# santi-pdp/segan_pytorch

Hardware: AMD Instinct MI355X
Metric: 16384-sample waveform chunks/sec (GAN step) (higher is better)
Workload: dtype f32

## Files before the change

### include/segan_hip.h

```cpp
#ifndef SEGAN_HIP_H
#define SEGAN_HIP_H

#include <stddef.h>
#include <stdint.h>

#ifdef __cplusplus
extern "C" {
#endif

#define SEGAN_ABI_VERSION 17

#define SEGAN_PAD_REFLECT 0
#define SEGAN_PAD_ZERO 1

#define SEGAN_ACT_NONE 0
#define SEGAN_ACT_TANH 1

typedef struct segan_src {
  const float* p0;
  const float* p1;
  int32_t C0;
  int32_t C1;
  const float* scale;
  const float* shift;
// ... 2 lines not shown

int segan_abi_version(void);
const char* segan_last_error(void);

int segan_set_reserved_slots(int n);

size_t segan_packed_f_bytes(int M, int N, int S);
size_t segan_packed_t_bytes(int M, int N, int S);

int segan_pack_weights(const float* w, float* wf, float* wt, int M, int N, int K, int S,
                       int pad_t, void* stream);

#define SEGAN_PREC_FP32 0
#define SEGAN_PREC_BF16 1
#define SEGAN_PREC_BF16X3 3
#define SEGAN_PREC_FP32_BLOCKED 4
size_t segan_packed_bf_bytes(int M, int N, int S, int tform, int planes);
int segan_pack_weights_bf(const float* w, void* out, int M, int N, int K, int S, int tform,
                          int pad_t, int planes, void* stream);

size_t segan_bf16_scratch_bytes(int op, int B, int N, int M, int L, int K, int S, int pad, int planes);
size_t segan_corr_scratch_bytes(void);
void segan_debug_last_corr(int* out6);
void segan_debug_last_wgrad(int* out6);

int segan_conv1d_fwd(const segan_src* x, const void* wf, const float* bias, float* out, int B,
                     int N, int M, int L, int K, int S, int padL, int mode, int roll,
                     int precision, void* scratch, size_t scratch_bytes, void* stream);

int segan_conv1d_dgrad(const float* da, const void* wt, const float* w, float* dx, float* halo,
                       int B, int N, int M, int L, int K, int S, int padL, int roll, int precision,
                       void* scratch, size_t scratch_bytes, void* stream);

#define SEGAN_WGRAD_DETERMINISTIC 1
size_t segan_wgrad_scratch_bytes(int B, int M, int N, int Ls, int S, int precision, int flags);
int segan_wgrad(const segan_src* lo, const segan_src* hi, float* dw, int B, int M, int N, int Ls,
                int K, int S, int padL, int mode, int roll, int precision, int flags, void* scratch,
                size_t scratch_bytes, void* stream);

int segan_deconv1d_fwd(const segan_src* x, const void* wt, const float* w, const float* bias,
                       float* y, int B, int M, int N, int Ls, int K, int S, int pad, int act,
                       int precision, void* scratch, size_t scratch_bytes, void* stream);

int segan_deconv1d_dgrad(const float* dy, const void* wf, float* dx0, float* dx1, int B, int M,
                         int M0, int N, int Ls, int K, int S, int pad, int precision, void* scratch,
                         size_t scratch_bytes, void* stream);


int segan_bn_nsplit(int B, int C, int L);
int segan_bn_stats(const float* x, const float* gamma, const float* beta, float eps,
                   float momentum, float* running_mean, float* running_var, float* mean,
                   float* rstd, float* scale, float* shift, float* ws, int B, int C, int L,
                   void* stream);
int segan_bn_partial(const float* x, float* ws, int B, int C, int L, void* stream);
int segan_bn_final(const float* ws, int nsplit_total, const float* gamma, const float* beta,
                   float eps, float momentum, float* running_mean, float* running_var, float* mean,
                   float* rstd, float* scale, float* shift, int C, void* stream);

int segan_affine_tanh(const float* x, const float* scale, const float* shift, float* y, int B,
                      int C, int L, void* stream);
int segan_scale_mask(const float* x, const float* scale, const float* mask, float* y, int B, int C,
                     int L, void* stream);

int segan_affine_prelu(const float* x, const float* scale, const float* shift, const float* slope,
                       float* y, int B, int C, int L, void* stream);

int segan_sum_skip(const float* x0, const float* slope0, const float* x1, const float* alpha,
                   float* out, int B, int C, int L, void* stream);

int segan_act_bwd(const float* a, const float* dh, const float* dskip, const float* slope,
                  const float* alpha, const float* bn_mean, const float* bn_rstd,
                  const float* bn_gamma, const float* bn_beta, float* da, float* dslope,
                  float* dalpha, float* dgamma, float* dbeta, float* dbias, float* ws, int B, int C,
                  int L, void* stream);
int segan_act_bwd_bn_reduce(const float* a, const float* dh, const float* slope,
                            const float* bn_mean, const float* bn_rstd, const float* bn_gamma,
                            const float* bn_beta, float* dslope, float* dgamma, float* dbeta,
                            float* totals, float* ws, int B, int C, int L, void* stream);
int segan_act_bwd_bn_apply(const float* a, const float* dh, const float* slope,
                           const float* bn_mean, const float* bn_rstd, const float* bn_gamma,
                           const float* bn_beta, const float* totals, float* da, float* dbias,
                           float* ws, int B, int C, int L, double count_total, void* stream);

int segan_tanh_bwd(const float* y, const float* dy, const float* clean, float l1_scale, float* da,
                   float* dbias, float* ws, int B, int C, int L, void* stream);


#define SEGAN_GEMM_DETERMINISTIC 1
size_t segan_gemm_scratch_bytes(int M, int N, int K);
int segan_gemm(const float* A, int64_t sam, int64_t sak, const float* B, int64_t sbk, int64_t sbn,
               float* C, int64_t ldc, int M, int N, int K, int beta0, int flags, void* scratch,
               size_t scratch_bytes, void* stream);

int segan_bias_prelu_rows(const float* x, const float* bias, const float* slope, float* y,
                          int rows, int cols, void* stream);
int segan_bias_prelu_rows_bwd(const float* x, const float* bias, const float* slope,
                              const float* dy, float* dx, float* dslope, float* dbias, int rows,
                              int cols, void* stream);

int segan_mse_const(const float* x, float target, float* loss, float* grad, const float* gout,
                    float gscale, int n, void* stream);
int segan_bce_logits_const(const float* x, float target, float* loss, float* grad,
                           const float* gout, float gscale, int n, void* stream);
int segan_l1_mean(const float* x, const float* y, float* loss, float* ws, int64_t n,
                  void* stream);
int segan_l1_bwd(const float* x, const float* y, const float* gout, float gscale, float* grad,
                 int64_t n, void* stream);

size_t segan_packed_g_bytes(int M, int N, int S);
int segan_pack_weights_g(const float* w, float* wg, int M, int N, int K, int S, void* stream);
int segan_conv1d_dgrad_short(const float* da, const float* wg, float* dx, int B, int N, int M,
                             int L, int K, int S, int padL, int roll, void* stream);

int segan_pool_time_fwd(const float* x, float* y, int* idx, int rows, int L, int mode,
                        void* stream);
int segan_pool_time_bwd(const float* dy, const int* idx, float* dx, int rows, int L, int mode,
                        void* stream);

int segan_mse_mean(const float* x, const float* y, float* loss, float* ws, int64_t n,
                   void* stream);
int segan_mse_bwd(const float* x, const float* y, const float* gout, float gscale, float* grad,
                  int64_t n, void* stream);

size_t segan_snorm_ws_floats(int A, int Bd, int K, int dim);
int segan_snorm_fwd(const float* w, float* u, float* v, float* w_sn, float* sigma, float* ws, int A,
                    int Bd, int K, int dim, int power_iteration, float eps, void* stream);
int segan_snorm_bwd(const float* dw_sn, const float* w, const float* u, const float* v,
                    const float* sigma, float* dw, float* ws, int A, int Bd, int K, int dim,
                    void* stream);

int segan_stft_pitch(int n_fft);
int segan_stft_basis(float* basis, int n_fft, int win, void* stream);
int segan_stft_frames(const float* x, float* frames, int B, int T, int n_fft, int hop, int win,
                      void* stream);
int segan_powdb(const float* S, float* db, int64_t rows, int nbins, int pitch, float eps,
                void* stream);
int segan_powdb_bwd(const float* S, const float* ddb, float* dS, int64_t rows, int nbins, int pitch,
                    float eps, void* stream);
int segan_stft_overlap_add(const float* dframes, float* dx, int B, int T, int n_fft, int hop,
                           int win, void* stream);

int segan_pcm16_prep(const int16_t* pcm, const unsigned char* first, float* clean, float* noisy,
                     int B, int T, double coef, void* stream);

int segan_deemphasis(const float* y, float* x, int rows, int T, double coef, void* stream);
int segan_ssnr_frames(int T, int srate);
int segan_ssnr(const float* ref, const float* deg, float* seg, float* out, int rows, int T,
               int srate, double eps, void* stream);
int segan_wss(const float* ref, const float* deg, double* dist, int rows, int T, int srate,
              void* stream);
int segan_llr(const float* ref, const float* deg, double* dist, int rows, int T, int srate,
              void* stream);
int segan_stoi_plan(int srate, int* pq, int* ntaps, double* taps, int cap, int* bands);
int segan_stoi_dims(int T, int srate, int* dims);
int segan_stoi(const float* ref, const float* deg, const int* lengths, int rows, int T, int srate,
               double* xr, double* yr, double* energy, int* mask, int* kept, int* count,
               double* xs, double* ys, double* X, double* Y, double* rho, double* d, void* stream);

int segan_asl_p56(const float* x, const int* lengths, int rows, int T, int srate, int nbits,
                  double* level, int* counts, int* status, double* q, void* stream);
int segan_additive_mix(const float* clean, const int* lengths, const float* bank, int64_t n_bank,
                       const int64_t* starts, const double* snr_db, const double* px,
                       const float* prev, int rows, int T, float* noisy, float* prev_out,
                       double* info, int* istat, void* stream);
int segan_pcm16_wave(const int16_t* pcm, const int* index, float* wave, float* prev, int n, int B,
                     int T, void* stream);
// ... 35 lines not shown
```

### segan_pytorch_amd/_lib.py

```python
import ctypes
import os
from ctypes import POINTER, Structure, c_char_p, c_double, c_float, c_int, c_int32, c_int64, c_size_t, c_void_p

_HERE = os.path.dirname(os.path.abspath(__file__))
LIB_PATH = os.environ.get('SEGAN_HIP_LIB') or os.path.join(_HERE, 'libsegan_hip.so')

PAD_REFLECT = 0
PAD_ZERO = 1
ACT_NONE = 0
ACT_TANH = 1
ABI_VERSION = 17


class SeganSrc(Structure):
    _fields_ = [('p0', c_void_p), ('p1', c_void_p), ('C0', c_int32), ('C1', c_int32),
                ('scale', c_void_p), ('shift', c_void_p), ('slope', c_void_p)]


_P = c_void_p
_SRC = POINTER(SeganSrc)

SIGNATURES = {
    'segan_abi_version': (c_int, []),
    'segan_set_reserved_slots': (c_int, [c_int]),
    'segan_last_error': (c_char_p, []),
    'segan_packed_f_bytes': (c_size_t, [c_int, c_int, c_int]),
    'segan_packed_t_bytes': (c_size_t, [c_int, c_int, c_int]),
    'segan_pack_weights': (c_int, [_P, _P, _P, c_int, c_int, c_int, c_int, c_int, _P]),
    'segan_packed_bf_bytes': (c_size_t, [c_int, c_int, c_int, c_int, c_int]),
    'segan_pack_weights_bf': (c_int, [_P, _P, c_int, c_int, c_int, c_int, c_int, c_int, c_int, _P]),
    'segan_corr_scratch_bytes': (c_size_t, []),
    'segan_bf16_scratch_bytes': (c_size_t, [c_int] * 9),
    'segan_debug_last_corr': (None, [POINTER(c_int)]),
    'segan_debug_last_wgrad': (None, [POINTER(c_int)]),
    'segan_conv1d_fwd': (c_int, [_SRC, _P, _P, _P, c_int, c_int, c_int, c_int, c_int, c_int, c_int,
                                 c_int, c_int, c_int, _P, c_size_t, _P]),
    'segan_conv1d_dgrad': (c_int, [_P, _P, _P, _P, _P, c_int, c_int, c_int, c_int, c_int, c_int, c_int,
                                   c_int, c_int, _P, c_size_t, _P]),
    'segan_wgrad': (c_int, [_SRC, _SRC, _P, c_int, c_int, c_int, c_int, c_int, c_int, c_int, c_int,
                            c_int, c_int, c_int, _P, c_size_t, _P]),
    'segan_wgrad_scratch_bytes': (c_size_t, [c_int, c_int, c_int, c_int, c_int, c_int, c_int]),
    'segan_deconv1d_fwd': (c_int, [_SRC, _P, _P, _P, _P, c_int, c_int, c_int, c_int, c_int, c_int, c_int,
                                   c_int, c_int, _P, c_size_t, _P]),
    'segan_deconv1d_dgrad': (c_int, [_P, _P, _P, _P, c_int, c_int, c_int, c_int, c_int, c_int, c_int,
                                     c_int, c_int, _P, c_size_t, _P]),
    'segan_bn_nsplit': (c_int, [c_int, c_int, c_int]),
    'segan_bn_stats': (c_int, [_P, _P, _P, c_float, c_float, _P, _P, _P, _P, _P, _P, _P, c_int, c_int,
                               c_int, _P]),
    'segan_bn_partial': (c_int, [_P, _P, c_int, c_int, c_int, _P]),
    'segan_bn_final': (c_int, [_P, c_int, _P, _P, c_float, c_float, _P, _P, _P, _P, _P, _P, c_int, _P]),
    'segan_act_bwd_bn_reduce': (c_int, [_P] * 12 + [c_int, c_int, c_int, _P]),
    'segan_act_bwd_bn_apply': (c_int, [_P] * 11 + [c_int, c_int, c_int, c_double, _P]),
    'segan_affine_prelu': (c_int, [_P, _P, _P, _P, _P, c_int, c_int, c_int, _P]),
    'segan_affine_tanh': (c_int, [_P, _P, _P, _P, c_int, c_int, c_int, _P]),
    'segan_scale_mask': (c_int, [_P, _P, _P, _P, c_int, c_int, c_int, _P]),
    'segan_sum_skip': (c_int, [_P, _P, _P, _P, _P, c_int, c_int, c_int, _P]),
    'segan_bce_logits_const': (c_int, [_P, c_float, _P, _P, _P, c_float, c_int, _P]),
    'segan_act_bwd': (c_int, [_P] * 16 + [c_int, c_int, c_int, _P]),
    'segan_tanh_bwd': (c_int, [_P, _P, _P, c_float, _P, _P, _P, c_int, c_int, c_int, _P]),
    'segan_gemm_scratch_bytes': (c_size_t, [c_int, c_int, c_int]),
    'segan_gemm': (c_int, [_P, c_int64, c_int64, _P, c_int64, c_int64, _P, c_int64, c_int, c_int,
                           c_int, c_int, c_int, _P, c_size_t, _P]),
    'segan_bias_prelu_rows': (c_int, [_P, _P, _P, _P, c_int, c_int, _P]),
    'segan_bias_prelu_rows_bwd': (c_int, [_P, _P, _P, _P, _P, _P, _P, c_int, c_int, _P]),
    'segan_mse_const': (c_int, [_P, c_float, _P, _P, _P, c_float, c_int, _P]),
    'segan_l1_bwd': (c_int, [_P, _P, _P, c_float, _P, c_int64, _P]),
    'segan_l1_mean': (c_int, [_P, _P, _P, _P, c_int64, _P]),
    'segan_packed_g_bytes': (c_size_t, [c_int, c_int, c_int]),
    'segan_pack_weights_g': (c_int, [_P, _P, c_int, c_int, c_int, c_int, _P]),
    'segan_conv1d_dgrad_short': (c_int, [_P, _P, _P, c_int, c_int, c_int, c_int, c_int, c_int, c_int,
                                        c_int, _P]),
    'segan_pool_time_fwd': (c_int, [_P, _P, _P, c_int, c_int, c_int, _P]),
    'segan_pool_time_bwd': (c_int, [_P, _P, _P, c_int, c_int, c_int, _P]),
    'segan_mse_mean': (c_int, [_P, _P, _P, _P, c_int64, _P]),
    'segan_mse_bwd': (c_int, [_P, _P, _P, c_float, _P, c_int64, _P]),
    'segan_snorm_ws_floats': (c_size_t, [c_int, c_int, c_int, c_int]),
    'segan_snorm_fwd': (c_int, [_P, _P, _P, _P, _P, _P, c_int, c_int, c_int, c_int, c_int, c_float, _P]),
    'segan_snorm_bwd': (c_int, [_P, _P, _P, _P, _P, _P, _P, c_int, c_int, c_int, c_int, _P]),
    'segan_pcm16_prep': (c_int, [_P, _P, _P, _P, c_int, c_int, c_double, _P]),
    'segan_stft_basis': (c_int, [_P, c_int, c_int, _P]),
    'segan_stft_frames': (c_int, [_P, _P, c_int, c_int, c_int, c_int, c_int, _P]),
    'segan_stft_pitch': (c_int, [c_int]),
    'segan_powdb': (c_int, [_P, _P, c_int64, c_int, c_int, c_float, _P]),
    'segan_powdb_bwd': (c_int, [_P, _P, _P, c_int64, c_int, c_int, c_float, _P]),
    'segan_stft_overlap_add': (c_int, [_P, _P, c_int, c_int, c_int, c_int, c_int, _P]),
    'segan_deemphasis': (c_int, [_P, _P, c_int, c_int, c_double, _P]),
    'segan_ssnr_frames': (c_int, [c_int, c_int]),
    'segan_ssnr': (c_int, [_P, _P, _P, _P, c_int, c_int, c_int, c_double, _P]),
    'segan_wss': (c_int, [_P, _P, _P, c_int, c_int, c_int, _P]),
    'segan_llr': (c_int, [_P, _P, _P, c_int, c_int, c_int, _P]),
    'segan_stoi_plan': (c_int, [c_int, POINTER(c_int), POINTER(c_int), _P, c_int, POINTER(c_int)]),
    'segan_stoi_dims': (c_int, [c_int, c_int, POINTER(c_int)]),
    'segan_stoi': (c_int, [_P, _P, _P, c_int, c_int, c_int] + [_P] * 13),
    'segan_asl_p56': (c_int, [_P, _P, c_int, c_int, c_int, c_int, _P, _P, _P, _P, _P]),
    'segan_additive_mix': (c_int, [_P, _P, _P, c_int64, _P, _P, _P, _P, c_int, c_int, _P, _P, _P, _P, _P]),
    'segan_resample_plan': (c_int, [c_int, c_int, c_int, c_double, POINTER(c_int), POINTER(c_int), _P, c_int]),
    'segan_resample_dims': (c_int, [c_int, c_int, c_int, POINTER(c_int)]),
    'segan_resample': (c_int, [_P, c_int, _P, c_int, c_int, c_int, c_int, c_int, c_double, _P, c_int,
                               c_int, _P, _P, _P, _P]),
    'segan_pcm16_wave': (c_int, [_P, _P, _P, _P, c_int, c_int, c_int, _P]),
    'segan_preemph_rows': (c_int, [_P, _P, _P, _P, _P, c_int, c_int, c_int, c_double, _P]),
    'segan_rmsprop_step': (c_int, [_P, _P, _P, c_float, c_float, c_float, c_int64, _P]),
    'segan_adam_step': (c_int, [_P, _P, _P, _P, c_float, c_double, c_double, c_float, c_int, c_int64,
                                _P]),
    'segan_fill': (c_int, [_P, c_float, c_int64, _P]),
    'segan_scale': (c_int, [_P, c_float, c_int64, _P]),
    'segan_comm_id_bytes': (c_int, []),
    'segan_comm_unique_id': (c_int, [_P]),
    'segan_comm_init': (c_int, [POINTER(c_void_p), c_int, c_int, _P]),
    'segan_comm_destroy': (c_int, [_P]),
    'segan_comm_rank': (c_int, [_P]),
    'segan_comm_world': (c_int, [_P]),
    'segan_allreduce': (c_int, [_P, _P, c_size_t, c_float, _P]),
    'segan_broadcast': (c_int, [_P, _P, c_size_t, c_int, _P]),
    'segan_allgather': (c_int, [_P, _P, _P, c_size_t, _P]),
}

_lib = None


def load():
    global _lib
    if _lib is not None:
# ... 30 lines not shown
```

### segan_pytorch_amd/csrc/segan_common.h

```cpp
#pragma once
#include <hip/hip_runtime.h>
#include <stdint.h>
#include <stdio.h>
#include <stdarg.h>
#include "../../include/segan_hip.h"

#define SEGAN_OK 0
#define SEGAN_EINVAL (-1)
#define SEGAN_ELAUNCH (-2)
#define SEGAN_EUNSUPPORTED (-3)

void segan_set_error(const char* fmt, ...);
int segan_check_launch(const char* what);

#define SEGAN_REQUIRE(cond, ...)                 \
  do {                                           \
    if (!(cond)) {                               \
      segan_set_error(__VA_ARGS__);              \
      return SEGAN_EINVAL;                       \
    }                                            \
  } while (0)

typedef float f32x16 __attribute__((ext_vector_type(16)));
typedef float f32x4 __attribute__((ext_vector_type(4)));

#define SEGAN_ACC_BLOCK 8

template <int NI, int NJ>
__device__ __forceinline__ void acc_block_flush(f32x16 (&acc)[NI][NJ], f32x16 (&sum)[NI][NJ]) {
#pragma unroll
  for (int i = 0; i < NI; ++i)
#pragma unroll
    for (int j = 0; j < NJ; ++j) {
      sum[i][j] += acc[i][j];
#pragma unroll
      for (int e = 0; e < 16; ++e) acc[i][j][e] = 0.0f;
    }
}

int segan_reserved_slots_value(void);
static inline int segan_grid_slots(int occ) {
  const int g = 256 * occ - segan_reserved_slots_value();
  return g < 64 ? 64 : g;
}

static inline int ceil_div(int a, int b) { return (a + b - 1) / b; }
static inline int round_up(int a, int b) { return ceil_div(a, b) * b; }

__host__ __device__ static inline int segan_hi_index(int p, int L, int padL, int mode, int roll) {
  int i = p - padL;
  if (mode == SEGAN_PAD_REFLECT) {
    if (i < 0) i = -i;
    if (i >= L) i = 2 * (L - 1) - i;
  }
  if (i < 0 || i >= L) return -1;
  if (roll != 0) {
    i -= roll;
    if (i < 0) i += L;
    if (i >= L) i -= L;
  }
  return i;
}

#define SEGAN_MAX_XF_CH 16384

struct ChanXf {
  float sc, sh, sl;
};

__device__ __forceinline__ ChanXf segan_chan_xf(const segan_src& s, int c) {
  ChanXf x;
  x.sc = s.scale[c];
  x.sh = s.shift[c];
  x.sl = s.slope[c];
  return x;
}

__device__ __forceinline__ float segan_apply_xf(const ChanXf& x, float v) {
  v = fmaf(v, x.sc, x.sh);
  return v > 0.0f ? v : v * x.sl;
}

int segan_src_defaults(segan_src* s, hipStream_t st, const char* what);

__device__ __forceinline__ const float* segan_src_row(const segan_src& s, int b, int n, int L) {
  if (n < s.C0) return s.p0 + ((size_t)b * s.C0 + n) * (size_t)L;
  return s.p1 + ((size_t)b * s.C1 + (n - s.C0)) * (size_t)L;
}

__device__ __forceinline__ float warp_sum(float v) {
#pragma unroll
  for (int o = 32; o > 0; o >>= 1) v += __shfl_down(v, o, 64);
  return v;
}
```

### segan_pytorch_amd/csrc/segan_conv.hip

```cpp
#include "segan_conv_shared.h"

template <int MB, int NB, int WM, int U>
struct TileGeom {
  static constexpr int S = 32 / U;
  static constexpr int WN = 4 / WM;
  static constexpr int NI = MB / (32 * WM);
  static constexpr int NJ = NB / (32 * WN);
  static constexpr int NPT = MB / S;
};

struct TileWork {
  int tile, c0, c1;
  bool partial;
  int piece;
};

struct TileIter {
  int tileA;
  long unit, unit_end;
  int first_tile;
  __device__ __forceinline__ void init(const CorrArgs& a, int nch) {
    tileA = blockIdx.x;
    unit = (long)blockIdx.x * a.sk_units;
    unit_end = min(unit + (long)a.sk_units, a.sk_total);
// ... 1379 lines not shown
  SEGAN_REQUIRE(precision_ok(precision), "deconv1d_dgrad: precision must be 0, 1, 3 or 4");
  SEGAN_REQUIRE(stride_ok(S), "deconv1d_dgrad: stride %d not in {1,2,4}", S);
  SEGAN_REQUIRE(K >= 1 && K <= 32, "deconv1d_dgrad: kernel width %d not in [1,32]", K);
  SEGAN_REQUIRE(B > 0 && N > 0 && M > 0 && Ls > 0, "deconv1d_dgrad: bad sizes");
  SEGAN_REQUIRE(M0 >= 0 && M0 <= M, "deconv1d_dgrad: split %d outside [0,%d]", M0, M);
  SEGAN_REQUIRE(dy && wf, "deconv1d_dgrad: NULL pointer");
  SEGAN_REQUIRE(dx0 || dx1, "deconv1d_dgrad: both destinations NULL");
  const int U = 32 / S;
  CorrArgs a = {};
  a.acc_block = acc_block;
  a.in.p0 = dy; a.in.p1 = nullptr; a.in.C0 = N; a.in.C1 = 0;
  a.in.scale = a.in.shift = a.in.slope = nullptr;
  a.wp = (const float*)wf;
  a.bias = nullptr; a.halo = nullptr;
  a.B = B; a.Cv = N * S; a.Ktot = N * 32; a.RP = f_pitch(M); a.Rvalid = M;
  a.Tcols = Ls; a.Ctot = B * Ls;
  a.Lin = S * Ls; a.padL = pad; a.mode = SEGAN_PAD_ZERO; a.roll = 0;
  a.win_start = 0; a.H = U - 1;
  a.NP = 1; a.Nout = 0;
  if (M0 == 0) { a.out0 = dx1; a.OC0 = M; a.out1 = nullptr; a.OC1 = 0; }
  else { a.out0 = dx0; a.OC0 = M0; a.out1 = dx1; a.OC1 = M - M0; }
  a.Lout = Ls; a.act = SEGAN_ACT_NONE;
  a.out0_elems = (size_t)B * a.OC0 * Ls;
  a.out1_elems = (size_t)B * a.OC1 * Ls;
  a.f_pair = f_pair(N, K); a.zphase = -1;
  if (precision) {
    CorrArgs a2 = a;
    const int e = segan_corr_bf2_f(a2, U, wf, precision, scratch, scratch_bytes, (hipStream_t)stream);
    return e;
  }
  set_scratch(a, scratch, scratch_bytes);
  return launch_corr<true, false>(a, U, (hipStream_t)stream);
}

extern "C" int segan_deconv1d_fwd(const segan_src* x, const void* wt, const float* w,
                                  const float* bias, float* y, int B, int M, int N, int Ls, int K,
                                  int S, int pad, int act, int precision, void* scratch,
                                  size_t scratch_bytes, void* stream) {
  const int acc_block = precision == SEGAN_PREC_FP32_BLOCKED;
  if (acc_block) precision = SEGAN_PREC_FP32;
  SEGAN_REQUIRE(precision_ok(precision), "deconv1d_fwd: precision must be 0, 1, 3 or 4");
  SEGAN_REQUIRE(stride_ok(S), "deconv1d_fwd: stride %d not in {1,2,4}", S);
  SEGAN_REQUIRE(K >= 1 && K <= 32, "deconv1d_fwd: kernel width %d not in [1,32]", K);
  SEGAN_REQUIRE(B > 0 && N > 0 && M > 0 && Ls > 0, "deconv1d_fwd: bad sizes");
  SEGAN_REQUIRE(y && (wt || (w && N <= 2)), "deconv1d_fwd: NULL pointer");
  SEGAN_REQUIRE(pad >= 0 && K - 2 * pad - S == (K & 1),
                "deconv1d_fwd: K=%d S=%d pad=%d does not give an output of S*Ls samples", K, S, pad);
  SEGAN_REQUIRE(act == SEGAN_ACT_NONE || act == SEGAN_ACT_TANH, "deconv1d_fwd: bad activation");
  if (int e = check_src(x, M, "deconv1d_fwd")) return e;
  const int U = 32 / S;
  CorrArgs a = {};
  a.acc_block = acc_block;
  a.in = *x;
  a.wp = (const float*)wt;
  a.out0 = y; a.out1 = nullptr; a.bias = bias; a.halo = nullptr;
  a.NP = t_np(N, S); a.Nout = N;
  a.B = B; a.Cv = M; a.Ktot = M * U; a.RP = t_pitch(N, S); a.Rvalid = S * a.NP;
  a.Tcols = Ls; a.Ctot = B * Ls;
  a.Lin = Ls; a.padL = 0; a.mode = SEGAN_PAD_ZERO; a.roll = 0;
  int cmin = 1 << 30, cmax = 0;
  for (int r = 0; r < S; ++r) {
    const int c = (r + pad) / S;
    cmin = c < cmin ? c : cmin;
    cmax = c > cmax ? c : cmax;
  }
  for (int r = 0; r < 4; ++r) a.rowshift[r] = r < S ? (r + pad) / S - cmin : 0;
  a.win_start = cmin - (U - 1);
  a.H = U - 1 + (cmax - cmin);
  a.OC0 = N; a.OC1 = 0; a.Lout = S * Ls; a.act = act;
  a.o_padL = 0; a.o_roll = 0; a.o_padR = 0;
  a.out0_elems = (size_t)B * N * S * Ls;
  a.f_pair = 0; a.zphase = t_zphase(K, S, pad);
  if (w && N <= 2) return segan_launch_tsmall(a, w, K, M, N, S, pad, (hipStream_t)stream);
  if (precision && act == SEGAN_ACT_NONE) {
    CorrArgs a2 = a;
    const int e = segan_corr_bf2_t(a2, U, wt, precision, scratch, scratch_bytes, (hipStream_t)stream);
    return e;
  }
  SEGAN_REQUIRE(precision == 0, "deconv1d_fwd: tanh epilogue only on the fp32 path");
  set_scratch(a, scratch, scratch_bytes);
  return launch_corr<false, true>(a, U, (hipStream_t)stream);
}

extern "C" int segan_conv1d_dgrad(const float* da, const void* wt, const float* w, float* dx,
                                  float* halo, int B, int N, int M, int L, int K, int S, int padL,
                                  int roll, int precision, void* scratch, size_t scratch_bytes,
                                  void* stream) {
  const int acc_block = precision == SEGAN_PREC_FP32_BLOCKED;
  if (acc_block) precision = SEGAN_PREC_FP32;
  SEGAN_REQUIRE(precision_ok(precision), "conv1d_dgrad: precision must be 0, 1, 3 or 4");
  SEGAN_REQUIRE(stride_ok(S), "conv1d_dgrad: stride %d not in {1,2,4}", S);
  SEGAN_REQUIRE(K >= 1 && K <= 32, "conv1d_dgrad: kernel width %d not in [1,32]", K);
  SEGAN_REQUIRE(B > 0 && N > 0 && M > 0 && L > 0 && L % S == 0, "conv1d_dgrad: bad sizes");
  SEGAN_REQUIRE(da && dx && halo && (wt || (w && N <= 2)), "conv1d_dgrad: NULL pointer");
  SEGAN_REQUIRE(roll > -L && roll < L, "conv1d_dgrad: |roll| must be < L");
  const int padR = K - 1 - padL >= 0 ? (K - S - padL > 0 ? K - S - padL : 0) : -1;
  SEGAN_REQUIRE(padL >= 0 && padR >= 0 && padL < L && K - S - padL < L, "conv1d_dgrad: bad padding");
  const int U = 32 / S;
  const int Ls = L / S;
  hipStream_t st = (hipStream_t)stream;
  CorrArgs a = {};
  a.acc_block = acc_block;
  a.in.p0 = da; a.in.p1 = nullptr; a.in.C0 = M; a.in.C1 = 0;
  a.in.scale = a.in.shift = a.in.slope = nullptr;
  a.wp = (const float*)wt;
  a.out0 = dx; a.out1 = nullptr; a.bias = nullptr; a.halo = halo;
  a.NP = t_np(N, S); a.Nout = N;
  a.B = B; a.Cv = M; a.Ktot = M * U; a.RP = t_pitch(N, S); a.Rvalid = S * a.NP;
  a.Tcols = (L + padL + padR - 1) / S + 1;
  a.Ctot = B * a.Tcols;
  a.Lin = Ls; a.padL = 0; a.mode = SEGAN_PAD_ZERO; a.roll = 0;
  for (int r = 0; r < 4; ++r) a.rowshift[r] = 0;
  a.win_start = -(U - 1);
  a.H = U - 1;
  a.OC0 = N; a.OC1 = 0; a.Lout = L; a.act = SEGAN_ACT_NONE;
  a.o_padL = padL; a.o_roll = roll; a.o_padR = padR;
  a.out0_elems = (size_t)B * N * L;
  a.halo_elems = (size_t)B * N * (padL + padR);
  a.f_pair = 0; a.zphase = t_zphase(K, S, 0);
  set_scratch(a, scratch, scratch_bytes);
  int e;
  if (w && N <= 2) {
    e = segan_launch_tsmall(a, w, K, M, N, S, 0, st);
  } else if (precision) {
    CorrArgs a2 = a;
    e = segan_corr_bf2_t(a2, U, wt, precision, scratch, scratch_bytes, st);
  } else {
    e = launch_corr<false, true>(a, U, st);
  }
  if (e) return e;
  if (padL + padR > 0) {
    const int rows = B * N;
    const int per_sample = (padL < L - 1 - padR) ? 1 : 0;
    const long nthreads = per_sample ? (long)rows * (padL + padR) : rows;
    hipLaunchKernelGGL(fold_halo_kernel, dim3((unsigned)((nthreads + 255) / 256)), dim3(256), 0, st,
                       dx, halo, rows, L, padL, padR, roll, per_sample);
    return segan_check_launch("fold_halo_kernel");
  }
  return SEGAN_OK;
}

static bool short_ok(int N, int M, int L, int K, int S, int padL) {
  if (!stride_ok(S) || L % S != 0) return false;
  const int Ls = L / S;
  return (Ls == 4 || Ls == 8 || Ls == 16 || Ls == 32 || Ls == 64) && N % 4 == 0 &&
         M % CS_KC == 0 && K >= 1 && K <= 32 && padL >= 0 && K - 1 - padL >= 0 && padL < L &&
         K - S - padL < L;
}

extern "C" size_t segan_packed_g_bytes(int M, int N, int S) {
  if (!stride_ok(S) || M <= 0 || N <= 0) return 0;
  return (size_t)M * N * 32 * sizeof(float);
}

extern "C" int segan_pack_weights_g(const float* w, float* wg, int M, int N, int K, int S,
                                    void* stream) {
  SEGAN_REQUIRE(w && wg && M > 0 && N > 0, "pack_weights_g: bad arguments");
  SEGAN_REQUIRE(stride_ok(S) && K >= 1 && K <= 32, "pack_weights_g: stride in {1,2,4}, K <= 32");
  const size_t total = (size_t)M * N * 32;
  const int blocks = (int)((total + 255) / 256 > 8192 ? 8192 : (total + 255) / 256);
  hipLaunchKernelGGL(pack_g_kernel, dim3(blocks), dim3(256), 0, (hipStream_t)stream, w, wg, M, N, K,
                     S);
  return segan_check_launch("pack_weights_g");
}

extern "C" int segan_conv1d_dgrad_short(const float* da, const float* wg, float* dx, int B, int N,
                                        int M, int L, int K, int S, int padL, int roll,
                                        void* stream) {
  SEGAN_REQUIRE(da && wg && dx && B > 0, "conv1d_dgrad_short: bad arguments");
  SEGAN_REQUIRE(roll > -L && roll < L, "conv1d_dgrad_short: |roll| must be < L");
  if (!short_ok(N, M, L, K, S, padL)) {
    segan_set_error("conv1d_dgrad_short: geometry not covered (L/S in {4,8,16,32,64}, N %% 4 == 0, "
                    "M %% 16 == 0)");
    return SEGAN_EUNSUPPORTED;
  }
  ShortArgs a;
  a.da = da; a.wg = wg; a.dx = dx;
  a.B = B; a.N = N; a.M = M; a.L = L; a.Ls = L / S; a.padL = padL;
  a.padRw = K - S - padL > 0 ? K - S - padL : 0;
  a.roll = roll;
  a.ncoltiles = ceil_div(B, 128 / a.Ls);
  const size_t lds = 4 * 32 * 65 * sizeof(float);
  const dim3 grid((unsigned)(N / 4 * a.ncoltiles));
  static const bool blocked = [] {
    const char* e = getenv("SEGAN_SHORT_ORDER");
    return !(e && e[0] == '0');
  }();
  a.xr8 = a.xbc = 0;
  if (blocked && (N / 4) % 8 == 0) {
    a.xr8 = N / 4 / 8;
    a.xbc = a.xr8 >= 128 ? 1 : 128 / a.xr8;
  }
  hipStream_t st = (hipStream_t)stream;
  if (S == 4) hipLaunchKernelGGL(conv_dgrad_short_kernel<4>, grid, dim3(256), lds, st, a);
  else if (S == 2) hipLaunchKernelGGL(conv_dgrad_short_kernel<2>, grid, dim3(256), lds, st, a);
  else hipLaunchKernelGGL(conv_dgrad_short_kernel<1>, grid, dim3(256), lds, st, a);
  return segan_check_launch("conv_dgrad_short_kernel");
}
```

### segan_pytorch_amd/csrc/segan_conv_edge.hip

```cpp
#include "segan_conv_shared.h"

template <int S, int N, int PM, int KT>
__global__ __launch_bounds__(256) void tsmall_kernel(const CorrArgs a, const float* __restrict__ w,
                                                     int Krt, int M) {
  const int K = KT ? KT : Krt;
  constexpr int U = 32 / S;
  constexpr int MC = 16;
  constexpr int TW = 256 + U;
  __shared__ float xs[MC][TW + 1];
  const int tid = threadIdx.x;
  const int b = blockIdx.y;
  const int q0 = blockIdx.x * 256;
  const int q = q0 + tid;
  float acc[S][N];
#pragma unroll
  for (int r = 0; r < S; ++r)
#pragma unroll
    for (int n = 0; n < N; ++n) acc[r][n] = 0.0f;

  const int t0 = q0 + a.win_start + tid, t1 = t0 + 256;
  const bool ok0 = t0 >= 0 && t0 < a.Lin, ok1 = tid < U && t1 >= 0 && t1 < a.Lin;
  const int o0 = ok0 ? t0 : 0, o1 = ok1 ? t1 : 0;
  const int bo0 = b * a.in.C0 * a.Lin, bo1 = b * a.in.C1 * a.Lin;
  float pv0[MC], pv1[MC];
  auto load_rows = [&](int mc0) {
#pragma unroll
    for (int mc = 0; mc < MC; ++mc) {
      const int m = mc0 + mc < M ? mc0 + mc : 0;
      const bool seg1 = m >= a.in.C0;
      const float* rowp = seg1 ? a.in.p1 + (size_t)(m - a.in.C0) * a.Lin + bo1
                               : a.in.p0 + (size_t)m * a.Lin + bo0;
      pv0[mc] = rowp[o0];
      pv1[mc] = rowp[o1];
    }
  };
  load_rows(0);
  for (int mc0 = 0; mc0 < M; mc0 += MC) {
#pragma unroll
    for (int mc = 0; mc < MC; ++mc) {
      const bool mok = mc0 + mc < M;
      const ChanXf xf = segan_chan_xf(a.in, mok ? mc0 + mc : 0);
      xs[mc][tid] = (mok && ok0) ? segan_apply_xf(xf, pv0[mc]) : 0.0f;
      if (tid < U) xs[mc][256 + tid] = (mok && ok1) ? segan_apply_xf(xf, pv1[mc]) : 0.0f;
    }
    __syncthreads();
    if (mc0 + MC < M) load_rows(mc0 + MC);
    const int mcn = min(MC, M - mc0);
    for (int mc = 0; mc < mcn; ++mc) {
      float xv[U + 1];
#pragma unroll
      for (int j = 0; j <= U; ++j) xv[j] = xs[mc][tid + j];
      const float* wm = w + (size_t)(mc0 + mc) * N * K;
#pragma unroll
      for (int r = 0; r < S; ++r) {
        const int rho = (r + PM) % S;
        const int cs = (r + PM) / S;
#pragma unroll
        for (int u = 0; u < U; ++u) {
          const int k = S * u + rho;
          if (KT) {
            if (k < KT) {
#pragma unroll
              for (int n = 0; n < N; ++n)
                acc[r][n] = fmaf(wm[n * KT + k], xv[cs + (U - 1) - u], acc[r][n]);
            }
          } else {
            const int kc = k < K ? k : K - 1;
#pragma unroll
            for (int n = 0; n < N; ++n) {
              float wv = wm[n * K + kc];
              wv = k < K ? wv : 0.0f;
              acc[r][n] = fmaf(wv, xv[cs + (U - 1) - u], acc[r][n]);
            }
          }
        }
      }
    }
    __syncthreads();
  }
  if (q >= a.Tcols) return;
#pragma unroll
  for (int r = 0; r < S; ++r)
#pragma unroll
    for (int n = 0; n < N; ++n) {
      float v = acc[r][n] + (a.bias ? a.bias[n] : 0.0f);
      if (a.act == SEGAN_ACT_TANH) v = tanhf(v);
      const int P = S * q + r;
      int ii = P - a.o_padL;
      const size_t rowoff = (size_t)b * N + n;
      if (ii >= 0 && ii < a.Lout) {
        if (a.o_roll != 0) {
          ii -= a.o_roll;
          if (ii < 0) ii += a.Lout;
          if (ii >= a.Lout) ii -= a.Lout;
        }
        a.out0[rowoff * (size_t)a.Lout + ii] = v;
      } else if (a.halo != nullptr) {
        const int hl = a.o_padL + a.o_padR;
        if (ii < 0) a.halo[rowoff * hl + P] = v;
        else if (ii - a.Lout < a.o_padR) a.halo[rowoff * hl + a.o_padL + (ii - a.Lout)] = v;
      }
    }
}

template <int S, int N, int KT>
static int launch_tsmall_snk(const CorrArgs& a, const float* w, int K, int M, int pad,
                             hipStream_t st) {
  dim3 grid(ceil_div(a.Tcols, 256), a.B);
  switch (pad % S) {
    case 0: hipLaunchKernelGGL((tsmall_kernel<S, N, 0, KT>), grid, dim3(256), 0, st, a, w, K, M); break;
    case 1: hipLaunchKernelGGL((tsmall_kernel<S, N, 1 % S, KT>), grid, dim3(256), 0, st, a, w, K, M); break;
    case 2: hipLaunchKernelGGL((tsmall_kernel<S, N, 2 % S, KT>), grid, dim3(256), 0, st, a, w, K, M); break;
    default: hipLaunchKernelGGL((tsmall_kernel<S, N, 3 % S, KT>), grid, dim3(256), 0, st, a, w, K, M); break;
  }
  return segan_check_launch("tsmall_kernel");
}

template <int S, int N>
static int launch_tsmall_sn(const CorrArgs& a, const float* w, int K, int M, int pad,
                            hipStream_t st) {
  if (K == 31) return launch_tsmall_snk<S, N, 31>(a, w, K, M, pad, st);
  return launch_tsmall_snk<S, N, 0>(a, w, K, M, pad, st);
}


template <int N, int PM>
__global__ __launch_bounds__(256) void tsmall4_kernel(const CorrArgs a, const float* __restrict__ w,
                                                      int M) {
  constexpr int S = 4, U = 8, KT = 31, Q = 4;
  constexpr int MC = 8;
  constexpr int TWQ = Q * 256 + 12;
  __shared__ __attribute__((aligned(16))) float xs[MC][TWQ];
  const int tid = threadIdx.x;
  const int b = blockIdx.y;
  const int q0 = blockIdx.x * (Q * 256);
  typedef float f32x2 __attribute__((ext_vector_type(2)));
  f32x2 acc[Q / 2][S][N];
#pragma unroll
  for (int i = 0; i < Q / 2; ++i)
#pragma unroll
    for (int r = 0; r < S; ++r)
#pragma unroll
      for (int n = 0; n < N; ++n) acc[i][r][n] = f32x2{0.0f, 0.0f};
  int so[5];
  unsigned sok = 0u;
#pragma unroll
  for (int i = 0; i < 5; ++i) {
    const int j = tid + 256 * i;
    const int t = q0 + a.win_start + j;
    const bool ok = (i < 4 || tid < 12) && t >= 0 && t < a.Lin;
    so[i] = ok ? t : 0;
    if (ok) sok |= 1u << i;
  }
  const int bo0 = b * a.in.C0 * a.Lin, bo1 = b * a.in.C1 * a.Lin;
  float pv[MC][5];
  auto load_rows = [&](int mc0) {
#pragma unroll
    for (int mc = 0; mc < MC; ++mc) {
      const int m = mc0 + mc < M ? mc0 + mc : 0;
      const bool seg1 = m >= a.in.C0;
      const float* rowp = seg1 ? a.in.p1 + (size_t)(m - a.in.C0) * a.Lin + bo1
                               : a.in.p0 + (size_t)m * a.Lin + bo0;
#pragma unroll
      for (int i = 0; i < 5; ++i) pv[mc][i] = rowp[so[i]];
    }
  };
  load_rows(0);
  for (int mc0 = 0; mc0 < M; mc0 += MC) {
#pragma unroll
    for (int mc = 0; mc < MC; ++mc) {
      const bool mok = mc0 + mc < M;
      const ChanXf xf = segan_chan_xf(a.in, mok ? mc0 + mc : 0);
#pragma unroll
      for (int i = 0; i < 4; ++i)
        xs[mc][tid + 256 * i] = (mok && ((sok >> i) & 1u)) ? segan_apply_xf(xf, pv[mc][i]) : 0.0f;
      if (tid < 12) xs[mc][1024 + tid] = (mok && ((sok >> 4) & 1u)) ? segan_apply_xf(xf, pv[mc][4]) : 0.0f;
    }
    __syncthreads();
    if (mc0 + MC < M) load_rows(mc0 + MC);
    const int mcn = min(MC, M - mc0);
    for (int mc = 0; mc < mcn; ++mc) {
      f32x2 xe[6], xo[5];
#pragma unroll
      for (int i = 0; i < 3; ++i) {
        const f32x4 t4 = *reinterpret_cast<const f32x4*>(&xs[mc][4 * tid + 4 * i]);
        xe[2 * i] = f32x2{t4[0], t4[1]};
        xe[2 * i + 1] = f32x2{t4[2], t4[3]};
      }
#pragma unroll
      for (int i = 0; i < 5; ++i) xo[i] = f32x2{xs[mc][4 * tid + 2 * i + 1], xs[mc][4 * tid + 2 * i + 2]};
      typedef const __attribute__((address_space(4))) float cfl;
      constexpr int NPW = (N * KT + 1) / 2;
      cfl* wm = (cfl*)w + (size_t)(mc0 + mc) * N * KT;
      f32x2 wp[NPW];
#pragma unroll
      for (int p = 0; p < NPW; ++p) {
        const int f0 = 2 * p + 1 < N * KT ? 2 * p : N * KT - 2;
        wp[p] = f32x2{wm[f0], wm[f0 + 1]};
      }
#pragma unroll
      for (int r = 0; r < S; ++r) {
        const int rho = (r + PM) % S, cs = (r + PM) / S;
#pragma unroll
        for (int u = 0; u < U; ++u) {
          const int k = S * u + rho;
          if (k < KT) {
#pragma unroll
            for (int n = 0; n < N; ++n) {
              const int f = n * KT + k;
              const bool last = 2 * (f >> 1) + 1 >= N * KT;
              const int p = f >> 1, h = last ? 1 : (f & 1);
#pragma unroll
              for (int ip = 0; ip < Q / 2; ++ip) {
                const int j = 2 * ip + cs + (U - 1) - u;
                const f32x2 xp = (j & 1) ? xo[j >> 1] : xe[j >> 1];
                if (h)
                  asm("v_pk_fma_f32 %0, %1, %2, %0 op_sel:[1,0,0] op_sel_hi:[1,1,1]"
                      : "+v"(acc[ip][r][n]) : "s"(wp[p]), "v"(xp));
                else
                  asm("v_pk_fma_f32 %0, %1, %2, %0 op_sel:[0,0,0] op_sel_hi:[0,1,1]"
                      : "+v"(acc[ip][r][n]) : "s"(wp[p]), "v"(xp));
              }
            }
          }
        }
      }
    }
    __syncthreads();
  }
#pragma unroll
  for (int n = 0; n < N; ++n) {
    const float bs = a.bias ? a.bias[n] : 0.0f;
    const size_t rowoff = (size_t)b * N + n;
#pragma unroll
    for (int i = 0; i < Q; ++i) {
      const int q = q0 + Q * tid + i;
      if (q >= a.Tcols) continue;
      float v[S];
#pragma unroll
      for (int r = 0; r < S; ++r) {
        v[r] = acc[i >> 1][r][n][i & 1] + bs;
        if (a.act == SEGAN_ACT_TANH) v[r] = tanhf(v[r]);
      }
      const int i0 = S * q - a.o_padL;
      if (a.o_roll == 0 && i0 >= 0 && i0 + 3 < a.Lout && (a.o_padL & 3) == 0) {
        const f32x4 o = {v[0], v[1], v[2], v[3]};
        *reinterpret_cast<f32x4*>(a.out0 + rowoff * (size_t)a.Lout + i0) = o;
        continue;
      }
#pragma unroll
      for (int r = 0; r < S; ++r) {
        const int P = S * q + r;
        int ii = P - a.o_padL;
        if (ii >= 0 && ii < a.Lout) {
          if (a.o_roll != 0) {
            ii -= a.o_roll;
            if (ii < 0) ii += a.Lout;
            if (ii >= a.Lout) ii -= a.Lout;
          }
          a.out0[rowoff * (size_t)a.Lout + ii] = v[r];
        } else if (a.halo != nullptr) {
          const int hl = a.o_padL + a.o_padR;
          if (ii < 0) a.halo[rowoff * hl + P] = v[r];
          else if (ii - a.Lout < a.o_padR) a.halo[rowoff * hl + a.o_padL + (ii - a.Lout)] = v[r];
        }
      }
    }
  }
}

template <int N>
static int launch_tsmall4(const CorrArgs& a, const float* w, int M, int pad, hipStream_t st) {
  dim3 grid(ceil_div(a.Tcols, 1024), a.B);
  switch (pad % 4) {
    case 0: hipLaunchKernelGGL((tsmall4_kernel<N, 0>), grid, dim3(256), 0, st, a, w, M); break;
    case 1: hipLaunchKernelGGL((tsmall4_kernel<N, 1>), grid, dim3(256), 0, st, a, w, M); break;
    case 2: hipLaunchKernelGGL((tsmall4_kernel<N, 2>), grid, dim3(256), 0, st, a, w, M); break;
    default: hipLaunchKernelGGL((tsmall4_kernel<N, 3>), grid, dim3(256), 0, st, a, w, M); break;
  }
  return segan_check_launch("tsmall4_kernel");
}

int segan_launch_tsmall(CorrArgs& a, const float* w, int K, int M, int N, int S, int pad,
                         hipStream_t st) {
  if (int e = segan_src_defaults(&a.in, st, "tsmall")) return e;
  if (S == 4 && K == 31 && a.Tcols >= 1024)
    return N == 1 ? launch_tsmall4<1>(a, w, M, pad, st) : launch_tsmall4<2>(a, w, M, pad, st);
  if (N == 1) {
    if (S == 4) return launch_tsmall_sn<4, 1>(a, w, K, M, pad, st);
    if (S == 2) return launch_tsmall_sn<2, 1>(a, w, K, M, pad, st);
    return launch_tsmall_sn<1, 1>(a, w, K, M, pad, st);
  }
  if (S == 4) return launch_tsmall_sn<4, 2>(a, w, K, M, pad, st);
  if (S == 2) return launch_tsmall_sn<2, 2>(a, w, K, M, pad, st);
  return launch_tsmall_sn<1, 2>(a, w, K, M, pad, st);
}


template <int S, int N, int XW>
__device__ __forceinline__ void fsmall_stage_window(const CorrArgs& a, int b, int t0, int tid,
                                                    float (&xs)[N][XW]) {
  constexpr int NX = (XW + 255) / 256;
  constexpr int BT = 6;
  const float* rows[N];
  ChanXf xf[N];
#pragma unroll
  for (int n = 0; n < N; ++n) {
    rows[n] = segan_src_row(a.in, b, n, a.Lin);
    xf[n] = segan_chan_xf(a.in, n);
  }
#pragma unroll
  for (int g0 = 0; g0 < NX; g0 += BT) {
    float v[N][BT];
    int idx[BT];
#pragma unroll
    for (int i = 0; i < BT; ++i) {
      const int j = tid + 256 * (g0 + i);
      idx[i] = (g0 + i < NX && j < XW) ? segan_hi_index(S * t0 + j, a.Lin, a.padL, a.mode, a.roll) : -1;
#pragma unroll
      for (int n = 0; n < N; ++n) v[n][i] = rows[n][idx[i] >= 0 ? idx[i] : 0];
    }
#pragma unroll
    for (int i = 0; i < BT; ++i) {
      const int j = tid + 256 * (g0 + i);
      if (g0 + i < NX && j < XW) {
#pragma unroll
        for (int n = 0; n < N; ++n) xs[n][j] = idx[i] >= 0 ? segan_apply_xf(xf[n], v[n][i]) : 0.0f;
      }
    }
  }
}

template <int S, int N, int WST>
__device__ __forceinline__ void fsmall_stage_weights(const CorrArgs& a, int m0, int tid, float* ws) {
  constexpr int U = 32 / S;
  constexpr int NW = 64 * N * 32 / 256;
  constexpr int BT = 8;
  static_assert(NW % BT == 0, "weight staging batches");
#pragma unroll
  for (int g0 = 0; g0 < NW; g0 += BT) {
    float v[BT];
#pragma unroll
    for (int i = 0; i < BT; ++i) {
      const int e = tid + 256 * (g0 + i);
      const int ml = e & 63, nk = e >> 6;
      const int n = nk >> 5, k = nk & 31;
      const int row = (n * S + k % S) * U + k / S;
      const int m = m0 + ml;
      v[i] = a.wp[(size_t)row * a.RP + (m < a.RP ? m : 0)];
      v[i] = m < a.RP ? v[i] : 0.0f;
    }
#pragma unroll
    for (int i = 0; i < BT; ++i) {
      const int e = tid + 256 * (g0 + i);
      const int ml = e & 63, nk = e >> 6;
      ws[ml * WST + (nk >> 5) * 32 + (nk & 31)] = v[i];
    }
  }
}

template <int S, int N>
__global__ __launch_bounds__(256) void fsmall_kernel(const CorrArgs a, int M) {
  constexpr int XW = S * 256 + 32;
  constexpr int WST = N * 32 + 4;
  __shared__ __attribute__((aligned(16))) float xs[N][XW];
  __shared__ __attribute__((aligned(16))) float ws[64 * WST];
  const int tid = threadIdx.x;
  const int b = blockIdx.y;
  const int t0 = blockIdx.x * 256;
  fsmall_stage_window<S, N, XW>(a, b, t0, tid, xs);
  const int t = t0 + tid;
  for (int m0 = 0; m0 < M; m0 += 64) {
    fsmall_stage_weights<S, N, WST>(a, m0, tid, ws);
    __syncthreads();
    float xv[N][32];
#pragma unroll
    for (int n = 0; n < N; ++n) {
      if (S == 4) {
// ... 146 lines not shown
```

### segan_pytorch_amd/csrc/segan_conv_shared.h

```cpp
#pragma once
#include "segan_common.h"
#include <stdlib.h>

#define KCH 64

struct ColTile {
  int col0, b0, t_first, len0;
};

__device__ __forceinline__ ColTile make_coltile(int col0, int Tcols, int NBcols) {
  ColTile t;
  t.col0 = col0;
  t.b0 = col0 / Tcols;
  t.t_first = col0 - t.b0 * Tcols;
  t.len0 = min(Tcols - t.t_first, NBcols);
  return t;
}

__device__ __forceinline__ void lds_pos_decode(const ColTile& ct, int j, int Tcols, int H, int& s,
                                               int& tau) {
  if (j < ct.len0 + H) {
    s = 0;
    tau = ct.t_first + j;
  } else {
// ... 23 lines not shown
  int Lin;
  int padL, mode, roll;
  int win_start, H, RLs;
  int rowshift[4];
  int NP, Nout;
  int OC0, OC1, Lout, act;
  int o_padL, o_roll, o_padR;
  int in_identity;
  int sk_nfull;
  int sk_units;
  long sk_total;
  int rt0;
  size_t out0_elems, out1_elems, halo_elems;
  float* sk_ws;
  size_t sk_ws_floats;
  int xf_mode;
  int acc_block;
  int RLv, nld;
  int f_pair;
  int zphase;
  int tile_order, nrt;
};




static inline int samples_per_tile(int Tcols, int NB) {
  if (Tcols >= NB) return (Tcols % NB == 0) ? 1 : 2;
  return (NB % Tcols == 0) ? NB / Tcols : (NB + Tcols - 2) / Tcols + 1;
}

static inline int t_np(int N, int S) { return round_up(N, 128 / S); }

struct WgradArgs {
  segan_src lo;
  segan_src hi;
  float* dw;
  int B, M, N, K, Ls, Lhi;
  int Cv;
  int padL, mode, roll;
  int Ctot;
  int cols_per_split;
  int H, RLw;
  int ls_magic;
  int per_magic;
  int bf_qc;
  int bf_cps;
  int Mp;
  int w2_cps, w2_nch;
  int w2_cpsample;
  int w2_spc;
  int w2_lsshift;
  int w2_pw, w2_nld;
  float* w2_slabs;
};

__device__ __forceinline__ float epi_bias(const float* bias, int base, int rl0, int h) {
  typedef const __attribute__((address_space(4))) float cfloat;
  cfloat* bp = (cfloat*)bias + base;
  const float lo = bp[rl0], hi = bp[rl0 + 4];
  return h ? hi : lo;
}

static inline int f_pitch(int M) { return M <= 64 ? 64 : round_up(M, 128); }
static inline int f_rows(int N) { return round_up(N * 32, KCH); }
static inline int t_pitch(int N, int S) { return S * t_np(N, S); }
static inline int t_rows(int M, int S) { return round_up(M * (32 / S), KCH); }

static inline int f_pair(int N, int K) { return K == 31 && N > 2 && (N & 1) == 0; }
static inline int t_zphase(int K, int S, int pad_t) {
  return (K == 31 && S > 1) ? (((S - 1 - pad_t) % S) + S) % S : -1;
}

static inline bool stride_ok(int S) { return S == 1 || S == 2 || S == 4; }
static inline bool precision_ok(int p) { return p == 0 || p == 1 || p == 3; }
static inline int check_src(const segan_src* s, int C, const char* what) {
  SEGAN_REQUIRE(s != nullptr && s->p0 != nullptr, "%s: source is NULL", what);
  SEGAN_REQUIRE(s->C0 > 0 && s->C1 >= 0 && s->C0 + s->C1 == C,
                "%s: channel segments %d+%d != %d", what, s->C0, s->C1, C);
  SEGAN_REQUIRE(s->C1 == 0 || s->p1 != nullptr, "%s: second segment pointer is NULL", what);
  return SEGAN_OK;
}

int segan_launch_tsmall(CorrArgs& a, const float* w, int K, int M, int N, int S, int pad, hipStream_t st);
int segan_launch_fsmall(CorrArgs& a, int M, int N, int S, hipStream_t st);

void segan_note_corr_launch(int kind, unsigned grid, const CorrArgs& a, int ntiles);
int segan_corr_bf2_f(CorrArgs& a, int U, const void* wp3, int planes, void* scratch,
                     size_t scratch_bytes, hipStream_t st);
int segan_corr_bf2_t(CorrArgs& a, int U, const void* wp3, int planes, void* scratch,
                     size_t scratch_bytes, hipStream_t st);
size_t segan_corr_bf2_scratch_bytes(int B, int Cv, int Tcols, int H, int planes);
int segan_wgrad_bf2(WgradArgs& a, int U, int planes, void* scratch, size_t scratch_bytes, hipStream_t st);
void segan_note_wgrad_launch(int kind, int tiles, int nsplit, int chunks_per_split);
size_t segan_wgrad_bf2_scratch_bytes(int B, int M, int N, int Ls, int S, int planes);
```

### segan_pytorch_amd/csrc/segan_pointwise.hip

```cpp
#include "segan_common.h"

#define PW_THREADS 256

static int pw_nsplit(int B, int C, int L) {
  int ns = ceil_div(2048, C);
  if (ns > B) ns = B;
  long per = (long)B * L / ns;
  while (ns > 1 && per < 2048) {
    ns = (ns + 1) / 2;
    per = (long)B * L / ns;
  }
  return ns < 1 ? 1 : ns;
}

extern "C" int segan_bn_nsplit(int B, int C, int L) {
  if (B <= 0 || C <= 0 || L <= 0) return 0;
  return pw_nsplit(B, C, L);
}

template <int NV>
__device__ __forceinline__ void block_sum(float (&v)[NV], float* sm) {
  const int lane = threadIdx.x & 63, wave = threadIdx.x >> 6;
#pragma unroll
  for (int k = 0; k < NV; ++k) v[k] = warp_sum(v[k]);
  if (lane == 0)
#pragma unroll
    for (int k = 0; k < NV; ++k) sm[wave * NV + k] = v[k];
  __syncthreads();
  if (threadIdx.x == 0) {
#pragma unroll
    for (int k = 0; k < NV; ++k) {
      float s = 0.f;
      for (int w = 0; w < PW_THREADS / 64; ++w) s += sm[w * NV + k];
      v[k] = s;
    }
  }
  __syncthreads();
}

struct ChanRange {
  int c, b_beg, b_end;
};
__device__ __forceinline__ ChanRange chan_range(int B, int nsplit) {
  ChanRange r;
  r.c = blockIdx.x;
  const int per = (B + nsplit - 1) / nsplit;
  r.b_beg = blockIdx.y * per;
  r.b_end = min(B, r.b_beg + per);
  return r;
}

__device__ __forceinline__ void chan_combine(float& n, float& mean, float& m2, float nb, float mb,
                                             float qb) {
  const float tot = n + nb;
  if (tot <= 0.0f) return;
  const float d = mb - mean;
  const float f = nb / tot;
  mean = fmaf(d, f, mean);
  m2 = m2 + qb + d * d * n * f;
  n = tot;
}

__global__ void bn_partial_kernel(const float* __restrict__ x, float* __restrict__ ws, int B, int C,
                                  int L, int nsplit) {
  __shared__ float sm[3 * (PW_THREADS / 64)];
  const ChanRange cr = chan_range(B, nsplit);
  const int nb = cr.b_end - cr.b_beg;
  const float* base = x + ((size_t)cr.b_beg * C + cr.c) * L;
  const size_t sstride = (size_t)C * L;
  const bool vec = (L & 3) == 0 && ((uintptr_t)x & 15) == 0;
  const int Lv = vec ? L >> 2 : L;
  int tr = PW_THREADS;
  while (tr > Lv && tr > 1) tr >>= 1;
  const int rp = PW_THREADS / tr;
  const int t0 = threadIdx.x % tr, r0 = threadIdx.x / tr;
  float K = 0.0f, s1 = 0.0f, s2 = 0.0f, n = 0.0f;
  if (r0 < nb && t0 < Lv) K = base[(size_t)r0 * sstride + (vec ? 4 * t0 : t0)];
  for (int b = r0; b < nb; b += rp) {
    const float* row = base + b * sstride;
    if (vec) {
      for (int t = t0; t < Lv; t += tr) {
        const f32x4 u = *reinterpret_cast<const f32x4*>(row + 4 * t);
#pragma unroll
        for (int e = 0; e < 4; ++e) {
          const float d = u[e] - K;
          s1 += d;
          s2 = fmaf(d, d, s2);
        }
        n += 4.0f;
      }
    } else {
      for (int t = t0; t < Lv; t += tr) {
        const float d = row[t] - K;
        s1 += d;
        s2 = fmaf(d, d, s2);
        n += 1.0f;
      }
    }
  }
  float mean = 0.0f, m2 = 0.0f;
  if (n > 0.0f) {
    const float r = s1 / n;
    mean = K + r;
    m2 = fmaxf(s2 - s1 * r, 0.0f);
  }
#pragma unroll
  for (int o = 32; o > 0; o >>= 1) {
    const float nb2 = __shfl_down(n, o, 64), mb2 = __shfl_down(mean, o, 64), qb2 = __shfl_down(m2, o, 64);
    chan_combine(n, mean, m2, nb2, mb2, qb2);
  }
  const int lane = threadIdx.x & 63, wave = threadIdx.x >> 6;
  if (lane == 0) {
    sm[3 * wave] = n; sm[3 * wave + 1] = mean; sm[3 * wave + 2] = m2;
  }
  __syncthreads();
  if (threadIdx.x == 0) {
    for (int w = 1; w < PW_THREADS / 64; ++w) chan_combine(n, mean, m2, sm[3 * w], sm[3 * w + 1], sm[3 * w + 2]);
    float* w = ws + ((size_t)blockIdx.y * C + cr.c) * 3;
    w[0] = n;
    w[1] = mean;
    w[2] = m2;
  }
}

__device__ __forceinline__ void bn_affine(float gamma, float beta, float mean, float rstd,
                                          float& scale, float& shift) {
  scale = gamma * rstd;
  shift = fmaf(-mean, scale, beta);
}

__global__ void bn_final_kernel(const float* __restrict__ ws, const float* gamma, const float* beta,
                                float eps, float momentum, float* running_mean, float* running_var,
                                float* mean_o, float* rstd_o, float* scale_o, float* shift_o, int C,
                                int nsplit) {
  const int c = blockIdx.x * blockDim.x + threadIdx.x;
  if (c >= C) return;
  double n = 0.0, mean = 0.0, m2 = 0.0;
  for (int s = 0; s < nsplit; ++s) {
    const float* w = ws + ((size_t)s * C + c) * 3;
    const double nb = w[0], mb = w[1], qb = w[2];
    if (nb <= 0.0) continue;
    const double tot = n + nb;
    const double d = mb - mean;
    mean += d * nb / tot;
    m2 += qb + d * d * n * nb / tot;
    n = tot;
  }
  const double var = n > 0 ? m2 / n : 0.0;
  const float rstd = (float)(1.0 / sqrt(var + (double)eps));
  const float g = gamma ? gamma[c] : 1.0f;
  const float bt = beta ? beta[c] : 0.0f;
  float sc, sh;
  bn_affine(g, bt, (float)mean, rstd, sc, sh);
  if (mean_o) mean_o[c] = (float)mean;
  if (rstd_o) rstd_o[c] = rstd;
  if (scale_o) scale_o[c] = sc;
  if (shift_o) shift_o[c] = sh;
  if (running_mean) running_mean[c] = (1.0f - momentum) * running_mean[c] + momentum * (float)mean;
  if (running_var) {
    const double unb = n > 1 ? m2 / (n - 1.0) : var;
    running_var[c] = (1.0f - momentum) * running_var[c] + momentum * (float)unb;
  }
}

extern "C" int segan_bn_stats(const float* x, const float* gamma, const float* beta, float eps,
                              float momentum, float* running_mean, float* running_var, float* mean,
                              float* rstd, float* scale, float* shift, float* ws, int B, int C,
                              int L, void* stream) {
  SEGAN_REQUIRE(x && ws, "bn_stats: NULL pointer");
  SEGAN_REQUIRE(B > 0 && C > 0 && L > 0, "bn_stats: bad sizes");
  hipStream_t st = (hipStream_t)stream;
  const int ns = pw_nsplit(B, C, L);
  hipLaunchKernelGGL(bn_partial_kernel, dim3(C, ns), dim3(PW_THREADS), 0, st, x, ws, B, C, L, ns);
  hipLaunchKernelGGL(bn_final_kernel, dim3(ceil_div(C, 64)), dim3(64), 0, st, ws, gamma, beta, eps,
                     momentum, running_mean, running_var, mean, rstd, scale, shift, C, ns);
  return segan_check_launch("bn_stats");
}

extern "C" int segan_bn_partial(const float* x, float* ws, int B, int C, int L, void* stream) {
  SEGAN_REQUIRE(x && ws, "bn_partial: NULL pointer");
  SEGAN_REQUIRE(B > 0 && C > 0 && L > 0, "bn_partial: bad sizes");
  const int ns = pw_nsplit(B, C, L);
  hipLaunchKernelGGL(bn_partial_kernel, dim3(C, ns), dim3(PW_THREADS), 0, (hipStream_t)stream, x, ws,
                     B, C, L, ns);
  return segan_check_launch("bn_partial");
}

extern "C" int segan_bn_final(const float* ws, int nsplit_total, const float* gamma,
                              const float* beta, float eps, float momentum, float* running_mean,
                              float* running_var, float* mean, float* rstd, float* scale,
                              float* shift, int C, void* stream) {
  SEGAN_REQUIRE(ws && nsplit_total > 0 && C > 0, "bn_final: bad arguments");
  hipLaunchKernelGGL(bn_final_kernel, dim3(ceil_div(C, 64)), dim3(64), 0, (hipStream_t)stream, ws,
                     gamma, beta, eps, momentum, running_mean, running_var, mean, rstd, scale, shift,
                     C, nsplit_total);
  return segan_check_launch("bn_final");
}

__global__ void affine_prelu_kernel(const float* __restrict__ x, const float* scale,
                                    const float* shift, const float* slope, float* __restrict__ y,
                                    size_t total, int C, int L) {
  for (size_t i = blockIdx.x * (size_t)blockDim.x + threadIdx.x; i < total;
       i += (size_t)gridDim.x * blockDim.x) {
    const int c = (int)((i / L) % C);
    float v = x[i];
    v = fmaf(v, scale ? scale[c] : 1.0f, shift ? shift[c] : 0.0f);
    if (slope) v = v > 0.f ? v : v * slope[c];
    y[i] = v;
  }
}

extern "C" int segan_affine_prelu(const float* x, const float* scale, const float* shift,
                                  const float* slope, float* y, int B, int C, int L, void* stream) {
// ... 5 lines not shown
                     shift, slope, y, total, C, L);
  return segan_check_launch("affine_prelu");
}

__global__ void affine_tanh_kernel(const float* __restrict__ x, const float* scale,
                                   const float* shift, float* __restrict__ y, size_t total, int C,
                                   int L) {
  for (size_t i = blockIdx.x * (size_t)blockDim.x + threadIdx.x; i < total;
       i += (size_t)gridDim.x * blockDim.x) {
    const int c = (int)((i / L) % C);
    y[i] = tanhf(fmaf(x[i], scale ? scale[c] : 1.0f, shift ? shift[c] : 0.0f));
  }
}

extern "C" int segan_affine_tanh(const float* x, const float* scale, const float* shift, float* y,
                                 int B, int C, int L, void* stream) {
  SEGAN_REQUIRE(x && y, "affine_tanh: NULL pointer");
  SEGAN_REQUIRE(B > 0 && C > 0 && L > 0, "affine_tanh: bad sizes");
  const size_t total = (size_t)B * C * L;
  const int blocks = (int)((total + 255) / 256 > 4096 ? 4096 : (total + 255) / 256);
  hipLaunchKernelGGL(affine_tanh_kernel, dim3(blocks), dim3(256), 0, (hipStream_t)stream, x, scale,
                     shift, y, total, C, L);
  return segan_check_launch("affine_tanh");
}

__global__ void scale_mask_kernel(const float* __restrict__ x, const float* scale,
                                  const float* __restrict__ mask, float* __restrict__ y,
                                  size_t total, int C, int L) {
  for (size_t i = blockIdx.x * (size_t)blockDim.x + threadIdx.x; i < total;
       i += (size_t)gridDim.x * blockDim.x) {
    const int c = (int)((i / L) % C);
    y[i] = x[i] * (scale ? scale[c] : 1.0f) * mask[i];
  }
}

extern "C" int segan_scale_mask(const float* x, const float* scale, const float* mask, float* y,
                                int B, int C, int L, void* stream) {
  SEGAN_REQUIRE(x && mask && y, "scale_mask: NULL pointer");
  SEGAN_REQUIRE(B > 0 && C > 0 && L > 0, "scale_mask: bad sizes");
  const size_t total = (size_t)B * C * L;
  const int blocks = (int)((total + 255) / 256 > 4096 ? 4096 : (total + 255) / 256);
  hipLaunchKernelGGL(scale_mask_kernel, dim3(blocks), dim3(256), 0, (hipStream_t)stream, x, scale,
                     mask, y, total, C, L);
  return segan_check_launch("scale_mask");
}

__global__ void sum_skip_kernel(const float* __restrict__ x0, const float* slope0,
                                const float* __restrict__ x1, const float* alpha,
                                float* __restrict__ out, size_t total, int C, int L) {
  for (size_t i = blockIdx.x * (size_t)blockDim.x + threadIdx.x; i < total;
       i += (size_t)gridDim.x * blockDim.x) {
    const int c = (int)((i / L) % C);
    float v = x0[i];
    if (slope0) v = v > 0.f ? v : v * slope0[c];
    out[i] = fmaf(alpha[c], x1[i], v);
  }
}

extern "C" int segan_sum_skip(const float* x0, const float* slope0, const float* x1,
                              const float* alpha, float* out, int B, int C, int L, void* stream) {
  SEGAN_REQUIRE(x0 && x1 && alpha && out, "sum_skip: NULL pointer");
  SEGAN_REQUIRE(B > 0 && C > 0 && L > 0, "sum_skip: bad sizes");
  const size_t total = (size_t)B * C * L;
  const int blocks = (int)((total + 255) / 256 > 4096 ? 4096 : (total + 255) / 256);
  hipLaunchKernelGGL(sum_skip_kernel, dim3(blocks), dim3(256), 0, (hipStream_t)stream, x0, slope0,
                     x1, alpha, out, total, C, L);
  return segan_check_launch("sum_skip");
}

struct ActBwdArgs {
  const float* a;
  const float* dh;
  const float* dskip;
  const float* slope;
  const float* alpha;
  const float* mean;
  const float* rstd;
  const float* gamma;
  const float* beta;
  float* da;
  float* ws;
  int B, C, L, nsplit;
  float inv_count;
};

template <int PHASE>
__global__ void act_bwd_kernel(const ActBwdArgs p) {
  __shared__ float sm[16];
  const ChanRange cr = chan_range(p.B, p.nsplit);
  const int c = cr.c;
  const int nb = cr.b_end - cr.b_beg;
  const float sl = p.slope ? p.slope[c] : 1.0f;
  const float al = p.alpha ? p.alpha[c] : 0.0f;
  float mu = 0.f, rs = 1.f, ga = 1.f, be = 0.f, dbeta_m = 0.f, dgamma_m = 0.f, sc = 1.f, sh = 0.f;
  if (PHASE != 0) {
    mu = p.mean[c];
    rs = p.rstd[c];
    ga = p.gamma ? p.gamma[c] : 1.0f;
    be = p.beta ? p.beta[c] : 0.0f;
    bn_affine(ga, be, mu, rs, sc, sh);
  }
  if (PHASE == 2) {
    const float* tot = p.ws + (size_t)p.nsplit * p.C * 4 + (size_t)c * 2;
    dbeta_m = tot[0] * p.inv_count;
    dgamma_m = tot[1] * p.inv_count;
  }
  float r[3] = {0.f, 0.f, 0.f};
  const bool has_skip = p.dskip != nullptr;
  auto elem = [&](float av, float dh, float ds) -> float {
    if (PHASE == 0) {
      float g = dh * (av > 0.f ? 1.0f : sl);
      r[0] += dh * (av > 0.f ? 0.0f : av);
      if (has_skip) {
        g = fmaf(al, ds, g);
        r[1] = fmaf(ds, av, r[1]);
      }
      r[2] += g;
      return g;
    }
    const float xh = (av - mu) * rs;
    const float v = fmaf(av, sc, sh);
    const float g = dh * (v > 0.f ? 1.0f : sl);
    if (PHASE == 1) {
      r[0] += dh * (v > 0.f ? 0.0f : v);
      r[1] += g;
      r[2] = fmaf(g, xh, r[2]);
      return 0.0f;
    }
    const float d = ga * rs * (g - dbeta_m - xh * dgamma_m);
    r[0] += d;
    return d;
  };
  const size_t base = ((size_t)cr.b_beg * p.C + c) * p.L;
  const size_t sstride = (size_t)p.C * p.L;
  const bool vec = (p.L & 3) == 0 &&
                   (((uintptr_t)p.a | (uintptr_t)p.dh | (uintptr_t)p.dskip | (uintptr_t)p.da) & 15) == 0;
  const int Lv = vec ? p.L >> 2 : p.L;
  int tr = PW_THREADS;
  while (tr > Lv && tr > 1) tr >>= 1;
  const int rp = PW_THREADS / tr;
  const int t0 = threadIdx.x % tr, r0 = threadIdx.x / tr;
  const f32x4 z4 = {0.f, 0.f, 0.f, 0.f};
  for (int b = r0; b < nb; b += rp) {
    const size_t ro = base + b * sstride;
    if (vec) {
      for (int t = t0; t < Lv; t += tr) {
        const size_t i = ro + 4 * (size_t)t;
        const f32x4 av = *reinterpret_cast<const f32x4*>(p.a + i);
        const f32x4 dh = p.dh ? *reinterpret_cast<const f32x4*>(p.dh + i) : z4;
        const f32x4 ds = has_skip ? *reinterpret_cast<const f32x4*>(p.dskip + i) : z4;
        f32x4 o;
#pragma unroll
        for (int e = 0; e < 4; ++e) o[e] = elem(av[e], dh[e], ds[e]);
        if (PHASE != 1) *reinterpret_cast<f32x4*>(p.da + i) = o;
      }
    } else {
      for (int t = t0; t < Lv; t += tr) {
        const size_t i = ro + t;
        const float o = elem(p.a[i], p.dh ? p.dh[i] : 0.0f, has_skip ? p.dskip[i] : 0.0f);
        if (PHASE != 1) p.da[i] = o;
      }
    }
  }
  block_sum<3>(r, sm);
  if (threadIdx.x == 0) {
    float* w = p.ws + ((size_t)blockIdx.y * p.C + c) * 4;
    w[0] = r[0];
    w[1] = r[1];
    w[2] = r[2];
  }
}

template <int PHASE>
__global__ void act_bwd_final_kernel(const ActBwdArgs p, float* dslope, float* dalpha,
                                     float* dgamma, float* dbeta, float* dbias) {
  const int c = blockIdx.x * blockDim.x + threadIdx.x;
  if (c >= p.C) return;
  float s0 = 0.f, s1 = 0.f, s2 = 0.f;
  for (int s = 0; s < p.nsplit; ++s) {
    const float* w = p.ws + ((size_t)s * p.C + c) * 4;
    s0 += w[0];
    s1 += w[1];
    s2 += w[2];
  }
  if (PHASE == 0) {
    if (dslope) dslope[c] += s0;
    if (dalpha) dalpha[c] += s1;
    if (dbias) dbias[c] += s2;
  } else if (PHASE == 1) {
    if (dslope) dslope[c] += s0;
    if (dbeta) dbeta[c] += s1;
    if (dgamma) dgamma[c] += s2;
    float* tot = p.ws + (size_t)p.nsplit * p.C * 4 + (size_t)c * 2;
    tot[0] = s1;
    tot[1] = s2;
  } else {
    if (dbias) dbias[c] += s0;
  }
}

extern "C" int segan_act_bwd(const float* a, const float* dh, const float* dskip,
                             const float* slope, const float* alpha, const float* bn_mean,
                             const float* bn_rstd, const float* bn_gamma, const float* bn_beta,
                             float* da, float* dslope, float* dalpha, float* dgamma, float* dbeta,
                             float* dbias, float* ws, int B, int C, int L, void* stream) {
  SEGAN_REQUIRE(a && da && ws, "act_bwd: NULL pointer");
  SEGAN_REQUIRE(dh || dskip, "act_bwd: no incoming gradient");
  SEGAN_REQUIRE(B > 0 && C > 0 && L > 0, "act_bwd: bad sizes");
  SEGAN_REQUIRE((bn_mean == nullptr) == (bn_rstd == nullptr), "act_bwd: mean/rstd must pair");
  SEGAN_REQUIRE(!(dskip && !alpha), "act_bwd: dskip needs alpha");
  SEGAN_REQUIRE(!(bn_mean && dskip), "act_bwd: BN layers have no skip tap");
  hipStream_t st = (hipStream_t)stream;
  ActBwdArgs p;
  p.a = a; p.dh = dh; p.dskip = dskip; p.slope = slope; p.alpha = alpha;
  p.mean = bn_mean; p.rstd = bn_rstd; p.gamma = bn_gamma; p.beta = bn_beta;
  p.da = da; p.ws = ws; p.B = B; p.C = C; p.L = L;
  p.nsplit = pw_nsplit(B, C, L);
  p.inv_count = 1.0f / ((float)B * (float)L);
  const dim3 grid(C, p.nsplit), fgrid(ceil_div(C, 64));
  if (!bn_mean) {
    hipLaunchKernelGGL(act_bwd_kernel<0>, grid, dim3(PW_THREADS), 0, st, p);
    hipLaunchKernelGGL(act_bwd_final_kernel<0>, fgrid, dim3(64), 0, st, p, dslope, dalpha, dgamma,
                       dbeta, dbias);
  } else {
    hipLaunchKernelGGL(act_bwd_kernel<1>, grid, dim3(PW_THREADS), 0, st, p);
    hipLaunchKernelGGL(act_bwd_final_kernel<1>, fgrid, dim3(64), 0, st, p, dslope, dalpha, dgamma,
                       dbeta, dbias);
    hipLaunchKernelGGL(act_bwd_kernel<2>, grid, dim3(PW_THREADS), 0, st, p);
    hipLaunchKernelGGL(act_bwd_final_kernel<2>, fgrid, dim3(64), 0, st, p, dslope, dalpha, dgamma,
                       dbeta, dbias);
  }
  return segan_check_launch("act_bwd");
}

extern "C" int segan_act_bwd_bn_reduce(const float* a, const float* dh, const float* slope,
                                       const float* bn_mean, const float* bn_rstd,
                                       const float* bn_gamma, const float* bn_beta, float* dslope,
                                       float* dgamma, float* dbeta, float* totals, float* ws, int B,
                                       int C, int L, void* stream) {
  SEGAN_REQUIRE(a && dh && bn_mean && bn_rstd && totals && ws, "act_bwd_bn_reduce: NULL pointer");
  SEGAN_REQUIRE(B > 0 && C > 0 && L > 0, "act_bwd_bn_reduce: bad sizes");
  hipStream_t st = (hipStream_t)stream;
  ActBwdArgs p;
  p.a = a; p.dh = dh; p.dskip = nullptr; p.slope = slope; p.alpha = nullptr;
  p.mean = bn_mean; p.rstd = bn_rstd; p.gamma = bn_gamma; p.beta = bn_beta;
  p.da = nullptr; p.ws = ws; p.B = B; p.C = C; p.L = L;
  p.nsplit = pw_nsplit(B, C, L);
  p.inv_count = 1.0f / ((float)B * (float)L);
  hipLaunchKernelGGL(act_bwd_kernel<1>, dim3(C, p.nsplit), dim3(PW_THREADS), 0, st, p);
  hipLaunchKernelGGL(act_bwd_final_kernel<1>, dim3(ceil_div(C, 64)), dim3(64), 0, st, p, dslope,
                     (float*)nullptr, dgamma, dbeta, (float*)nullptr);
  if (hipMemcpyAsync(totals, ws + (size_t)p.nsplit * C * 4, (size_t)C * 2 * sizeof(float),
                     hipMemcpyDeviceToDevice, st) != hipSuccess) {
    segan_set_error("act_bwd_bn_reduce: copy of the totals failed");
    return SEGAN_ELAUNCH;
  }
  return segan_check_launch("act_bwd_bn_reduce");
}

extern "C" int segan_act_bwd_bn_apply(const float* a, const float* dh, const float* slope,
                                      const float* bn_mean, const float* bn_rstd,
                                      const float* bn_gamma, const float* bn_beta,
                                      const float* totals, float* da, float* dbias, float* ws, int B,
                                      int C, int L, double count_total, void* stream) {
  SEGAN_REQUIRE(a && dh && bn_mean && bn_rstd && totals && da && ws, "act_bwd_bn_apply: NULL pointer");
  SEGAN_REQUIRE(B > 0 && C > 0 && L > 0 && count_total >= (double)B * L, "act_bwd_bn_apply: bad sizes");
  hipStream_t st = (hipStream_t)stream;
  ActBwdArgs p;
  p.a = a; p.dh = dh; p.dskip = nullptr; p.slope = slope; p.alpha = nullptr;
  p.mean = bn_mean; p.rstd = bn_rstd; p.gamma = bn_gamma; p.beta = bn_beta;
  p.da = da; p.ws = ws; p.B = B; p.C = C; p.L = L;
  p.nsplit = pw_nsplit(B, C, L);
  p.inv_count = (float)(1.0 / count_total);
  if (hipMemcpyAsync(ws + (size_t)p.nsplit * C * 4, totals, (size_t)C * 2 * sizeof(float),
                     hipMemcpyDeviceToDevice, st) != hipSuccess) {
    segan_set_error("act_bwd_bn_apply: copy of the totals failed");
    return SEGAN_ELAUNCH;
  }
  hipLaunchKernelGGL(act_bwd_kernel<2>, dim3(C, p.nsplit), dim3(PW_THREADS), 0, st, p);
  hipLaunchKernelGGL(act_bwd_final_kernel<2>, dim3(ceil_div(C, 64)), dim3(64), 0, st, p,
                     (float*)nullptr, (float*)nullptr, (float*)nullptr, (float*)nullptr, dbias);
  return segan_check_launch("act_bwd_bn_apply");
}

__global__ void tanh_bwd_kernel(const float* __restrict__ y, const float* dy, const float* clean,
                                float l1_scale, float* __restrict__ da, float* ws, int B, int C,
                                int L, int nsplit) {
  __shared__ float sm[16];
  const ChanRange cr = chan_range(B, nsplit);
  const int nb = cr.b_end - cr.b_beg;
  const long cnt = (long)(nb > 0 ? nb : 0) * L;
  float r[1] = {0.f};
  for (long e = threadIdx.x; e < cnt; e += PW_THREADS) {
    const int b = cr.b_beg + (int)(e / L);
    const int t = (int)(e % L);
    const size_t i = ((size_t)b * C + cr.c) * L + t;
    const float yv = y[i];
    float g = dy ? dy[i] : 0.0f;
    if (clean) {
      const float d = yv - clean[i];
      g += l1_scale * (d > 0.f ? 1.0f : (d < 0.f ? -1.0f : 0.0f));
    }
    const float d = g * (1.0f - yv * yv);
    da[i] = d;
    r[0] += d;
  }
  block_sum<1>(r, sm);
  if (threadIdx.x == 0) ws[(size_t)blockIdx.y * C + cr.c] = r[0];
}

__global__ void sum_splits_add_kernel(const float* ws, float* out, int C, int nsplit) {
  const int c = blockIdx.x * blockDim.x + threadIdx.x;
  if (c >= C) return;
  float s = 0.f;
  for (int k = 0; k < nsplit; ++k) s += ws[(size_t)k * C + c];
  out[c] += s;
}

extern "C" int segan_tanh_bwd(const float* y, const float* dy, const float* clean, float l1_scale,
                              float* da, float* dbias, float* ws, int B, int C, int L,
                              void* stream) {
  SEGAN_REQUIRE(y && da && ws, "tanh_bwd: NULL pointer");
  SEGAN_REQUIRE(dy || clean, "tanh_bwd: no incoming gradient");
  SEGAN_REQUIRE(B > 0 && C > 0 && L > 0, "tanh_bwd: bad sizes");
  hipStream_t st = (hipStream_t)stream;
  const int ns = pw_nsplit(B, C, L);
  hipLaunchKernelGGL(tanh_bwd_kernel, dim3(C, ns), dim3(PW_THREADS), 0, st, y, dy, clean, l1_scale,
                     da, ws, B, C, L, ns);
  if (dbias)
    hipLaunchKernelGGL(sum_splits_add_kernel, dim3(ceil_div(C, 64)), dim3(64), 0, st, ws, dbias, C,
                       ns);
  return segan_check_launch("tanh_bwd");
}

__global__ void bias_prelu_rows_kernel(const float* __restrict__ x, const float* bias,
                                       const float* slope, float* __restrict__ y, int rows,
                                       int cols) {
  const size_t total = (size_t)rows * cols;
  for (size_t i = blockIdx.x * (size_t)blockDim.x + threadIdx.x; i < total;
       i += (size_t)gridDim.x * blockDim.x) {
    const int c = (int)(i % cols);
    float v = x[i] + (bias ? bias[c] : 0.0f);
    if (slope) v = v > 0.f ? v : v * slope[c];
    y[i] = v;
  }
}

extern "C" int segan_bias_prelu_rows(const float* x, const float* bias, const float* slope,
                                     float* y, int rows, int cols, void* stream) {
  SEGAN_REQUIRE(x && y && rows > 0 && cols > 0, "bias_prelu_rows: bad arguments");
  const size_t total = (size_t)rows * cols;
  const int blocks = (int)((total + 255) / 256 > 2048 ? 2048 : (total + 255) / 256);
  hipLaunchKernelGGL(bias_prelu_rows_kernel, dim3(blocks), dim3(256), 0, (hipStream_t)stream, x,
                     bias, slope, y, rows, cols);
  return segan_check_launch("bias_prelu_rows");
}
// ... 342 lines not shown
```

### segan_pytorch_amd/csrc/segan_wgrad.hip

```cpp
#include "segan_conv_shared.h"


template <int TK>
__device__ __forceinline__ int wg_sdiv(int x, int Ls, int magic) {
  return (Ls >= TK) ? (x >= Ls ? 1 : 0) : ((x * magic) >> 16);
}

template <int NI, int NJ>
__device__ __forceinline__ void wgrad_slab_store(float* slab, const f32x16 (&acc)[NI][NJ], int tid) {
  f32x4* s4 = reinterpret_cast<f32x4*>(slab);
#pragma unroll
  for (int i = 0; i < NI; ++i)
#pragma unroll
    for (int j = 0; j < NJ; ++j)
#pragma unroll
      for (int q = 0; q < 4; ++q) {
        const f32x4 v = {acc[i][j][4 * q], acc[i][j][4 * q + 1], acc[i][j][4 * q + 2],
                         acc[i][j][4 * q + 3]};
        s4[((i * NJ + j) * 4 + q) * 256 + tid] = v;
      }
}

template <int MB, int NBT>
__global__ __launch_bounds__(256) void wgrad_group_kernel(float* slabs, int nsplit, int gsz) {
// ... 220 lines not shown
      }
    }
  };

  load_chunk(0);
  store_chunk(0);
  __syncthreads();
  for (int ch = 0; ch < nch; ++ch) {
    const int buf = ch & 1;
    if (ch + 1 < nch) load_chunk(ch + 1);
    const float* Al = Al0 + buf * (MB * AST);
    const float* Bl = Bl0 + buf * (CVW * RLw);
    const int t_first = (split_beg + ch * TK) % Ls;
    int bpos[NJ8][NJ];
#pragma unroll
    for (int j = 0; j < NJ8; ++j) {
      const int k0 = 8 * j + 4 * h;
      const int p = k0 + wg_sdiv<TK>(t_first + k0, Ls, a.ls_magic) * a.H;
#pragma unroll
      for (int jj = 0; jj < NJ; ++jj) bpos[j][jj] = bbase[jj] + p;
    }
    f32x4 af0[NI], af1[NI];
    float bv0[NJ], bv1[NJ];
    auto read_a = [&](int j, f32x4 (&af)[NI]) {
#pragma unroll
      for (int i = 0; i < NI; ++i) af[i] = *reinterpret_cast<const f32x4*>(Al + aoff[i] + 8 * j);
    };
    auto read_b = [&](int s, float (&bv)[NJ]) {
#pragma unroll
      for (int jj = 0; jj < NJ; ++jj) bv[jj] = Bl[bpos[s / 4][jj] + (s & 3)];
    };
    auto mma = [&](const f32x4 (&af)[NI], int e, const float (&bv)[NJ]) {
#pragma unroll
      for (int i = 0; i < NI; ++i)
#pragma unroll
        for (int jj = 0; jj < NJ; ++jj)
          acc[i][jj] = __builtin_amdgcn_mfma_f32_32x32x2f32(af[i][e], bv[jj], acc[i][jj], 0, 0, 0);
    };
    read_a(0, af0);
    read_b(0, bv0);
#define SB __builtin_amdgcn_sched_barrier(0)
#pragma unroll
    for (int j = 0; j < NJ8; j += 2) {
      read_a(j + 1, af1);
      read_b(4 * j + 1, bv1); SB; mma(af0, 0, bv0); SB;
      read_b(4 * j + 2, bv0); SB; mma(af0, 1, bv1); SB;
      read_b(4 * j + 3, bv1); SB; mma(af0, 2, bv0); SB;
      read_b(4 * j + 4, bv0); SB; mma(af0, 3, bv1); SB;
      if (j + 2 < NJ8) read_a(j + 2, af0);
      read_b(4 * j + 5, bv1); SB; mma(af1, 0, bv0); SB;
      read_b(4 * j + 6, bv0); SB; mma(af1, 1, bv1); SB;
      read_b(4 * j + 7, bv1); SB; mma(af1, 2, bv0); SB;
      if (4 * j + 8 < TK / 2) read_b(4 * j + 8, bv0);
      SB; mma(af1, 3, bv1); SB;
    }
#undef SB
    if (ch + 1 < nch) store_chunk(buf ^ 1);
    __syncthreads();
  }

  if (a.w2_slabs) {
    wgrad_slab_store<NI, NJ>(a.w2_slabs + ((size_t)(blockIdx.z * gridDim.y + blockIdx.y) * gridDim.x +
                                           blockIdx.x) * (MB * NBT), acc, tid);
    return;
  }
#pragma unroll
  for (int j = 0; j < NJ; ++j) {
    const int cc = wn * (NBT / 2) + 32 * j + l31;
    const int cv = cv0 + cc / U;
    const int u = cc % U;
    const int n = cv / S, r = cv % S;
    const int k = S * u + r;
    if (cv >= a.Cv || k >= a.K) continue;
#pragma unroll
    for (int i = 0; i < NI; ++i)
#pragma unroll
      for (int e = 0; e < 16; ++e) {
        const int m = m0 + wm * (MB / 2) + 32 * i + (e & 3) + 8 * (e >> 2) + 4 * h;
        if (m < a.M) atomicAdd(a.dw + ((size_t)m * a.N + n) * a.K + k, acc[i][j][e]);
      }
  }
}

template <int U, int RB, int NN, bool LO_ID, bool HI_ID>
__global__ __launch_bounds__(256, RB >= 4 ? 1 : 2) void wgrad_edge_kernel(const WgradArgs a, int spw) {
  constexpr int S = 32 / U;
  constexpr int MB = RB <= 2 ? 64 : 128;
  constexpr int NIW = MB / 64;
  constexpr int NBLK = RB * NN;
  extern __shared__ __attribute__((aligned(16))) float red[];
  const int tid = threadIdx.x, lane = tid & 63;
  const int wave = __builtin_amdgcn_readfirstlane(tid >> 6);
  const int l31 = lane & 31, h = lane >> 5;
  const int k = S * (l31 % U) + l31 / U;
  const int Ls = a.Ls, Lhi = a.Lhi;
  const int spb = Ls >> 5;
  const int nsteps = a.B * spb;
  constexpr int DEPTH = RB * NN >= 4 ? 1 : 2;
  const int wg_beg = min(nsteps, (int)blockIdx.z * 4 * spw), wg_end = min(nsteps, wg_beg + 4 * spw);
  const int cnt = wg_end - wg_beg > wave ? (wg_end - wg_beg - wave + 3) / 4 : 0;

  f32x16 acc[RB][NN];
#pragma unroll
  for (int i = 0; i < RB; ++i)
#pragma unroll
    for (int j = 0; j < NN; ++j)
#pragma unroll
      for (int e = 0; e < 16; ++e) acc[i][j][e] = 0.0f;

  bool rok[RB];
  ChanXf axf[RB];
#pragma unroll
  for (int i = 0; i < RB; ++i) {
    const int m = 32 * i + l31;
    rok[i] = m < a.M;
    if (!LO_ID) axf[i] = segan_chan_xf(a.lo, rok[i] ? m : 0);
  }
  const int lrow = lane >> 3, lpc = lane & 7;
  int crow[RB][4];
  bool cs1[RB][4];
#pragma unroll
  for (int i = 0; i < RB; ++i)
#pragma unroll
    for (int q = 0; q < 4; ++q) {
      int m = 32 * i + 8 * q + lrow;
      m = m < a.M ? m : 0;
      cs1[i][q] = m >= a.lo.C0;
      crow[i][q] = (cs1[i][q] ? m - a.lo.C0 : m) * Ls;
    }
  const bool rows_full = (a.M & 31) == 0;
  bool hs1[NN];
  int hn[NN];
  ChanXf bxf[NN];
#pragma unroll
  for (int j = 0; j < NN; ++j) {
    const int n = j < a.N ? j : 0;
    hs1[j] = n >= a.hi.C0;
    hn[j] = hs1[j] ? n - a.hi.C0 : n;
    if (!HI_ID) bxf[j] = segan_chan_xf(a.hi, n);
  }

  constexpr int XWIN = 32 * S + 32, XL = (XWIN + 63) / 64;
  constexpr int WLDS = NN * XL * 64 + RB * 1024;
  float* win = red + wave * WLDS;
  float* atile = win + NN * XL * 64;
  struct Regs {
    f32x4 A[RB][4];
    float X[NN][XL];
    unsigned xok;
  };
  auto load = [&](Regs& R, int st) {
    const int b = st / spb;
    const int t0 = (st - b * spb) << 5;
    const float* sb0 = a.lo.p0 + (size_t)b * a.lo.C0 * Ls + t0 + 4 * lpc;
    const float* sb1 = a.lo.p1 + (size_t)b * a.lo.C1 * Ls + t0 + 4 * lpc;
#pragma unroll
    for (int i = 0; i < RB; ++i)
#pragma unroll
      for (int q = 0; q < 4; ++q)
        R.A[i][q] = *reinterpret_cast<const f32x4*>((cs1[i][q] ? sb1 : sb0) + crow[i][q]);
    R.xok = 0u;
    int off[XL];
#pragma unroll
    for (int e = 0; e < XL; ++e) {
      const int pw = lane + 64 * e;
      const int idx = segan_hi_index(S * t0 + pw, Lhi, a.padL, a.mode, a.roll);
      const bool ok = pw < XWIN && idx >= 0;
      if (ok) R.xok |= 1u << e;
      off[e] = ok ? idx : 0;
    }
#pragma unroll
    for (int j = 0; j < NN; ++j) {
      const float* q = hs1[j] ? a.hi.p1 + ((size_t)b * a.hi.C1 + hn[j]) * Lhi
                              : a.hi.p0 + ((size_t)b * a.hi.C0 + hn[j]) * Lhi;
#pragma unroll
      for (int e = 0; e < XL; ++e) R.X[j][e] = q[off[e]];
    }
  };
  auto compute = [&](Regs& R) {
#pragma unroll
    for (int i = 0; i < RB; ++i)
#pragma unroll
      for (int q = 0; q < 4; ++q)
        *reinterpret_cast<f32x4*>(atile + (32 * i + 8 * q + lrow) * 32 + 4 * (lpc ^ lrow)) = R.A[i][q];
    f32x4 Af[RB][4];
#pragma unroll
    for (int i = 0; i < RB; ++i)
#pragma unroll
      for (int q = 0; q < 4; ++q)
        Af[i][q] = *reinterpret_cast<const f32x4*>(atile + (32 * i + l31) * 32 + 4 * ((4 * h + q) ^ (l31 & 7)));
    if (!LO_ID || !rows_full) {
#pragma unroll
      for (int i = 0; i < RB; ++i)
#pragma unroll
        for (int q = 0; q < 4; ++q)
#pragma unroll
          for (int e = 0; e < 4; ++e) {
            float v = Af[i][q][e];
            if (!LO_ID) v = segan_apply_xf(axf[i], v);
            Af[i][q][e] = rok[i] ? v : 0.0f;
          }
    }
#pragma unroll
    for (int j = 0; j < NN; ++j)
#pragma unroll
      for (int e = 0; e < XL; ++e) {
        float v = R.X[j][e];
        if (!HI_ID) v = segan_apply_xf(bxf[j], v);
        win[j * (XL * 64) + lane + 64 * e] = ((R.xok >> e) & 1u) ? v : 0.0f;
      }
    float Bv[NN][16];
#pragma unroll
    for (int j = 0; j < NN; ++j)
#pragma unroll
      for (int s2 = 0; s2 < 16; ++s2) Bv[j][s2] = win[j * (XL * 64) + S * (16 * h + s2) + k];
#pragma unroll
    for (int s2 = 0; s2 < 16; ++s2)
#pragma unroll
      for (int i = 0; i < RB; ++i)
#pragma unroll
        for (int j = 0; j < NN; ++j)
          acc[i][j] = __builtin_amdgcn_mfma_f32_32x32x2f32(Af[i][s2 >> 2][s2 & 3], Bv[j][s2],
                                                           acc[i][j], 0, 0, 0);
  };

  if (cnt > 0) {
    auto stp = [&](int i) { return wg_beg + 4 * min(i, cnt - 1) + wave; };
    if (DEPTH == 1) {
      Regs R0, R1;
      load(R0, stp(0));
      for (int i = 0; i < cnt; i += 2) {
        load(R1, stp(i + 1));
        compute(R0);
        load(R0, stp(i + 2));
        if (i + 1 < cnt) compute(R1);
      }
    } else {
      Regs R0, R1, R2;
      load(R0, stp(0));
      load(R1, stp(1));
      for (int i = 0; i < cnt; i += 3) {
        load(R2, stp(i + 2));
        compute(R0);
        load(R0, stp(i + 3));
        if (i + 1 < cnt) compute(R1);
        load(R1, stp(i + 4));
        if (i + 2 < cnt) compute(R2);
      }
    }
  }

  __syncthreads();
#pragma unroll
  for (int i = 0; i < RB; ++i)
#pragma unroll
    for (int j = 0; j < NN; ++j)
#pragma unroll
      for (int e = 0; e < 16; ++e) red[((wave * NBLK + i * NN + j) * 16 + e) * 64 + lane] = acc[i][j][e];
  __syncthreads();
  const int wm = wave >> 1, wn = wave & 1;
  f32x16 out[NIW][1];
#pragma unroll
  for (int ii = 0; ii < NIW; ++ii) {
    const int rb = wm * NIW + ii;
#pragma unroll
    for (int e = 0; e < 16; ++e) {
      float sum = 0.0f;
      if (rb < RB && wn < NN) {
#pragma unroll
        for (int w = 0; w < 4; ++w) sum += red[((w * NBLK + rb * NN + wn) * 16 + e) * 64 + lane];
      }
      out[ii][0][e] = sum;
    }
  }
  if (a.w2_slabs) {
    wgrad_slab_store<NIW, 1>(a.w2_slabs + (size_t)blockIdx.z * (MB * 64), out, tid);
    return;
  }
  const int cc = wn * 32 + l31;
  const int cv = cc / U, u = cc % U;
  const int n = cv / S, r = cv % S;
  const int kk = S * u + r;
  if (cv >= a.Cv || kk >= a.K) return;
#pragma unroll
  for (int ii = 0; ii < NIW; ++ii)
#pragma unroll
    for (int e = 0; e < 16; ++e) {
      const int m = wm * (MB / 2) + 32 * ii + (e & 3) + 8 * (e >> 2) + 4 * h;
      if (m < a.M) atomicAdd(a.dw + ((size_t)m * a.N + n) * a.K + kk, out[ii][0][e]);
    }
}

#define WG2_TK 32
#define WG2_NLD 4

template <int U, bool XF, int MB = 128>
__global__ __launch_bounds__(256, 2) void wgrad2_kernel(const WgradArgs a) {
  constexpr int S = 32 / U;
  constexpr int TK = WG2_TK;
  constexpr int NBT = 128;
  constexpr int CVW = NBT / U;
  constexpr int WM = MB >= 64 ? 2 : 1, WN = 4 / WM;
  constexpr int NI = MB / (32 * WM), NJ = NBT / (32 * WN);
  constexpr int NLD = WG2_NLD;
  constexpr int NDMA = MB / 32;
  static_assert(CVW / S == 4, "one real hi channel per wave");
  static_assert(MB == 128 || MB == 64 || MB == 32, "block rows");

  extern __shared__ __attribute__((aligned(16))) float smem[];
  const int RLw = a.RLw;
  float* Al0 = smem;
  float* Bl0 = Al0 + 2 * MB * TK;

  const int tid = threadIdx.x;
  const int lane = tid & 63;
  const int wave = __builtin_amdgcn_readfirstlane(tid >> 6);
  const int wm = wave / WN, wn = wave % WN;
  const int l31 = lane & 31, h = lane >> 5;

  const int cv0 = blockIdx.x * CVW;
  const int m0 = blockIdx.y * MB;
  const int ch_beg = blockIdx.z * a.w2_cps;
  const int ch_end = min(ch_beg + a.w2_cps, a.w2_nch);
  if (ch_beg >= ch_end) return;
  const int Ls = a.Ls;
  const int cpsm = a.w2_cpsample;
  const int spc = a.w2_spc;

  const int b_first = cpsm ? ch_beg / cpsm : ch_beg * spc;
  int tq = cpsm ? ch_beg - b_first * cpsm : 0;
  int brel = 0;

  const long lo_left = (long)(a.B - b_first) * a.M * Ls * 4;
  const __amdgpu_buffer_rsrc_t lor = __builtin_amdgcn_make_buffer_rsrc(
      const_cast<float*>(a.lo.p0) + (size_t)b_first * a.M * Ls, 0,
// ... 326 lines not shown
    if (a.M <= 64) return launch_wgrad2<U, XF, 64>(a, st, deterministic, slabs, slab_floats_avail);
  }
  return launch_wgrad2<U, XF, 128>(a, st, deterministic, slabs, slab_floats_avail);
}

template <int U, bool LO_ID, bool HI_ID, int MB, int NBT>
static int launch_wgrad_tile(WgradArgs& a, hipStream_t st, float* slabs, size_t slab_floats) {
  constexpr int CVW = NBT / U;
  constexpr int TK = 32;
  int NS;
  if (a.Ls >= TK) NS = (a.Ls % TK == 0) ? 1 : 2;
  else NS = (TK % a.Ls == 0) ? TK / a.Ls : (TK + a.Ls - 2) / a.Ls + 1;
  a.H = U - 1;
  a.RLw = TK + NS * a.H;
  a.RLw += (8 - a.RLw % 32 + 32) % 32;
  if (a.RLw > 256 || a.Ls % 4 != 0) {
    segan_set_error("wgrad: low-rate length %d unsupported for stride %d (needs a multiple of 4, "
                    "and >= %d)", a.Ls, 32 / U, U / 2);
    return SEGAN_EUNSUPPORTED;
  }
  if ((long)a.B * a.M * a.Ls >= (1L << 31) || (long)a.B * a.N * a.Lhi >= (1L << 31)) {
    segan_set_error("wgrad: operand exceeds the 2^31 element indexing limit");
    return SEGAN_EUNSUPPORTED;
  }
  if (int e = segan_src_defaults(&a.lo, st, "wgrad(lo)")) return e;
  if (int e = segan_src_defaults(&a.hi, st, "wgrad(hi)")) return e;
  a.ls_magic = (65536 + a.Ls - 1) / a.Ls;
  a.per_magic = (65536 + a.Ls + a.H - 1) / (a.Ls + a.H);
  const int ncol = ceil_div(a.Cv, CVW);
  const int nrow = ceil_div(a.M, MB);
  const int tiles = ncol * nrow;
  const int chunks = ceil_div(a.Ctot, TK);
  int nsplit = ceil_div(1536, tiles);
  if (nsplit > chunks / 4) nsplit = chunks / 4;
  if (nsplit < 1) nsplit = 1;
  const int chunks_per = ceil_div(chunks, nsplit);
  nsplit = ceil_div(chunks, chunks_per);
  a.cols_per_split = chunks_per * TK;
  const size_t lds = (size_t)(2 * MB * (TK + 4) + 2 * CVW * a.RLw) * sizeof(float);
  auto kern = wgrad_kernel<U, TK, LO_ID, HI_ID, MB, NBT>;
  static bool attr_done[16];
  const int d = wg_cur_device();
  if (!attr_done[d]) {
    (void)hipFuncSetAttribute(reinterpret_cast<const void*>(kern),
                              hipFuncAttributeMaxDynamicSharedMemorySize, 160 * 1024);
    attr_done[d] = true;
  }
  a.w2_slabs = nullptr;
  if (nsplit == 1) slabs = nullptr;
  if (slabs) {
    if (slab_floats < (size_t)tiles * nsplit * MB * NBT) {
      segan_set_error("wgrad: deterministic mode needs %zu bytes of scratch for the partial tiles",
                      (size_t)tiles * nsplit * MB * NBT * sizeof(float));
      return SEGAN_EINVAL;
    }
    a.w2_slabs = slabs;
  }
  g_last_wgrad[0] = 1; g_last_wgrad[1] = tiles; g_last_wgrad[2] = nsplit; g_last_wgrad[3] = chunks_per;
  g_last_wgrad[4] = 0; g_last_wgrad[5] = 0;
  hipLaunchKernelGGL(kern, dim3(ncol, nrow, nsplit), dim3(256), lds, st, a);
  if (int e = segan_check_launch("wgrad_kernel")) return e;
  if (slabs) {
    int zstep = 1;
    if (nsplit >= 128 && tiles <= 8) {
      zstep = 32;
      hipLaunchKernelGGL((wgrad_group_kernel<MB, NBT>), dim3(ncol, nrow, ceil_div(nsplit, zstep)),
                         dim3(256), 0, st, slabs, nsplit, zstep);
      if (int e = segan_check_launch("wgrad_group_kernel")) return e;
    }
    hipLaunchKernelGGL((wgrad_reduce_kernel<U, MB, NBT>), dim3(ncol, nrow), dim3(256), 0, st, a, nsplit,
                       zstep);
    return segan_check_launch("wgrad_reduce_kernel");
  }
  return SEGAN_OK;
}

static bool wgrad_edge_geometry_ok(const WgradArgs& a, int U) {
  if (a.Cv > 64 / U || a.N > 2) return false;
  if (a.Ls % 32 != 0) return false;
  if (a.M > 128 || (a.M > 64 && a.N > 1)) return false;
  return true;
}

template <int U, int RB, int NN, bool LO_ID, bool HI_ID>
static int launch_wgrad_edge_tile(WgradArgs& a, hipStream_t st, float* slabs, size_t slab_floats) {
  constexpr int MB = RB <= 2 ? 64 : 128;
  if ((long)a.B * a.M * a.Ls >= (1L << 31) || (long)a.B * a.N * a.Lhi >= (1L << 31)) {
    segan_set_error("wgrad: operand exceeds the 2^31 element indexing limit");
    return SEGAN_EUNSUPPORTED;
  }
  if (int e = segan_src_defaults(&a.lo, st, "wgrad(lo)")) return e;
  if (int e = segan_src_defaults(&a.hi, st, "wgrad(hi)")) return e;
  const int nsteps = a.B * (a.Ls / 32);
  constexpr int OCC = RB >= 4 ? 1 : 2;
  int nwg = ceil_div(nsteps, 4 * 8);
  if (nwg > 256 * OCC) nwg = 256 * OCC;
  const int spw = ceil_div(nsteps, 4 * nwg);
  nwg = ceil_div(nsteps, 4 * spw);
  a.w2_slabs = nullptr;
  if (nwg == 1) slabs = nullptr;
  if (slabs) {
    if (slab_floats < (size_t)nwg * MB * 64) {
      segan_set_error("wgrad: deterministic mode needs %zu bytes of scratch for the partial tiles",
                      (size_t)nwg * MB * 64 * sizeof(float));
      return SEGAN_EINVAL;
    }
    a.w2_slabs = slabs;
  }
  g_last_wgrad[0] = 4; g_last_wgrad[1] = 1; g_last_wgrad[2] = nwg; g_last_wgrad[3] = spw;
  g_last_wgrad[4] = 0; g_last_wgrad[5] = 0;
  constexpr int XL = (32 * (32 / U) + 32 + 63) / 64;
  const size_t lds_red = (size_t)4 * RB * NN * 1024 * sizeof(float);
  const size_t lds_win = (size_t)4 * (NN * XL * 64 + RB * 1024) * sizeof(float);
  const size_t lds = lds_red > lds_win ? lds_red : lds_win;
  auto kern = wgrad_edge_kernel<U, RB, NN, LO_ID, HI_ID>;
  static bool attr_done[16];
  const int d = wg_cur_device();
  if (!attr_done[d]) {
    (void)hipFuncSetAttribute(reinterpret_cast<const void*>(kern),
                              hipFuncAttributeMaxDynamicSharedMemorySize, 160 * 1024);
    attr_done[d] = true;
  }
  hipLaunchKernelGGL(kern, dim3(1, 1, nwg), dim3(256), lds, st, a, spw);
  if (int e = segan_check_launch("wgrad_edge_kernel")) return e;
  if (slabs) {
    int zstep = 1;
    if (nwg >= 128) {
      zstep = 32;
      hipLaunchKernelGGL((wgrad_group_kernel<MB, 64>), dim3(1, 1, ceil_div(nwg, zstep)), dim3(256), 0,
                         st, slabs, nwg, zstep);
      if (int e = segan_check_launch("wgrad_group_kernel")) return e;
    }
    hipLaunchKernelGGL((wgrad_reduce_kernel<U, MB, 64>), dim3(1, 1), dim3(256), 0, st, a, nwg, zstep);
    return segan_check_launch("wgrad_reduce_kernel");
  }
  return SEGAN_OK;
}

template <int U, bool LO_ID, bool HI_ID>
static int launch_wgrad_edge(WgradArgs& a, hipStream_t st, float* slabs, size_t slab_floats) {
  if (a.N == 1) {
    if (a.M <= 32) return launch_wgrad_edge_tile<U, 1, 1, LO_ID, HI_ID>(a, st, slabs, slab_floats);
    if (a.M <= 64) return launch_wgrad_edge_tile<U, 2, 1, LO_ID, HI_ID>(a, st, slabs, slab_floats);
    return launch_wgrad_edge_tile<U, 4, 1, LO_ID, HI_ID>(a, st, slabs, slab_floats);
  }
  if (a.M <= 32) return launch_wgrad_edge_tile<U, 1, 2, LO_ID, HI_ID>(a, st, slabs, slab_floats);
  return launch_wgrad_edge_tile<U, 2, 2, LO_ID, HI_ID>(a, st, slabs, slab_floats);
}

template <int U, bool LO_ID, bool HI_ID>
static int launch_wgrad_x(WgradArgs& a, hipStream_t st, float* slabs, size_t slab_floats) {
  static const bool edge_on = getenv("SEGAN_WGRAD_EDGE") == nullptr || atoi(getenv("SEGAN_WGRAD_EDGE")) != 0;
  if (edge_on && wgrad_edge_geometry_ok(a, U)) return launch_wgrad_edge<U, LO_ID, HI_ID>(a, st, slabs, slab_floats);
  if (a.Cv <= 64 / U) {
    if (a.M <= 64) return launch_wgrad_tile<U, LO_ID, HI_ID, 64, 64>(a, st, slabs, slab_floats);
    return launch_wgrad_tile<U, LO_ID, HI_ID, 128, 64>(a, st, slabs, slab_floats);
  }
  return launch_wgrad_tile<U, LO_ID, HI_ID, 128, 128>(a, st, slabs, slab_floats);
}

template <int U>
static int launch_wgrad_t(WgradArgs& a, hipStream_t st, float* slabs, size_t slab_floats) {
  const bool lo_id = !a.lo.scale && !a.lo.shift && !a.lo.slope;
  const bool hi_id = !a.hi.scale && !a.hi.shift && !a.hi.slope;
  if (lo_id && hi_id) return launch_wgrad_x<U, true, true>(a, st, slabs, slab_floats);
  if (lo_id) return launch_wgrad_x<U, true, false>(a, st, slabs, slab_floats);
  if (hi_id) return launch_wgrad_x<U, false, true>(a, st, slabs, slab_floats);
  return launch_wgrad_x<U, false, false>(a, st, slabs, slab_floats);
}

template <int U>
static int launch_wgrad_fp32(WgradArgs& a, hipStream_t st, bool deterministic, float* scratch,
                             size_t scratch_floats) {
  float* slabs = nullptr;
  size_t slab_floats = 0;
  const size_t lo_floats = (size_t)a.B * a.M * a.Ls;
  const bool lo_plain = !a.lo.scale && !a.lo.shift && !a.lo.slope && a.lo.C1 == 0;
  bool fast = wgrad2_geometry_ok(a, U);
  if (fast && !lo_plain && (scratch == nullptr || scratch_floats < lo_floats)) fast = false;
  size_t used = (fast && !lo_plain) ? lo_floats : 0;
  if (deterministic) {
    if (scratch == nullptr) {
      segan_set_error("wgrad: deterministic mode needs scratch (segan_wgrad_scratch_bytes)");
      return SEGAN_EINVAL;
    }
    slabs = scratch + used;
    slab_floats = scratch_floats - used;
  }
  if (fast) {
    if (!lo_plain) {
      if (int e = segan_src_defaults(&a.lo, st, "wgrad(lo)")) return e;
      const bool xf = true;
      const long total = (long)lo_floats / 4;
      const unsigned grid = (unsigned)(total / 256 > 8192 ? 8192 : (total + 255) / 256);
      hipLaunchKernelGGL(wgrad_lo_materialize_kernel, dim3(grid), dim3(256), 0, st, a.lo, scratch,
                         a.B, a.M, a.Ls / 4, xf ? 1 : 0);
      if (int e = segan_check_launch("wgrad_lo_materialize_kernel")) return e;
      a.lo.p0 = scratch; a.lo.p1 = nullptr; a.lo.C0 = a.M; a.lo.C1 = 0;
      a.lo.scale = a.lo.shift = a.lo.slope = nullptr;
    }
    const bool hi_xf = a.hi.scale || a.hi.shift || a.hi.slope;
    if (hi_xf) {
      if (int e = segan_src_defaults(&a.hi, st, "wgrad(hi)")) return e;
    }
    const int rc = hi_xf ? launch_wgrad2_rows<U, true>(a, st, deterministic, slabs, slab_floats)
                         : launch_wgrad2_rows<U, false>(a, st, deterministic, slabs, slab_floats);
    if (rc != SEGAN_EUNSUPPORTED) return rc;
  }
  return launch_wgrad_t<U>(a, st, slabs, slab_floats);
}

extern "C" size_t segan_wgrad_scratch_bytes(int B, int M, int N, int Ls, int S, int precision,
                                            int flags) {
  if (B <= 0 || M <= 0 || N <= 0 || Ls <= 0 || !stride_ok(S)) return 0;
  if (precision != SEGAN_PREC_FP32) {
    const int planes = precision == SEGAN_PREC_BF16 ? 1 : 3;
    return segan_wgrad_bf2_scratch_bytes(B, M, N, Ls, S, planes);
  }
  size_t bytes = (size_t)B * M * Ls * sizeof(float);
  if (flags & SEGAN_WGRAD_DETERMINISTIC) {
    const int U = 32 / S;
    const size_t tiles = (size_t)ceil_div(N * S, 128 / U) * ceil_div(M, 128);
    bytes += (tiles > 4096 ? tiles : 4096) * 128 * 128 * sizeof(float);
  }
  return bytes;
}

extern "C" int segan_wgrad(const segan_src* lo, const segan_src* hi, float* dw, int B, int M, int N,
                           int Ls, int K, int S, int padL, int mode, int roll, int precision,
                           int flags, void* scratch, size_t scratch_bytes, void* stream) {
  SEGAN_REQUIRE(precision_ok(precision), "wgrad: bad precision %d", precision);
  SEGAN_REQUIRE(stride_ok(S), "wgrad: stride %d not in {1,2,4}", S);
  SEGAN_REQUIRE(K >= 1 && K <= 32, "wgrad: kernel width %d not in [1,32]", K);
  SEGAN_REQUIRE(B > 0 && N > 0 && M > 0 && Ls > 0, "wgrad: bad sizes");
  SEGAN_REQUIRE(dw != nullptr, "wgrad: dw is NULL");
  SEGAN_REQUIRE(mode == SEGAN_PAD_REFLECT || mode == SEGAN_PAD_ZERO, "wgrad: bad pad mode");
  if (int e = check_src(lo, M, "wgrad(lo)")) return e;
  if (int e = check_src(hi, N, "wgrad(hi)")) return e;
  const int L = S * Ls;
  SEGAN_REQUIRE(roll > -L && roll < L, "wgrad: |roll| must be < L");
  WgradArgs a = {};
  a.lo = *lo; a.hi = *hi; a.dw = dw;
  a.B = B; a.M = M; a.N = N; a.K = K; a.Ls = Ls; a.Lhi = L;
  a.Cv = N * S; a.padL = padL; a.mode = mode; a.roll = roll;
  a.Ctot = B * Ls;
  hipStream_t st = (hipStream_t)stream;
  if (precision != SEGAN_PREC_FP32) {
    const int planes = precision == SEGAN_PREC_BF16 ? 1 : 3;
    WgradArgs a2 = a;
    return segan_wgrad_bf2(a2, 32 / S, planes, scratch, scratch_bytes, st);
  }
  const bool det = (flags & SEGAN_WGRAD_DETERMINISTIC) != 0;
  float* sc = (float*)scratch;
  const size_t scf = scratch ? scratch_bytes / sizeof(float) : 0;
  switch (S) {
    case 4: return launch_wgrad_fp32<8>(a, st, det, sc, scf);
    case 2: return launch_wgrad_fp32<16>(a, st, det, sc, scf);
    default: return launch_wgrad_fp32<32>(a, st, det, sc, scf);
  }
}
```

### segan_pytorch_amd/distributed.py

```python
import os
import time

import torch
import torch.distributed as dist

from . import ops


def is_dist():
    return dist.is_available() and dist.is_initialized() and dist.get_world_size() > 1


def world_size():
    return dist.get_world_size() if (dist.is_available() and dist.is_initialized()) else 1


def _collectives_on():
    if not (dist.is_available() and dist.is_initialized()):
        return False
    return dist.get_world_size() > 1 or os.environ.get('SEGAN_DP_SINGLE') == '1'


def rank():
    return dist.get_rank() if (dist.is_available() and dist.is_initialized()) else 0
# ... 374 lines not shown
def drop_reducer(optimizer):
    global _active
    r = _reducers.pop(id(optimizer), None)
    if r is not None and _active is r:
        _active = None


def arm(optimizer, passes=1):
    global _active
    if not _collectives_on():
        return
    _active = _reducer(optimizer)
    _active.arm(passes)


def grad_ready(*params):
    if _active is None:
        return
    for p in params:
        if p is not None:
            _active.ready(p)


def allreduce_grads(optimizer):
    global _active
    if not _collectives_on():
        return
    r = _reducer(optimizer)
    if _active is not None and _active is not r:
        _active.armed = False
    r.finish()
    _active = None


def broadcast_params(module, src=0):
    if not _collectives_on():
        return
    with torch.no_grad():
        for t in list(module.parameters()) + list(module.buffers()):
            if _native_cur is not None and t.is_cuda and t.dtype == torch.float32 and t.is_contiguous():
                _native_cur.broadcast(t.data, src)
            else:
                dist.broadcast(t.data, src)
    ops.bump_weights_epoch()


def broadcast_scalar(value, src=0, device=None):
    if not is_dist():
        return float(value)
    if device is None or dist.get_backend() != 'nccl':
        device = torch.device('cpu') if dist.get_backend() != 'nccl' else \
            torch.device('cuda', torch.cuda.current_device())
    t = torch.tensor([float(value)], dtype=torch.float64, device=device)
    dist.broadcast(t, src)
    return float(t.item())


def shard_batch(t, dim=0):
    ws, rk = world_size(), rank()
    if ws <= 1:
        return t
    n = t.shape[dim]
    if n % ws != 0:
        raise ValueError('global batch {} is not divisible by world size {}'.format(n, ws))
    per = n // ws
    return t.narrow(dim, rk * per, per)


def sync_bn_enabled():
    return _collectives_on() and os.environ.get("SEGAN_SYNC_BN", "0") == "1"


def bn_stats_sync(x, gamma, beta, eps, momentum, running_mean, running_var):
    ws = ops.bn_partial(x)
    if _native_cur is not None:
        allp = _native_cur.allgather(ws).view(-1, ws.shape[1], 3)
    else:
        parts = [torch.empty_like(ws) for _ in range(world_size())]
        dist.all_gather(parts, ws)
        allp = torch.cat(parts, 0).contiguous()
    return ops.bn_final(allp, gamma, beta, eps, momentum, running_mean, running_var)


def act_bwd_bn_sync(a, dh, slope, bn, dslope=None, dgamma=None, dbeta=None, dbias=None):
    totals, ws = ops.act_bwd_bn_reduce(a, dh, slope, bn, dslope, dgamma, dbeta)
    if _native_cur is not None:
        _native_cur.allreduce(totals, 1.0)
    else:
        dist.all_reduce(totals, op=dist.ReduceOp.SUM)
    count = float(a.shape[0]) * float(a.shape[2]) * world_size()
    return ops.act_bwd_bn_apply(a, dh, slope, bn, totals, count, dbias, ws)
```

### segan_pytorch_amd/functional.py

```python
import os

import torch

from . import ops
from .ops import ACT_NONE, ACT_TANH, PAD_REFLECT, PAD_ZERO, Src


def grad_buf(p):
    if p.grad is None:
        p.grad = torch.zeros_like(p, memory_format=torch.contiguous_format)
    elif not p.grad.is_contiguous():
        p.grad = p.grad.contiguous()
    return p.grad


def _gb(p, needed=True):
    if p is None or not needed or not p.requires_grad:
        return None
    return grad_buf(p)


def _bn_batch_stats(bn, training):
    return training or bn.running_mean is None or bn.running_var is None


def _bn_train_stats(c, bn, training=True):
    from . import distributed as sdist
    fn = sdist.bn_stats_sync if sdist.sync_bn_enabled() else ops.bn_stats
    track = training and bn.running_mean is not None and bn.running_var is not None
    momentum = 0.0
    if track:
        if bn.num_batches_tracked is not None:
            bn.num_batches_tracked += 1
        if bn.momentum is not None:
            momentum = bn.momentum
        else:
            momentum = 1.0 / float(bn.num_batches_tracked) if bn.num_batches_tracked is not None else 0.0
    return fn(c, bn.weight, bn.bias, bn.eps, momentum, bn.running_mean if track else None,
              bn.running_var if track else None)


def _bn_eval_affine(bn):
    rstd = torch.rsqrt(bn.running_var + bn.eps)
    gamma = bn.weight.detach() if bn.weight is not None else torch.ones_like(rstd)
    beta = bn.bias.detach() if bn.bias is not None else torch.zeros_like(rstd)
    scale = (gamma * rstd).contiguous()
    shift = (beta - bn.running_mean * scale).contiguous()
    return scale, shift, rstd.contiguous()


def _eval_bn_act_bwd(c, bn, scale, shift, rstd, dh, slope, dslope, y_tanh=None, dbias=None):
    if y_tanh is not None:
        g = ops.tanh_bwd(y_tanh, dh, dbias=_gb(bn.bias))
    else:
        v = ops.affine_prelu(c, scale, shift, None)
        g = ops.act_bwd(v, dh, slope=slope, dslope=dslope, dbias=_gb(bn.bias))
    if bn.weight is not None and bn.weight.requires_grad:
        xhat = ops.affine_prelu(c, rstd, (-bn.running_mean * rstd).contiguous(), None)
        grad_buf(bn.weight).add_((g * xhat).sum((0, 2)))
    dc = ops.affine_prelu(g, scale, None, None)
    if dbias is not None:
        ops.act_bwd(dc, dc, dbias=dbias)
    return dc


def _act_bwd_bn(a, dh, slope, bn, dslope, dgamma, dbeta, dbias):
    from . import distributed as sdist
    if sdist.sync_bn_enabled():
        return sdist.act_bwd_bn_sync(a, dh, slope, bn, dslope, dgamma, dbeta, dbias)
    return ops.act_bwd(a, dh, slope=slope, bn=bn, dslope=dslope, dgamma=dgamma, dbeta=dbeta,
                       dbias=dbias)


_WGRAD_OVERLAP = os.environ.get('SEGAN_WGRAD_OVERLAP', '0') == '1'
_side_streams = {}


class _SideStream(object):

    def __init__(self, *tensors):
        flat = []
        for t in tensors:
            if isinstance(t, Src):
                flat.extend((t.t0, t.t1, t.scale, t.shift, t.slope))
            else:
                flat.append(t)
        self.tensors = [t for t in flat if torch.is_tensor(t) and t.is_cuda]
        self.on = _WGRAD_OVERLAP and bool(self.tensors)

    def __enter__(self):
        if not self.on:
            return self
        dev = self.tensors[0].device
        main = torch.cuda.current_stream(dev)
        key = (dev.index, main.cuda_stream)
        side = _side_streams.get(key)
        if side is None:
            side = _side_streams[key] = torch.cuda.Stream(device=dev)
        side.wait_stream(main)
        self.side = side
        self.ctx = torch.cuda.stream(side)
        self.ctx.__enter__()
        return self

    def __exit__(self, *exc):
        if not self.on:
            return False
        self.ctx.__exit__(*exc)
        for t in self.tensors:
            t.record_stream(self.side)
        return False


def _join_side(ref):
    if not _WGRAD_OVERLAP or ref is None or not ref.is_cuda:
        return
    main = torch.cuda.current_stream(ref.device)
    side = _side_streams.get((ref.device.index, main.cuda_stream))
    if side is not None:
        main.wait_stream(side)


def _ready(*mods_or_params):
    from . import distributed as sdist
    if sdist._active is None:
        return
    ps = []
    for m in mods_or_params:
        if m is None:
            continue
        if isinstance(m, torch.nn.Module):
            ps.extend(torch.nn.Module.parameters(m))
        else:
            ps.append(m)
    sdist.grad_ready(*ps)


def _ones(n, ref):
    return torch.ones(n, device=ref.device, dtype=torch.float32)


def _cat(a, b):
    return torch.cat((a.detach().reshape(-1), b.detach().reshape(-1)))


import itertools as _it

_sn_epoch = _it.count(1 << 40)


def _is_sn(mod):
    return hasattr(mod, 'weight_orig')


# ... 381 lines not shown
            head = (hf, y1, a1, y2, a2, y3)
        else:
            if pt == 'conv':
                pc = ops.conv1d_fwd(Src(h), W.get(disc.pool_conv), disc.pool_conv.bias, 1,
                                    pad_mode=PAD_ZERO, padL=0, pack=disc._pool_pack)
                hp, idx = pc.view(B, -1), None
                extra['avg_conv_h'] = hp
            else:
                hp, idx = ops.pool_time_fwd(h, 'max' if pt == 'gmax' else 'avg')
            y3 = ops.linear_fwd(hp, W.get(fc))
            out = ops.bias_prelu_rows(y3, fc.bias, None)
            head = (h, hp, idx, y3)
        ctx.disc = disc
        ctx.rolls = tuple(rolls)
        ctx.x_needs = x.requires_grad or (x1 is not None and x1.requires_grad)
        ctx.split = None if x1 is None else (x.shape[1], x.requires_grad, x1.requires_grad)
        ctx.state = (cs, srcs, bns, head, W)
        disc._last_fwd = (cs, xfs)
        disc._last_extra = extra
        disc._last_head = head
        return out

    @staticmethod
    def backward(ctx, dout):
        disc = ctx.disc
        cs, srcs, bns, head, W = ctx.state
        blocks = list(disc.enc_blocks)
        fc = disc.fc
        dout = dout.contiguous()
        def lin_wgrad(mod, dy, xin):
            if W.needs_grad(mod):
                gw = W.grad_target(mod)
                ops.linear_wgrad(dy, xin, gw)
                W.finish(mod, gw)

        def prelu_bwd(y, lin, act, dact):
            gs = W.grad_target(act) if W.needs_grad(act) else None
            d = ops.bias_prelu_rows_bwd(y, lin.bias, W.get(act), dact, gs, _gb(lin.bias))
            if gs is not None:
                W.finish(act, gs)
            return d

        if disc.pool_type == 'none':
            hf, y1, a1, y2, a2, y3 = head
            dy3 = ops.bias_prelu_rows_bwd(y3, fc[4].bias, None, dout, None, _gb(fc[4].bias))
            lin_wgrad(fc[4], dy3, a2)
            da2 = ops.linear_dgrad(dy3, W.get(fc[4]))
            dy2 = prelu_bwd(y2, fc[2], fc[3], da2)
            lin_wgrad(fc[2], dy2, a1)
            da1 = ops.linear_dgrad(dy2, W.get(fc[2]))
            dy1 = prelu_bwd(y1, fc[0], fc[1], da1)
            lin_wgrad(fc[0], dy1, hf)
            dh = ops.linear_dgrad(dy1, W.get(fc[0])).view(cs[-1].shape)
            _ready(fc)
        else:
            h, hp, idx, y3 = head
            Lh = h.shape[2]
            dy3 = ops.bias_prelu_rows_bwd(y3, fc.bias, None, dout, None, _gb(fc.bias))
            lin_wgrad(fc, dy3, hp)
            dhp = ops.linear_dgrad(dy3, W.get(fc))
            if disc.pool_type == 'conv':
                pcm = disc.pool_conv
                dpc = dhp.view(h.shape[0], 1, Lh)
                if pcm.bias is not None and pcm.bias.requires_grad:
                    ops.act_bwd(dpc, dpc, dbias=grad_buf(pcm.bias))
                if W.needs_grad(pcm):
                    gw = W.grad_target(pcm)
                    ops.wgrad(Src(dpc), Src(h), gw, 1, 1, 0, PAD_ZERO)
                    W.finish(pcm, gw)
                dh = ops.conv1d_dgrad(dpc, W.get(pcm), Lh, 1, padL=0, pack=disc._pool_pack)
                _ready(fc, pcm)
            else:
                dh = ops.pool_time_bwd(dhp, idx, Lh, 'max' if disc.pool_type == 'gmax' else 'avg')
                _ready(fc)
        dx = None
        for l in range(len(blocks) - 1, -1, -1):
            blk = blocks[l]
            w = W.get(blk.conv)
            K, S = blk.kwidth, blk.stride
            bn = bns[l]
            if bn == 'eval':
                raise RuntimeError('Discriminator backward in eval() mode with BatchNorm is not '
                                   'supported; call .train() (the reference never does this)')
            if bn is not None:
                dc = _act_bwd_bn(cs[l], dh, blk.act.weight, bn, _gb(blk.act.weight), _gb(bn[2]),
                                 _gb(bn[3]), _gb(blk.conv.bias))
            else:
                dc = ops.act_bwd(cs[l], dh, slope=blk.act.weight, dslope=_gb(blk.act.weight),
                                 dbias=_gb(blk.conv.bias))
            padL = ops.conv_pad(K, S)[0]
            with _SideStream(dc, srcs[l]):
                if W.needs_grad(blk.conv):
                    gw = W.grad_target(blk.conv)
                    ops.wgrad(Src(dc), srcs[l], gw, K, S, padL, PAD_REFLECT, roll=ctx.rolls[l])
                    W.finish(blk.conv, gw)
                _ready(blk)
            if l > 0:
                dh = ops.conv1d_dgrad(dc, w, srcs[l].L, S, roll=ctx.rolls[l], pack=blk._pack)
            elif ctx.x_needs:
                dx = ops.conv1d_dgrad(dc, w, srcs[l].L, S, roll=ctx.rolls[l], pack=blk._pack)
        _join_side(dout)
        ctx.state = None
        dx1 = None
        if dx is not None and ctx.split is not None:
            c0, need0, need1 = ctx.split
            dx1 = dx[:, c0:].contiguous() if need1 else None
            dx = dx[:, :c0].contiguous() if need0 else None
        return (None, None, dx, dx1) + (None,) * (len(ctx.needs_input_grad) - 4)


class ConvBlockFn(torch.autograd.Function):

    @staticmethod
    def forward(ctx, blk, x, *params):
        x = x.contiguous()
        src = Src(x)
        W = _Weights()
        c = ops.conv1d_fwd(src, W.get(blk.conv), blk.conv.bias, blk.stride, pack=blk._pack)
        bn_saved = None
        scale = shift = None
        if blk.norm is not None:
            bn = blk.norm
            if _bn_batch_stats(bn, blk.training):
                mean, rstd, scale, shift = _bn_train_stats(c, bn, blk.training)
                bn_saved = (mean, rstd, bn.weight, bn.bias)
            else:
                scale, shift, rstd = _bn_eval_affine(bn)
                bn_saved = ('eval', scale, shift, rstd)
        h = ops.affine_prelu(c, scale, shift, blk.act.weight)
        a = c if blk.norm is None else ops.affine_prelu(c, scale, shift, None)
        ctx.blk = blk
        ctx.set_materialize_grads(False)
        ctx.x_needs = x.requires_grad
        ctx.state = (src, c, bn_saved, W)
        return h, a

    @staticmethod
    def backward(ctx, dh, da_lin):
        blk = ctx.blk
        src, c, bn, W = ctx.state
        K, S = blk.kwidth, blk.stride
        w = W.get(blk.conv)
        if dh is None and da_lin is None:
            return (None,) * len(ctx.needs_input_grad)
        dh = dh.contiguous() if dh is not None else None
        if bn is None:
            lin = da_lin.contiguous() if da_lin is not None else None
            dc = ops.act_bwd(c, dh, dskip=lin, slope=blk.act.weight,
                             alpha=_ones(c.shape[1], c) if lin is not None else None,
                             dslope=_gb(blk.act.weight), dbias=_gb(blk.conv.bias))
        else:
            if da_lin is not None or dh is None:
                raise RuntimeError('gradient through the linear output of a normalised '
                                   'GConv1DBlock is unsupported')
            if isinstance(bn[0], str):
                dc = _eval_bn_act_bwd(c, blk.norm, bn[1], bn[2], bn[3], dh, blk.act.weight,
                                      _gb(blk.act.weight), dbias=_gb(blk.conv.bias))
            else:
                dc = _act_bwd_bn(c, dh, blk.act.weight, bn, _gb(blk.act.weight), _gb(bn[2]), _gb(bn[3]),
                                 _gb(blk.conv.bias))
        padL = ops.conv_pad(K, S)[0]
        if W.needs_grad(blk.conv):
            gw = W.grad_target(blk.conv)
            ops.wgrad(Src(dc), src, gw, K, S, padL, PAD_REFLECT)
            W.finish(blk.conv, gw)
        dx = ops.conv1d_dgrad(dc, w, src.L, S, pack=blk._pack) if ctx.x_needs else None
        ctx.state = None
        return (None, dx) + (None,) * (len(ctx.needs_input_grad) - 2)


class DeconvBlockFn(torch.autograd.Function):

    @staticmethod
    def forward(ctx, blk, x, *params):
        x = x.contiguous()
# ... 152 lines not shown
```

### segan_pytorch_amd/ops.py

```python
import ctypes
import operator

import torch

from . import _lib
from . import layout
from ._lib import ACT_NONE, ACT_TANH, PAD_REFLECT, PAD_ZERO, SeganSrc, check


import os as _os

PREC_FP32, PREC_BF16, PREC_BF16X3 = 0, 1, 3
_PREC_NAMES = {'fp32': PREC_FP32, 'bf16': PREC_BF16, 'bf16x3': PREC_BF16X3}
_precision = _PREC_NAMES[_os.environ.get('SEGAN_PRECISION', 'fp32')]
_EUNSUPPORTED = -3


_deterministic = _os.environ.get('SEGAN_DETERMINISTIC', '0') == '1'


def set_deterministic(on):
    global _deterministic
    _deterministic = bool(on)


def get_deterministic():
    return _deterministic


_ACC_NAMES = ('plain', 'blocked')
_accumulation = _os.environ.get('SEGAN_ACCUMULATION', 'plain')
if _accumulation not in _ACC_NAMES:
    raise ValueError('SEGAN_ACCUMULATION must be one of {}'.format(_ACC_NAMES))
PREC_FP32_BLOCKED = 4


def set_accumulation(mode):
    global _accumulation
    if mode not in _ACC_NAMES:
        raise ValueError('accumulation must be one of {}'.format(_ACC_NAMES))
    _accumulation = mode


def get_accumulation():
    return _accumulation


def _fp32():
    return PREC_FP32_BLOCKED if _accumulation == 'blocked' else PREC_FP32


def set_precision(mode):
    global _precision
    if mode not in _PREC_NAMES:
        raise ValueError('precision must be one of {}'.format(sorted(_PREC_NAMES)))
    _precision = _PREC_NAMES[mode]


def get_precision():
    return [k for k, v in _PREC_NAMES.items() if v == _precision][0]


def _stream():
    return ctypes.c_void_p(torch._C._cuda_getCurrentRawStream(torch._C._cuda_getDevice()))


def _ptr(t):
    if t is None:
        return None
    return ctypes.c_void_p(t.data_ptr())


def _chk(t, name, ndim=None):
    if not isinstance(t, torch.Tensor):
        raise TypeError('{} must be a tensor, got {}'.format(name, type(t)))
    if not t.is_cuda:
        raise RuntimeError(
            '{} is on {}: segan_pytorch_amd runs only on an MI355X (HIP) device; '
            'there is no CPU path'.format(name, t.device))
    if t.dtype != torch.float32:
        raise TypeError('{} must be float32, got {}'.format(name, t.dtype))
    if not t.is_contiguous():
        raise ValueError('{} must be contiguous'.format(name))
    if ndim is not None and t.dim() != ndim:
        raise ValueError('{} must have {} dims, got {}'.format(name, ndim, tuple(t.shape)))
    return t


class Src(object):

# ... 231 lines not shown
    if padL is None:
        padL = conv_pad(K, S)[0]
    small = N <= 2
    _chk(w, 'weight', 3)
    pack = pack or WeightPack()
    if not small and not _precision and short_rows_ok(N, M, L, S):
        return conv1d_dgrad_short(da, w, L, S, roll=roll, padL=padL, pack=pack)
    dx = torch.empty((B, N, L), device=da.device, dtype=torch.float32)
    halo = torch.empty((B * N * max(K - 1, 1),), device=da.device, dtype=torch.float32)
    lib = _lib.load()
    if small:
        check(lib.segan_conv1d_dgrad(_ptr(da), None, _ptr(w.detach()), _ptr(dx), _ptr(halo), B, N,
                                     M, L, K, S, padL, roll, PREC_FP32, None, 0, _stream()),
              'conv1d_dgrad')
        return dx
    if _precision:
        keep, sp, sn = _bf_scratch(1, B, N, M, L, K, S, padL, da.device)
        rc = lib.segan_conv1d_dgrad(_ptr(da), _ptr(pack.bf(w, S, 0, 1, _precision)), None, _ptr(dx),
                                    _ptr(halo), B, N, M, L, K, S, padL, roll, _precision, sp, sn,
                                    _stream())
        if rc != _EUNSUPPORTED:
            check(rc, 'conv1d_dgrad')
            return dx
    if short_rows_ok(N, M, L, S):
        return conv1d_dgrad_short(da, w, L, S, roll=roll, padL=padL, pack=pack)
    check(lib.segan_conv1d_dgrad(_ptr(da), _ptr(pack.t(w, S, 0)), None, _ptr(dx), _ptr(halo), B, N,
                                 M, L, K, S, padL, roll, _fp32(), *_scratch(), _stream()),
          'conv1d_dgrad')
    return dx


def conv1d_dgrad_short(da, w, L, S, roll=0, padL=None, pack=None):
    _chk(da, 'da', 3)
    _chk(w, 'weight', 3)
    M, N, K = w.shape
    B = da.shape[0]
    if padL is None:
        padL = conv_pad(K, S)[0]
    dx = torch.empty((B, N, L), device=da.device, dtype=torch.float32)
    pack = pack or WeightPack()
    check(_lib.load().segan_conv1d_dgrad_short(_ptr(da), _ptr(pack.g(w, S)), _ptr(dx), B, N,
                                               M, L, K, S, padL, roll, _stream()),
          'conv1d_dgrad_short')
    return dx


_SHORT_LS = (4, 8, 16, 32, 64)


def short_rows_ok(N, M, L, S):
    return S in (2, 4) and L % S == 0 and (L // S) in _SHORT_LS and N % 4 == 0 and M % 16 == 0


def wgrad(lo, hi, dw, K, S, padL, pad_mode, roll=0):
    _chk(dw, 'dw', 3)
    M, N = lo.C, hi.C
    if tuple(dw.shape) != (M, N, K):
        raise ValueError('wgrad: dw {} != ({}, {}, {})'.format(tuple(dw.shape), M, N, K))
    if lo.B != hi.B or lo.L * S != hi.L:
        raise ValueError('wgrad: lo [{}x{}] / hi [{}x{}] inconsistent for stride {}'.format(
            lo.B, lo.L, hi.B, hi.L, S))
    cl, ch = lo.c_struct(), hi.c_struct()
    lib = _lib.load()
    if _precision != PREC_FP32:
        nbytes = lib.segan_wgrad_scratch_bytes(lo.B, M, N, lo.L, S, _precision, 0)
        scratch = _stream_scratch(nbytes, dw.device)
        rc = lib.segan_wgrad(ctypes.byref(cl), ctypes.byref(ch), _ptr(dw), lo.B, M, N, lo.L, K, S,
                             padL, pad_mode, roll, _precision, 0,
                             ctypes.c_void_p(scratch.data_ptr()) if scratch is not None else None,
                             nbytes if scratch is not None else 0, _stream())
        if rc != -3:
            check(rc, 'wgrad')
            return
    flags = 1 if _deterministic else 0
    lo_plain = lo.t1 is None and lo.scale is None and lo.shift is None and lo.slope is None
    scratch, nbytes = None, 0
    if flags or not lo_plain:
        nbytes = lib.segan_wgrad_scratch_bytes(lo.B, M, N, lo.L, S, PREC_FP32, flags)
        scratch = _stream_scratch(nbytes, dw.device)
    check(lib.segan_wgrad(ctypes.byref(cl), ctypes.byref(ch), _ptr(dw), lo.B, M, N, lo.L, K, S, padL,
                          pad_mode, roll, PREC_FP32, flags,
                          ctypes.c_void_p(scratch.data_ptr()) if scratch is not None else None, nbytes,
                          _stream()), 'wgrad')


def deconv1d_fwd(src, w, bias, S, act=ACT_NONE, pack=None):
    M, N, K = w.shape
    if src.C != M:
        raise ValueError('deconv1d_fwd: input has {} channels, weight expects {}'.format(src.C, M))
    pad = deconv_pad(K, S)
    B, Ls = src.B, src.L
    y = torch.empty((B, N, S * Ls), device=w.device, dtype=torch.float32)
    cs = src.c_struct()
    small = N <= 2
    _chk(w, 'weight', 3)
    pack = pack or WeightPack()
    lib = _lib.load()
    if small:
        check(lib.segan_deconv1d_fwd(ctypes.byref(cs), None, _ptr(w.detach()), _ptr(bias), _ptr(y),
                                     B, M, N, Ls, K, S, pad, act, PREC_FP32, None, 0, _stream()),
              'deconv1d_fwd')
        return y
    if _precision and act == ACT_NONE:
        keep, sp, sn = _bf_scratch(2, B, N, M, S * Ls, K, S, pad, w.device)
        rc = lib.segan_deconv1d_fwd(ctypes.byref(cs), _ptr(pack.bf(w, S, pad, 1, _precision)), None,
                                    _ptr(bias), _ptr(y), B, M, N, Ls, K, S, pad, act, _precision,
                                    sp, sn, _stream())
        if rc != _EUNSUPPORTED:
            check(rc, 'deconv1d_fwd')
            return y
    check(lib.segan_deconv1d_fwd(ctypes.byref(cs), _ptr(pack.t(w, S, pad)), None, _ptr(bias),
                                 _ptr(y), B, M, N, Ls, K, S, pad, act, _fp32(), *_scratch(),
                                 _stream()), 'deconv1d_fwd')
    return y


def deconv1d_dgrad(dy, w, S, M0=0, need0=True, need1=True, pack=None):
    _chk(dy, 'dy', 3)
    M, N, K = w.shape
    B = dy.shape[0]
    if dy.shape[1] != N or dy.shape[2] % S != 0:
        raise ValueError('deconv1d_dgrad: dy {} inconsistent with weight {}'.format(
            tuple(dy.shape), tuple(w.shape)))
    Ls = dy.shape[2] // S
    pad = deconv_pad(K, S)
    dx0 = dx1 = None
    if M0 > 0 and need0:
        dx0 = torch.empty((B, M0, Ls), device=dy.device, dtype=torch.float32)
    if M - M0 > 0 and need1:
        dx1 = torch.empty((B, M - M0, Ls), device=dy.device, dtype=torch.float32)
    if dx0 is None and dx1 is None:
        return None, None
    pack = pack or WeightPack()
    lib = _lib.load()
    if _precision:
        keep, sp, sn = _bf_scratch(3, B, N, M, S * Ls, K, S, pad, dy.device)
        rc = lib.segan_deconv1d_dgrad(_ptr(dy), _ptr(pack.bf(w, S, 0, 0, _precision)), _ptr(dx0),
                                      _ptr(dx1), B, M, M0, N, Ls, K, S, pad, _precision, sp, sn,
                                      _stream())
        if rc != _EUNSUPPORTED:
            check(rc, 'deconv1d_dgrad')
            return dx0, dx1
    check(lib.segan_deconv1d_dgrad(_ptr(dy), _ptr(pack.f(w, S)), _ptr(dx0), _ptr(dx1), B, M, M0, N,
                                   Ls, K, S, pad, _fp32(), *_scratch(), _stream()), 'deconv1d_dgrad')
    return dx0, dx1


def _ws(B, C, L, per_split, extra, device):
    ns = _lib.load().segan_bn_nsplit(B, C, L)
    return torch.empty((per_split * ns * C + extra * C,), device=device, dtype=torch.float32)


def bn_stats(x, gamma, beta, eps, momentum, running_mean, running_var):
    _chk(x, 'x', 3)
    B, C, L = x.shape
    mean = torch.empty(C, device=x.device, dtype=torch.float32)
    rstd = torch.empty_like(mean)
    scale = torch.empty_like(mean)
    shift = torch.empty_like(mean)
    ws = _ws(B, C, L, 3, 0, x.device)
    check(_lib.load().segan_bn_stats(_ptr(x), _ptr(gamma), _ptr(beta), eps, momentum,
                                     _ptr(running_mean), _ptr(running_var), _ptr(mean), _ptr(rstd),
                                     _ptr(scale), _ptr(shift), _ptr(ws), B, C, L, _stream()),
          'bn_stats')
    return mean, rstd, scale, shift

# ... 786 lines not shown
```

Before: 3555.

## Fuse BatchNorm/PReLU backward into first discriminator layer's wgrad and dgrad

For the discriminator's first conv layer with BatchNorm, the activation-backward apply step is no longer materialised as a separate gradient tensor. A lazy gradient source (activation, upstream grad, BN stats, reduced totals) is passed straight into the weight-gradient and small-N transposed-conv edge kernels, which compute the PReLU/BN gradient on the fly while loading. This removes one full read-write pass over a large early-layer activation and one kernel launch. The cost is extra per-element arithmetic and an extra input stream in the tsmall kernels, plus fallback paths when the lazy kernels are unsupported.

```diff
diff --git a/include/segan_hip.h b/include/segan_hip.h
--- a/include/segan_hip.h
+++ b/include/segan_hip.h
@@ -108,6 +108,27 @@
                            const float* bn_beta, const float* totals, float* da, float* dbias,
                            float* ws, int B, int C, int L, double count_total, void* stream);
 
+typedef struct segan_grad_src {
+  const float* a;
+  const float* dh;
+  const float* dskip;
+  const float* slope;
+  const float* alpha;
+  const float* bn_mean;
+  const float* bn_rstd;
+  const float* bn_gamma;
+  const float* bn_beta;
+  const float* totals;
+  float inv_count;
+} segan_grad_src;
+
+int segan_wgrad_lazy(const segan_grad_src* g, const segan_src* hi, float* dw, float* dbias, int B,
+                     int M, int N, int Ls, int K, int S, int padL, int mode, int roll, int precision,
+                     int flags, void* scratch, size_t scratch_bytes, void* stream);
+int segan_conv1d_dgrad_lazy(const segan_grad_src* g, const float* w, float* dx, float* halo, int B,
+                            int N, int M, int L, int K, int S, int padL, int roll, int precision,
+                            void* stream);
+
 int segan_tanh_bwd(const float* y, const float* dy, const float* clean, float l1_scale, float* da,
                    float* dbias, float* ws, int B, int C, int L, void* stream);
 
diff --git a/segan_pytorch_amd/_lib.py b/segan_pytorch_amd/_lib.py
--- a/segan_pytorch_amd/_lib.py
+++ b/segan_pytorch_amd/_lib.py
@@ -17,8 +17,16 @@
                 ('scale', c_void_p), ('shift', c_void_p), ('slope', c_void_p)]
 
 
+class SeganGradSrc(Structure):
+    _fields_ = [('a', c_void_p), ('dh', c_void_p), ('dskip', c_void_p), ('slope', c_void_p),
+                ('alpha', c_void_p), ('bn_mean', c_void_p), ('bn_rstd', c_void_p),
+                ('bn_gamma', c_void_p), ('bn_beta', c_void_p), ('totals', c_void_p),
+                ('inv_count', c_float)]
+
+
 _P = c_void_p
 _SRC = POINTER(SeganSrc)
+_GSRC = POINTER(SeganGradSrc)
 
 SIGNATURES = {
     'segan_abi_version': (c_int, []),
@@ -39,6 +47,8 @@
                                    c_int, c_int, _P, c_size_t, _P]),
     'segan_wgrad': (c_int, [_SRC, _SRC, _P, c_int, c_int, c_int, c_int, c_int, c_int, c_int, c_int,
                             c_int, c_int, c_int, _P, c_size_t, _P]),
+    'segan_wgrad_lazy': (c_int, [_GSRC, _SRC, _P, _P] + [c_int] * 11 + [_P, c_size_t, _P]),
+    'segan_conv1d_dgrad_lazy': (c_int, [_GSRC, _P, _P, _P] + [c_int] * 9 + [_P]),
     'segan_wgrad_scratch_bytes': (c_size_t, [c_int, c_int, c_int, c_int, c_int, c_int, c_int]),
     'segan_deconv1d_fwd': (c_int, [_SRC, _P, _P, _P, _P, c_int, c_int, c_int, c_int, c_int, c_int, c_int,
                                    c_int, c_int, _P, c_size_t, _P]),
diff --git a/segan_pytorch_amd/csrc/segan_common.h b/segan_pytorch_amd/csrc/segan_common.h
--- a/segan_pytorch_amd/csrc/segan_common.h
+++ b/segan_pytorch_amd/csrc/segan_common.h
@@ -83,6 +83,49 @@
 
 int segan_src_defaults(segan_src* s, hipStream_t st, const char* what);
 
+__device__ __forceinline__ void bn_affine(float gamma, float beta, float mean, float rstd,
+                                          float& scale, float& shift) {
+  scale = gamma * rstd;
+  shift = fmaf(-mean, scale, beta);
+}
+
+struct GradXf {
+  float sc, sh, sl;
+  float mu, rs;
+  float dbm, dgm;
+  float al;
+};
+
+__device__ __forceinline__ GradXf segan_grad_xf(const segan_grad_src& g, int c) {
+  GradXf x;
+  x.sl = g.slope ? g.slope[c] : 1.0f;
+  x.al = g.alpha ? g.alpha[c] : 0.0f;
+  x.mu = 0.f; x.rs = 1.f; x.sc = 1.f; x.sh = 0.f; x.dbm = 0.f; x.dgm = 0.f;
+  if (g.bn_mean) {
+    x.mu = g.bn_mean[c];
+    x.rs = g.bn_rstd[c];
+    bn_affine(g.bn_gamma ? g.bn_gamma[c] : 1.0f, g.bn_beta ? g.bn_beta[c] : 0.0f, x.mu, x.rs, x.sc, x.sh);
+    x.dbm = g.totals[2 * c] * g.inv_count;
+    x.dgm = g.totals[2 * c + 1] * g.inv_count;
+  }
+  return x;
+}
+
+template <bool BN>
+__device__ __forceinline__ float segan_grad_value(const GradXf& x, float a, float dh, float ds,
+                                                  bool has_skip) {
+#pragma clang fp contract(off)
+  if (BN) {
+    const float v = fmaf(a, x.sc, x.sh);
+    const float xh = (a - x.mu) * x.rs;
+    const float t = fmaf(dh, v > 0.f ? 1.0f : x.sl, -x.dbm);
+    return x.sc * fmaf(-x.dgm, xh, t);
+  }
+  float g = dh * (a > 0.f ? 1.0f : x.sl);
+  if (has_skip) g = fmaf(x.al, ds, g);
+  return g;
+}
+
 __device__ __forceinline__ const float* segan_src_row(const segan_src& s, int b, int n, int L) {
   if (n < s.C0) return s.p0 + ((size_t)b * s.C0 + n) * (size_t)L;
   return s.p1 + ((size_t)b * s.C1 + (n - s.C0)) * (size_t)L;
diff --git a/segan_pytorch_amd/csrc/segan_conv.hip b/segan_pytorch_amd/csrc/segan_conv.hip
--- a/segan_pytorch_amd/csrc/segan_conv.hip
+++ b/segan_pytorch_amd/csrc/segan_conv.hip
@@ -1485,10 +1485,10 @@
   return launch_corr<false, true>(a, U, (hipStream_t)stream);
 }
 
-extern "C" int segan_conv1d_dgrad(const float* da, const void* wt, const float* w, float* dx,
-                                  float* halo, int B, int N, int M, int L, int K, int S, int padL,
-                                  int roll, int precision, void* scratch, size_t scratch_bytes,
-                                  void* stream) {
+static int conv1d_dgrad_impl(const float* da, const void* wt, const float* w, float* dx,
+                             float* halo, int B, int N, int M, int L, int K, int S, int padL,
+                             int roll, int precision, void* scratch, size_t scratch_bytes,
+                             void* stream, const segan_grad_src* lz) {
   const int acc_block = precision == SEGAN_PREC_FP32_BLOCKED;
   if (acc_block) precision = SEGAN_PREC_FP32;
   SEGAN_REQUIRE(precision_ok(precision), "conv1d_dgrad: precision must be 0, 1, 3 or 4");
@@ -1524,7 +1524,7 @@
   set_scratch(a, scratch, scratch_bytes);
   int e;
   if (w && N <= 2) {
-    e = segan_launch_tsmall(a, w, K, M, N, S, 0, st);
+    e = segan_launch_tsmall(a, w, K, M, N, S, 0, st, lz);
   } else if (precision) {
     CorrArgs a2 = a;
     e = segan_corr_bf2_t(a2, U, wt, precision, scratch, scratch_bytes, st);
@@ -1541,6 +1541,29 @@
     return segan_check_launch("fold_halo_kernel");
   }
   return SEGAN_OK;
+}
+
+extern "C" int segan_conv1d_dgrad(const float* da, const void* wt, const float* w, float* dx,
+                                  float* halo, int B, int N, int M, int L, int K, int S, int padL,
+                                  int roll, int precision, void* scratch, size_t scratch_bytes,
+                                  void* stream) {
+  return conv1d_dgrad_impl(da, wt, w, dx, halo, B, N, M, L, K, S, padL, roll, precision, scratch,
+                           scratch_bytes, stream, nullptr);
+}
+
+extern "C" int segan_conv1d_dgrad_lazy(const segan_grad_src* g, const float* w, float* dx, float* halo,
+                                       int B, int N, int M, int L, int K, int S, int padL, int roll,
+                                       int precision, void* stream) {
+  SEGAN_REQUIRE(g && g->a && g->dh && w, "conv1d_dgrad_lazy: NULL pointer");
+  SEGAN_REQUIRE((g->bn_mean == nullptr) == (g->bn_rstd == nullptr), "conv1d_dgrad_lazy: mean/rstd must pair");
+  SEGAN_REQUIRE(!g->bn_mean || g->totals, "conv1d_dgrad_lazy: the BatchNorm kind needs totals");
+  static const bool edge_on = getenv("SEGAN_WGRAD_EDGE") == nullptr || atoi(getenv("SEGAN_WGRAD_EDGE")) != 0;
+  if (precision != SEGAN_PREC_FP32 || N > 2 || !g->bn_mean || g->dskip || !edge_on) {
+    segan_set_error("conv1d_dgrad_lazy: not the direct edge kernels' case (fp32, N <= 2, BatchNorm kind)");
+    return SEGAN_EUNSUPPORTED;
+  }
+  return conv1d_dgrad_impl(g->a, nullptr, w, dx, halo, B, N, M, L, K, S, padL, roll, precision, nullptr,
+                           0, stream, g);
 }
 
 static bool short_ok(int N, int M, int L, int K, int S, int padL) {
diff --git a/segan_pytorch_amd/csrc/segan_conv_edge.hip b/segan_pytorch_amd/csrc/segan_conv_edge.hip
--- a/segan_pytorch_amd/csrc/segan_conv_edge.hip
+++ b/segan_pytorch_amd/csrc/segan_conv_edge.hip
@@ -1,8 +1,8 @@
 #include "segan_conv_shared.h"
 
-template <int S, int N, int PM, int KT>
+template <int S, int N, int PM, int KT, bool LZ = false>
 __global__ __launch_bounds__(256) void tsmall_kernel(const CorrArgs a, const float* __restrict__ w,
-                                                     int Krt, int M) {
+                                                     int Krt, int M, const segan_grad_src lz) {
   const int K = KT ? KT : Krt;
   constexpr int U = 32 / S;
   constexpr int MC = 16;
@@ -23,6 +23,7 @@
   const int o0 = ok0 ? t0 : 0, o1 = ok1 ? t1 : 0;
   const int bo0 = b * a.in.C0 * a.Lin, bo1 = b * a.in.C1 * a.Lin;
   float pv0[MC], pv1[MC];
+  float dv0[LZ ? MC : 1], dv1[LZ ? MC : 1];
   auto load_rows = [&](int mc0) {
 #pragma unroll
     for (int mc = 0; mc < MC; ++mc) {
@@ -32,6 +33,11 @@
                                : a.in.p0 + (size_t)m * a.Lin + bo0;
       pv0[mc] = rowp[o0];
       pv1[mc] = rowp[o1];
+      if (LZ) {
+        const float* rowd = lz.dh + (size_t)m * a.Lin + bo0;
+        dv0[mc] = rowd[o0];
+        dv1[mc] = rowd[o1];
+      }
     }
   };
   load_rows(0);
@@ -39,6 +45,13 @@
 #pragma unroll
     for (int mc = 0; mc < MC; ++mc) {
       const bool mok = mc0 + mc < M;
+      if (LZ) {
+        const GradXf gx = segan_grad_xf(lz, mok ? mc0 + mc : 0);
+        xs[mc][tid] = (mok && ok0) ? segan_grad_value<true>(gx, pv0[mc], dv0[mc], 0.0f, false) : 0.0f;
+        if (tid < U)
+          xs[mc][256 + tid] = (mok && ok1) ? segan_grad_value<true>(gx, pv1[mc], dv1[mc], 0.0f, false) : 0.0f;
+        continue;
+      }
       const ChanXf xf = segan_chan_xf(a.in, mok ? mc0 + mc : 0);
       xs[mc][tid] = (mok && ok0) ? segan_apply_xf(xf, pv0[mc]) : 0.0f;
       if (tid < U) xs[mc][256 + tid] = (mok && ok1) ? segan_apply_xf(xf, pv1[mc]) : 0.0f;
@@ -103,30 +116,39 @@
     }
 }
 
-template <int S, int N, int KT>
+template <int S, int N, int KT, bool LZ>
 static int launch_tsmall_snk(const CorrArgs& a, const float* w, int K, int M, int pad,
-                             hipStream_t st) {
+                             hipStream_t st, const segan_grad_src& lz) {
   dim3 grid(ceil_div(a.Tcols, 256), a.B);
+  if (LZ) {
+    hipLaunchKernelGGL((tsmall_kernel<S, N, 0, KT, LZ>), grid, dim3(256), 0, st, a, w, K, M, lz);
+    return segan_check_launch("tsmall_kernel");
+  }
   switch (pad % S) {
-    case 0: hipLaunchKernelGGL((tsmall_kernel<S, N, 0, KT>), grid, dim3(256), 0, st, a, w, K, M); break;
-    case 1: hipLaunchKernelGGL((tsmall_kernel<S, N, 1 % S, KT>), grid, dim3(256), 0, st, a, w, K, M); break;
-    case 2: hipLaunchKernelGGL((tsmall_kernel<S, N, 2 % S, KT>), grid, dim3(256), 0, st, a, w, K, M); break;
-    default: hipLaunchKernelGGL((tsmall_kernel<S, N, 3 % S, KT>), grid, dim3(256), 0, st, a, w, K, M); break;
+    case 0: hipLaunchKernelGGL((tsmall_kernel<S, N, 0, KT, LZ>), grid, dim3(256), 0, st, a, w, K, M, lz); break;
+    case 1: hipLaunchKernelGGL((tsmall_kernel<S, N, 1 % S, KT, false>), grid, dim3(256), 0, st, a, w, K, M, lz); break;
+    case 2: hipLaunchKernelGGL((tsmall_kernel<S, N, 2 % S, KT, false>), grid, dim3(256), 0, st, a, w, K, M, lz); break;
+    default: hipLaunchKernelGGL((tsmall_kernel<S, N, 3 % S, KT, false>), grid, dim3(256), 0, st, a, w, K, M, lz); break;
   }
   return segan_check_launch("tsmall_kernel");
 }
 
 template <int S, int N>
 static int launch_tsmall_sn(const CorrArgs& a, const float* w, int K, int M, int pad,
-                            hipStream_t st) {
-  if (K == 31) return launch_tsmall_snk<S, N, 31>(a, w, K, M, pad, st);
-  return launch_tsmall_snk<S, N, 0>(a, w, K, M, pad, st);
-}
-
-
-template <int N, int PM>
+                            hipStream_t st, const segan_grad_src* lz) {
+  if (lz) {
+    if (K == 31) return launch_tsmall_snk<S, N, 31, true>(a, w, K, M, 0, st, *lz);
+    return launch_tsmall_snk<S, N, 0, true>(a, w, K, M, 0, st, *lz);
+  }
+  const segan_grad_src none = {};
+  if (K == 31) return launch_tsmall_snk<S, N, 31, false>(a, w, K, M, pad, st, none);
+  return launch_tsmall_snk<S, N, 0, false>(a, w, K, M, pad, st, none);
+}
+
+
+template <int N, int PM, bool LZ = false>
 __global__ __launch_bounds__(256) void tsmall4_kernel(const CorrArgs a, const float* __restrict__ w,
-                                                      int M) {
+                                                      int M, const segan_grad_src lz) {
   constexpr int S = 4, U = 8, KT = 31, Q = 4;
   constexpr int MC = 8;
   constexpr int TWQ = Q * 256 + 12;
@@ -154,6 +176,7 @@
   }
   const int bo0 = b * a.in.C0 * a.Lin, bo1 = b * a.in.C1 * a.Lin;
   float pv[MC][5];
+  float dv[LZ ? MC : 1][5];
   auto load_rows = [&](int mc0) {
 #pragma unroll
     for (int mc = 0; mc < MC; ++mc) {
@@ -163,6 +186,11 @@
                                : a.in.p0 + (size_t)m * a.Lin + bo0;
 #pragma unroll
       for (int i = 0; i < 5; ++i) pv[mc][i] = rowp[so[i]];
+      if (LZ) {
+        const float* rowd = lz.dh + (size_t)m * a.Lin + bo0;
+#pragma unroll
+        for (int i = 0; i < 5; ++i) dv[mc][i] = rowd[so[i]];
+      }
     }
   };
   load_rows(0);
@@ -170,6 +198,17 @@
 #pragma unroll
     for (int mc = 0; mc < MC; ++mc) {
       const bool mok = mc0 + mc < M;
+      if (LZ) {
+        const GradXf gx = segan_grad_xf(lz, mok ? mc0 + mc : 0);
+#pragma unroll
+        for (int i = 0; i < 4; ++i)
+          xs[mc][tid + 256 * i] = (mok && ((sok >> i) & 1u))
+                                      ? segan_grad_value<true>(gx, pv[mc][i], dv[mc][i], 0.0f, false) : 0.0f;
+        if (tid < 12)
+          xs[mc][1024 + tid] = (mok && ((sok >> 4) & 1u))
+                                   ? segan_grad_value<true>(gx, pv[mc][4], dv[mc][4], 0.0f, false) : 0.0f;
+        continue;
+      }
       const ChanXf xf = segan_chan_xf(a.in, mok ? mc0 + mc : 0);
 #pragma unroll
       for (int i = 0; i < 4; ++i)
@@ -270,30 +309,40 @@
 }
 
 template <int N>
-static int launch_tsmall4(const CorrArgs& a, const float* w, int M, int pad, hipStream_t st) {
+static int launch_tsmall4(const CorrArgs& a, const float* w, int M, int pad, hipStream_t st,
+                          const segan_grad_src* lz) {
   dim3 grid(ceil_div(a.Tcols, 1024), a.B);
+  if (lz) {
+    hipLaunchKernelGGL((tsmall4_kernel<N, 0, true>), grid, dim3(256), 0, st, a, w, M, *lz);
+    return segan_check_launch("tsmall4_kernel");
+  }
+  const segan_grad_src none = {};
   switch (pad % 4) {
-    case 0: hipLaunchKernelGGL((tsmall4_kernel<N, 0>), grid, dim3(256), 0, st, a, w, M); break;
-    case 1: hipLaunchKernelGGL((tsmall4_kernel<N, 1>), grid, dim3(256), 0, st, a, w, M); break;
-    case 2: hipLaunchKernelGGL((tsmall4_kernel<N, 2>), grid, dim3(256), 0, st, a, w, M); break;
-    default: hipLaunchKernelGGL((tsmall4_kernel<N, 3>), grid, dim3(256), 0, st, a, w, M); break;
+    case 0: hipLaunchKernelGGL((tsmall4_kernel<N, 0>), grid, dim3(256), 0, st, a, w, M, none); break;
+    case 1: hipLaunchKernelGGL((tsmall4_kernel<N, 1>), grid, dim3(256), 0, st, a, w, M, none); break;
+    case 2: hipLaunchKernelGGL((tsmall4_kernel<N, 2>), grid, dim3(256), 0, st, a, w, M, none); break;
+    default: hipLaunchKernelGGL((tsmall4_kernel<N, 3>), grid, dim3(256), 0, st, a, w, M, none); break;
   }
   return segan_check_launch("tsmall4_kernel");
 }
 
 int segan_launch_tsmall(CorrArgs& a, const float* w, int K, int M, int N, int S, int pad,
-                         hipStream_t st) {
+                         hipStream_t st, const segan_grad_src* lz) {
+  if (lz && pad != 0) {
+    segan_set_error("tsmall: a lazy input needs pad = 0");
+    return SEGAN_EINVAL;
+  }
   if (int e = segan_src_defaults(&a.in, st, "tsmall")) return e;
   if (S == 4 && K == 31 && a.Tcols >= 1024)
-    return N == 1 ? launch_tsmall4<1>(a, w, M, pad, st) : launch_tsmall4<2>(a, w, M, pad, st);
+    return N == 1 ? launch_tsmall4<1>(a, w, M, pad, st, lz) : launch_tsmall4<2>(a, w, M, pad, st, lz);
   if (N == 1) {
-    if (S == 4) return launch_tsmall_sn<4, 1>(a, w, K, M, pad, st);
-    if (S == 2) return launch_tsmall_sn<2, 1>(a, w, K, M, pad, st);
-    return launch_tsmall_sn<1, 1>(a, w, K, M, pad, st);
-  }
-  if (S == 4) return launch_tsmall_sn<4, 2>(a, w, K, M, pad, st);
-  if (S == 2) return launch_tsmall_sn<2, 2>(a, w, K, M, pad, st);
-  return launch_tsmall_sn<1, 2>(a, w, K, M, pad, st);
+    if (S == 4) return launch_tsmall_sn<4, 1>(a, w, K, M, pad, st, lz);
+    if (S == 2) return launch_tsmall_sn<2, 1>(a, w, K, M, pad, st, lz);
+    return launch_tsmall_sn<1, 1>(a, w, K, M, pad, st, lz);
+  }
+  if (S == 4) return launch_tsmall_sn<4, 2>(a, w, K, M, pad, st, lz);
+  if (S == 2) return launch_tsmall_sn<2, 2>(a, w, K, M, pad, st, lz);
+  return launch_tsmall_sn<1, 2>(a, w, K, M, pad, st, lz);
 }
 
 
diff --git a/segan_pytorch_amd/csrc/segan_conv_shared.h b/segan_pytorch_amd/csrc/segan_conv_shared.h
--- a/segan_pytorch_amd/csrc/segan_conv_shared.h
+++ b/segan_pytorch_amd/csrc/segan_conv_shared.h
@@ -129,7 +129,8 @@
   return SEGAN_OK;
 }
 
-int segan_launch_tsmall(CorrArgs& a, const float* w, int K, int M, int N, int S, int pad, hipStream_t st);
+int segan_launch_tsmall(CorrArgs& a, const float* w, int K, int M, int N, int S, int pad, hipStream_t st,
+                        const segan_grad_src* lz = nullptr);
 int segan_launch_fsmall(CorrArgs& a, int M, int N, int S, hipStream_t st);
 
 void segan_note_corr_launch(int kind, unsigned grid, const CorrArgs& a, int ntiles);
diff --git a/segan_pytorch_amd/csrc/segan_pointwise.hip b/segan_pytorch_amd/csrc/segan_pointwise.hip
--- a/segan_pytorch_amd/csrc/segan_pointwise.hip
+++ b/segan_pytorch_amd/csrc/segan_pointwise.hip
@@ -39,13 +39,14 @@
 }
 
 struct ChanRange {
-  int c, b_beg, b_end;
+  int c, split, b_beg, b_end;
 };
-__device__ __forceinline__ ChanRange chan_range(int B, int nsplit) {
+__device__ __forceinline__ ChanRange chan_range(int B, int nsplit, bool rev = false) {
   ChanRange r;
-  r.c = blockIdx.x;
+  r.c = rev ? gridDim.x - 1 - blockIdx.x : blockIdx.x;
+  r.split = rev ? gridDim.y - 1 - blockIdx.y : blockIdx.y;
   const int per = (B + nsplit - 1) / nsplit;
-  r.b_beg = blockIdx.y * per;
+  r.b_beg = r.split * per;
   r.b_end = min(B, r.b_beg + per);
   return r;
 }
@@ -123,12 +124,6 @@
   }
 }
 
-__device__ __forceinline__ void bn_affine(float gamma, float beta, float mean, float rstd,
-                                          float& scale, float& shift) {
-  scale = gamma * rstd;
-  shift = fmaf(-mean, scale, beta);
-}
-
 __global__ void bn_final_kernel(const float* __restrict__ ws, const float* gamma, const float* beta,
                                 float eps, float momentum, float* running_mean, float* running_var,
                                 float* mean_o, float* rstd_o, float* scale_o, float* shift_o, int C,
@@ -300,12 +295,13 @@
   float* ws;
   int B, C, L, nsplit;
   float inv_count;
+  int rev2;
 };
 
 template <int PHASE>
 __global__ void act_bwd_kernel(const ActBwdArgs p) {
   __shared__ float sm[16];
-  const ChanRange cr = chan_range(p.B, p.nsplit);
+  const ChanRange cr = chan_range(p.B, p.nsplit, PHASE == 2 && p.rev2);
   const int c = cr.c;
   const int nb = cr.b_end - cr.b_beg;
   const float sl = p.slope ? p.slope[c] : 1.0f;
@@ -325,29 +321,29 @@
   }
   float r[3] = {0.f, 0.f, 0.f};
   const bool has_skip = p.dskip != nullptr;
+  GradXf gx;
+  gx.sc = sc; gx.sh = sh; gx.sl = sl; gx.mu = mu; gx.rs = rs; gx.dbm = dbeta_m; gx.dgm = dgamma_m;
+  gx.al = al;
   auto elem = [&](float av, float dh, float ds) -> float {
     if (PHASE == 0) {
-      float g = dh * (av > 0.f ? 1.0f : sl);
+      const float g = segan_grad_value<false>(gx, av, dh, ds, has_skip);
       r[0] += dh * (av > 0.f ? 0.0f : av);
-      if (has_skip) {
-        g = fmaf(al, ds, g);
-        r[1] = fmaf(ds, av, r[1]);
-      }
+      if (has_skip) r[1] = fmaf(ds, av, r[1]);
       r[2] += g;
       return g;
+    }
+    if (PHASE == 2) {
+      const float d = segan_grad_value<true>(gx, av, dh, 0.0f, false);
+      r[0] += d;
+      return d;
     }
     const float xh = (av - mu) * rs;
     const float v = fmaf(av, sc, sh);
     const float g = dh * (v > 0.f ? 1.0f : sl);
-    if (PHASE == 1) {
-      r[0] += dh * (v > 0.f ? 0.0f : v);
-      r[1] += g;
-      r[2] = fmaf(g, xh, r[2]);
-      return 0.0f;
-    }
-    const float d = ga * rs * (g - dbeta_m - xh * dgamma_m);
-    r[0] += d;
-    return d;
+    r[0] += dh * (v > 0.f ? 0.0f : v);
+    r[1] += g;
+    r[2] = fmaf(g, xh, r[2]);
+    return 0.0f;
   };
   const size_t base = ((size_t)cr.b_beg * p.C + c) * p.L;
   const size_t sstride = (size_t)p.C * p.L;
@@ -382,7 +378,7 @@
   }
   block_sum<3>(r, sm);
   if (threadIdx.x == 0) {
-    float* w = p.ws + ((size_t)blockIdx.y * p.C + c) * 4;
+    float* w = p.ws + ((size_t)cr.split * p.C + c) * 4;
     w[0] = r[0];
     w[1] = r[1];
     w[2] = r[2];
@@ -415,6 +411,11 @@
   } else {
     if (dbias) dbias[c] += s0;
   }
+}
+
+static int act_bwd_reverse() {
+  static const int on = getenv("SEGAN_ACT_BWD_REVERSE") == nullptr || atoi(getenv("SEGAN_ACT_BWD_REVERSE")) != 0;
+  return on;
 }
 
 extern "C" int segan_act_bwd(const float* a, const float* dh, const float* dskip,
@@ -435,6 +436,7 @@
   p.da = da; p.ws = ws; p.B = B; p.C = C; p.L = L;
   p.nsplit = pw_nsplit(B, C, L);
   p.inv_count = 1.0f / ((float)B * (float)L);
+  p.rev2 = act_bwd_reverse();
   const dim3 grid(C, p.nsplit), fgrid(ceil_div(C, 64));
   if (!bn_mean) {
     hipLaunchKernelGGL(act_bwd_kernel<0>, grid, dim3(PW_THREADS), 0, st, p);
@@ -465,6 +467,7 @@
   p.da = nullptr; p.ws = ws; p.B = B; p.C = C; p.L = L;
   p.nsplit = pw_nsplit(B, C, L);
   p.inv_count = 1.0f / ((float)B * (float)L);
+  p.rev2 = 0;
   hipLaunchKernelGGL(act_bwd_kernel<1>, dim3(C, p.nsplit), dim3(PW_THREADS), 0, st, p);
   hipLaunchKernelGGL(act_bwd_final_kernel<1>, dim3(ceil_div(C, 64)), dim3(64), 0, st, p, dslope,
                      (float*)nullptr, dgamma, dbeta, (float*)nullptr);
@@ -490,6 +493,7 @@
   p.da = da; p.ws = ws; p.B = B; p.C = C; p.L = L;
   p.nsplit = pw_nsplit(B, C, L);
   p.inv_count = (float)(1.0 / count_total);
+  p.rev2 = act_bwd_reverse();
   if (hipMemcpyAsync(ws + (size_t)p.nsplit * C * 4, totals, (size_t)C * 2 * sizeof(float),
                      hipMemcpyDeviceToDevice, st) != hipSuccess) {
     segan_set_error("act_bwd_bn_apply: copy of the totals failed");
diff --git a/segan_pytorch_amd/csrc/segan_wgrad.hip b/segan_pytorch_amd/csrc/segan_wgrad.hip
--- a/segan_pytorch_amd/csrc/segan_wgrad.hip
+++ b/segan_pytorch_amd/csrc/segan_wgrad.hip
@@ -326,8 +326,15 @@
   }
 }
 
-template <int U, int RB, int NN, bool LO_ID, bool HI_ID>
-__global__ __launch_bounds__(256, RB >= 4 ? 1 : 2) void wgrad_edge_kernel(const WgradArgs a, int spw) {
+struct WgradLazyArgs {
+  segan_grad_src g;
+  float* dbias;
+  float* part;
+};
+
+template <int U, int RB, int NN, bool LO_ID, bool HI_ID, bool LZ = false>
+__global__ __launch_bounds__(256, RB >= 4 ? 1 : 2) void wgrad_edge_kernel(const WgradArgs a, int spw,
+                                                                          const WgradLazyArgs lz) {
   constexpr int S = 32 / U;
   constexpr int MB = RB <= 2 ? 64 : 128;
   constexpr int NIW = MB / 64;
@@ -360,6 +367,15 @@
     rok[i] = m < a.M;
     if (!LO_ID) axf[i] = segan_chan_xf(a.lo, rok[i] ? m : 0);
   }
+  GradXf gxf[RB];
+  float bsum[RB];
+  if (LZ) {
+#pragma unroll
+    for (int i = 0; i < RB; ++i) {
+      gxf[i] = segan_grad_xf(lz.g, rok[i] ? 32 * i + l31 : 0);
+      bsum[i] = 0.0f;
+    }
+  }
   const int lrow = lane >> 3, lpc = lane & 7;
   int crow[RB][4];
   bool cs1[RB][4];
@@ -390,6 +406,7 @@
   float* atile = win + NN * XL * 64;
   struct Regs {
     f32x4 A[RB][4];
+    f32x4 D[LZ ? RB : 1][4];
     float X[NN][XL];
     unsigned xok;
   };
@@ -403,6 +420,13 @@
 #pragma unroll
       for (int q = 0; q < 4; ++q)
         R.A[i][q] = *reinterpret_cast<const f32x4*>((cs1[i][q] ? sb1 : sb0) + crow[i][q]);
+    if (LZ) {
+      const float* sd = lz.g.dh + (size_t)b * a.lo.C0 * Ls + t0 + 4 * lpc;
+#pragma unroll
+      for (int i = 0; i < RB; ++i)
+#pragma unroll
+        for (int q = 0; q < 4; ++q) R.D[i][q] = *reinterpret_cast<const f32x4*>(sd + crow[i][q]);
+    }
     R.xok = 0u;
     int off[XL];
 #pragma unroll
@@ -468,6 +492,77 @@
                                                            acc[i][j], 0, 0, 0);
   };
 
+  auto lz_stage = [&](Regs& R, f32x4 (&Af)[RB][4]) {
+    f32x4 Df[RB][4];
+#pragma unroll
+    for (int i = 0; i < RB; ++i)
+#pragma unroll
+      for (int q = 0; q < 4; ++q)
+        *reinterpret_cast<f32x4*>(atile + (32 * i + 8 * q + lrow) * 32 + 4 * (lpc ^ lrow)) = R.A[i][q];
+#pragma unroll
+    for (int i = 0; i < RB; ++i)
+#pragma unroll
+      for (int q = 0; q < 4; ++q)
+        Af[i][q] = *reinterpret_cast<const f32x4*>(atile + (32 * i + l31) * 32 + 4 * ((4 * h + q) ^ (l31 & 7)));
+#pragma unroll
+    for (int i = 0; i < RB; ++i)
+#pragma unroll
+      for (int q = 0; q < 4; ++q)
+        *reinterpret_cast<f32x4*>(atile + (32 * i + 8 * q + lrow) * 32 + 4 * (lpc ^ lrow)) = R.D[i][q];
+#pragma unroll
+    for (int i = 0; i < RB; ++i)
+#pragma unroll
+      for (int q = 0; q < 4; ++q)
+        Df[i][q] = *reinterpret_cast<const f32x4*>(atile + (32 * i + l31) * 32 + 4 * ((4 * h + q) ^ (l31 & 7)));
+#pragma unroll
+    for (int j = 0; j < NN; ++j)
+#pragma unroll
+      for (int e = 0; e < XL; ++e) {
+        float v = R.X[j][e];
+        if (!HI_ID) v = segan_apply_xf(bxf[j], v);
+        win[j * (XL * 64) + lane + 64 * e] = ((R.xok >> e) & 1u) ? v : 0.0f;
+      }
+#pragma unroll
+    for (int i = 0; i < RB; ++i)
+#pragma unroll
+      for (int q = 0; q < 4; ++q)
+#pragma unroll
+        for (int e = 0; e < 4; ++e) {
+          float v = segan_grad_value<true>(gxf[i], Af[i][q][e], Df[i][q][e], 0.0f, false);
+          v = rok[i] ? v : 0.0f;
+          Af[i][q][e] = v;
+          bsum[i] += v;
+        }
+  };
+  auto lz_mma = [&](const f32x4 (&Af)[RB][4]) {
+    float Bv[NN][16];
+#pragma unroll
+    for (int j = 0; j < NN; ++j)
+#pragma unroll
+      for (int s2 = 0; s2 < 16; ++s2) Bv[j][s2] = win[j * (XL * 64) + S * (16 * h + s2) + k];
+#pragma unroll
+    for (int s2 = 0; s2 < 16; ++s2)
+#pragma unroll
+      for (int i = 0; i < RB; ++i)
+#pragma unroll
+        for (int j = 0; j < NN; ++j)
+          acc[i][j] = __builtin_amdgcn_mfma_f32_32x32x2f32(Af[i][s2 >> 2][s2 & 3], Bv[j][s2],
+                                                           acc[i][j], 0, 0, 0);
+  };
+
+  if (LZ) {
+    if (cnt > 0) {
+      auto stp = [&](int i) { return wg_beg + 4 * min(i, cnt - 1) + wave; };
+      f32x4 Af[RB][4];
+      Regs R0;
+      load(R0, stp(0));
+      for (int i = 0; i < cnt; ++i) {
+        lz_stage(R0, Af);
+        load(R0, stp(i + 1));
+        lz_mma(Af);
+      }
+    }
+  } else
   if (cnt > 0) {
     auto stp = [&](int i) { return wg_beg + 4 * min(i, cnt - 1) + wave; };
     if (DEPTH == 1) {
@@ -495,6 +590,22 @@
   }
 
   __syncthreads();
+  if (LZ) {
+#pragma unroll
+    for (int i = 0; i < RB; ++i) {
+      bsum[i] += __shfl_xor(bsum[i], 32, 64);
+      if (h == 0) red[(wave * RB + i) * 32 + l31] = bsum[i];
+    }
+    __syncthreads();
+    if (tid < 32 * RB) {
+      float sum = 0.0f;
+#pragma unroll
+      for (int w = 0; w < 4; ++w) sum += red[w * RB * 32 + tid];
+      if (lz.part) lz.part[(size_t)blockIdx.z * (32 * RB) + tid] = sum;
+      else if (lz.dbias && tid < a.M) atomicAdd(lz.dbias + tid, sum);
+    }
+    __syncthreads();
+  }
 #pragma unroll
   for (int i = 0; i < RB; ++i)
 #pragma unroll
@@ -987,9 +1098,20 @@
   return true;
 }
 
-template <int U, int RB, int NN, bool LO_ID, bool HI_ID>
-static int launch_wgrad_edge_tile(WgradArgs& a, hipStream_t st, float* slabs, size_t slab_floats) {
+__global__ void wgrad_lazy_sums_kernel(const WgradLazyArgs lz, int nwg, int pitch, int M) {
+  const int m = blockIdx.x * blockDim.x + threadIdx.x;
+  if (m >= M) return;
+  float sum = 0.0f;
+  for (int z = 0; z < nwg; ++z) sum += lz.part[(size_t)z * pitch + m];
+  lz.dbias[m] += sum;
+}
+
+template <int U, int RB, int NN, bool LO_ID, bool HI_ID, bool LZ = false>
+static int launch_wgrad_edge_tile(WgradArgs& a, hipStream_t st, float* slabs, size_t slab_floats,
+                                  const WgradLazyArgs* lzp = nullptr) {
   constexpr int MB = RB <= 2 ? 64 : 128;
+  WgradLazyArgs lz = {};
+  if (LZ) lz = *lzp;
   if ((long)a.B * a.M * a.Ls >= (1L << 31) || (long)a.B * a.N * a.Lhi >= (1L << 31)) {
     segan_set_error("wgrad: operand exceeds the 2^31 element indexing limit");
     return SEGAN_EUNSUPPORTED;
@@ -1004,13 +1126,15 @@
   nwg = ceil_div(nsteps, 4 * spw);
   a.w2_slabs = nullptr;
   if (nwg == 1) slabs = nullptr;
+  const size_t part_floats = LZ ? (size_t)nwg * 32 * RB : 0;
   if (slabs) {
-    if (slab_floats < (size_t)nwg * MB * 64) {
+    if (slab_floats < (size_t)nwg * MB * 64 + part_floats) {
       segan_set_error("wgrad: deterministic mode needs %zu bytes of scratch for the partial tiles",
-                      (size_t)nwg * MB * 64 * sizeof(float));
+                      ((size_t)nwg * MB * 64 + part_floats) * sizeof(float));
       return SEGAN_EINVAL;
     }
     a.w2_slabs = slabs;
+    if (LZ) lz.part = slabs + (size_t)nwg * MB * 64;
   }
   g_last_wgrad[0] = 4; g_last_wgrad[1] = 1; g_last_wgrad[2] = nwg; g_last_wgrad[3] = spw;
   g_last_wgrad[4] = 0; g_last_wgrad[5] = 0;
@@ -1018,7 +1142,7 @@
   const size_t lds_red = (size_t)4 * RB * NN * 1024 * sizeof(float);
   const size_t lds_win = (size_t)4 * (NN * XL * 64 + RB * 1024) * sizeof(float);
   const size_t lds = lds_red > lds_win ? lds_red : lds_win;
-  auto kern = wgrad_edge_kernel<U, RB, NN, LO_ID, HI_ID>;
+  auto kern = wgrad_edge_kernel<U, RB, NN, LO_ID, HI_ID, LZ>;
   static bool attr_done[16];
   const int d = wg_cur_device();
   if (!attr_done[d]) {
@@ -1026,8 +1150,13 @@
                               hipFuncAttributeMaxDynamicSharedMemorySize, 160 * 1024);
     attr_done[d] = true;
   }
-  hipLaunchKernelGGL(kern, dim3(1, 1, nwg), dim3(256), lds, st, a, spw);
+  hipLaunchKernelGGL(kern, dim3(1, 1, nwg), dim3(256), lds, st, a, spw, lz);
   if (int e = segan_check_launch("wgrad_edge_kernel")) return e;
+  if (LZ && lz.part && lz.dbias) {
+    hipLaunchKernelGGL(wgrad_lazy_sums_kernel, dim3(ceil_div(a.M, 64)), dim3(64), 0, st, lz, nwg, 32 * RB,
+                       a.M);
+    if (int e = segan_check_launch("wgrad_lazy_sums_kernel")) return e;
+  }
   if (slabs) {
     int zstep = 1;
     if (nwg >= 128) {
@@ -1164,3 +1293,62 @@
     default: return launch_wgrad_fp32<32>(a, st, det, sc, scf);
   }
 }
+
+template <int U>
+static int launch_wgrad_edge_lazy(WgradArgs& a, hipStream_t st, float* slabs, size_t slab_floats,
+                                  const WgradLazyArgs& lz) {
+  if (a.N == 1) {
+    if (a.M <= 32) return launch_wgrad_edge_tile<U, 1, 1, true, true, true>(a, st, slabs, slab_floats, &lz);
+    if (a.M <= 64) return launch_wgrad_edge_tile<U, 2, 1, true, true, true>(a, st, slabs, slab_floats, &lz);
+    return launch_wgrad_edge_tile<U, 4, 1, true, true, true>(a, st, slabs, slab_floats, &lz);
+  }
+  if (a.M <= 32) return launch_wgrad_edge_tile<U, 1, 2, true, true, true>(a, st, slabs, slab_floats, &lz);
+  return launch_wgrad_edge_tile<U, 2, 2, true, true, true>(a, st, slabs, slab_floats, &lz);
+}
+
+extern "C" int segan_wgrad_lazy(const segan_grad_src* g, const segan_src* hi, float* dw, float* dbias,
+                                int B, int M, int N, int Ls, int K, int S, int padL, int mode,
+                                int roll, int precision, int flags, void* scratch,
+                                size_t scratch_bytes, void* stream) {
+  SEGAN_REQUIRE(precision_ok(precision), "wgrad_lazy: bad precision %d", precision);
+  SEGAN_REQUIRE(stride_ok(S), "wgrad_lazy: stride %d not in {1,2,4}", S);
+  SEGAN_REQUIRE(K >= 1 && K <= 32, "wgrad_lazy: kernel width %d not in [1,32]", K);
+  SEGAN_REQUIRE(B > 0 && N > 0 && M > 0 && Ls > 0, "wgrad_lazy: bad sizes");
+  SEGAN_REQUIRE(dw != nullptr, "wgrad_lazy: dw is NULL");
+  SEGAN_REQUIRE(mode == SEGAN_PAD_REFLECT || mode == SEGAN_PAD_ZERO, "wgrad_lazy: bad pad mode");
+  SEGAN_REQUIRE(g && g->a && g->dh, "wgrad_lazy: NULL gradient operand");
+  SEGAN_REQUIRE((g->bn_mean == nullptr) == (g->bn_rstd == nullptr), "wgrad_lazy: mean/rstd must pair");
+  SEGAN_REQUIRE(!g->bn_mean || g->totals, "wgrad_lazy: the BatchNorm kind needs totals");
+  SEGAN_REQUIRE(!(g->dskip && !g->alpha), "wgrad_lazy: dskip needs alpha");
+  SEGAN_REQUIRE(!(g->bn_mean && g->dskip), "wgrad_lazy: BN layers have no skip tap");
+  if (int e = check_src(hi, N, "wgrad_lazy(hi)")) return e;
+  const int L = S * Ls;
+  SEGAN_REQUIRE(roll > -L && roll < L, "wgrad_lazy: |roll| must be < L");
+  WgradArgs a = {};
+  a.lo.p0 = g->a; a.lo.p1 = nullptr; a.lo.C0 = M; a.lo.C1 = 0;
+  a.hi = *hi; a.dw = dw;
+  a.B = B; a.M = M; a.N = N; a.K = K; a.Ls = Ls; a.Lhi = L;
+  a.Cv = N * S; a.padL = padL; a.mode = mode; a.roll = roll;
+  a.Ctot = B * Ls;
+  const int U = 32 / S;
+  static const bool edge_on = getenv("SEGAN_WGRAD_EDGE") == nullptr || atoi(getenv("SEGAN_WGRAD_EDGE")) != 0;
+  if (precision != SEGAN_PREC_FP32 || !edge_on || !wgrad_edge_geometry_ok(a, U) || !g->bn_mean || hi->scale ||
+      hi->shift || hi->slope || (((uintptr_t)g->a | (uintptr_t)g->dh) & 15) != 0) {
+    segan_set_error("wgrad_lazy: not the streaming edge kernel's case (fp32, BatchNorm kind, <= 2 plain hi "
+                    "channels, Ls %% 32 == 0, 16-byte aligned tensors)");
+    return SEGAN_EUNSUPPORTED;
+  }
+  const bool det = (flags & SEGAN_WGRAD_DETERMINISTIC) != 0;
+  SEGAN_REQUIRE(!det || scratch, "wgrad_lazy: deterministic mode needs scratch (segan_wgrad_scratch_bytes)");
+  float* slabs = det ? (float*)scratch : nullptr;
+  const size_t slab_floats = det ? scratch_bytes / sizeof(float) : 0;
+  WgradLazyArgs lz = {};
+  lz.g = *g;
+  lz.dbias = dbias;
+  hipStream_t st = (hipStream_t)stream;
+  switch (S) {
+    case 4: return launch_wgrad_edge_lazy<8>(a, st, slabs, slab_floats, lz);
+    case 2: return launch_wgrad_edge_lazy<16>(a, st, slabs, slab_floats, lz);
+    default: return launch_wgrad_edge_lazy<32>(a, st, slabs, slab_floats, lz);
+  }
+}
diff --git a/segan_pytorch_amd/distributed.py b/segan_pytorch_amd/distributed.py
--- a/segan_pytorch_amd/distributed.py
+++ b/segan_pytorch_amd/distributed.py
@@ -480,11 +480,16 @@
     return ops.bn_final(allp, gamma, beta, eps, momentum, running_mean, running_var)
 
 
-def act_bwd_bn_sync(a, dh, slope, bn, dslope=None, dgamma=None, dbeta=None, dbias=None):
+def act_bwd_bn_reduce_sync(a, dh, slope, bn, dslope=None, dgamma=None, dbeta=None):
     totals, ws = ops.act_bwd_bn_reduce(a, dh, slope, bn, dslope, dgamma, dbeta)
     if _native_cur is not None:
         _native_cur.allreduce(totals, 1.0)
     else:
         dist.all_reduce(totals, op=dist.ReduceOp.SUM)
     count = float(a.shape[0]) * float(a.shape[2]) * world_size()
+    return totals, ws, count
+
+
+def act_bwd_bn_sync(a, dh, slope, bn, dslope=None, dgamma=None, dbeta=None, dbias=None):
+    totals, ws, count = act_bwd_bn_reduce_sync(a, dh, slope, bn, dslope, dgamma, dbeta)
     return ops.act_bwd_bn_apply(a, dh, slope, bn, totals, count, dbias, ws)
diff --git a/segan_pytorch_amd/functional.py b/segan_pytorch_amd/functional.py
--- a/segan_pytorch_amd/functional.py
+++ b/segan_pytorch_amd/functional.py
@@ -70,6 +70,26 @@
         return sdist.act_bwd_bn_sync(a, dh, slope, bn, dslope, dgamma, dbeta, dbias)
     return ops.act_bwd(a, dh, slope=slope, bn=bn, dslope=dslope, dgamma=dgamma, dbeta=dbeta,
                        dbias=dbias)
+
+
+def _act_bwd_bn_reduce(a, dh, slope, bn, dslope, dgamma, dbeta):
+    from . import distributed as sdist
+    if sdist.sync_bn_enabled():
+        return sdist.act_bwd_bn_reduce_sync(a, dh, slope, bn, dslope, dgamma, dbeta)
+    totals, ws = ops.act_bwd_bn_reduce(a, dh, slope, bn, dslope, dgamma, dbeta)
+    return totals, ws, float(a.shape[0]) * float(a.shape[2])
+
+
+_LAZY_EDGE_GRAD = os.environ.get('SEGAN_LAZY_EDGE_GRAD', '1') != '0'
+
+
+def set_lazy_edge_grad(on):
+    global _LAZY_EDGE_GRAD
+    _LAZY_EDGE_GRAD = bool(on)
+
+
+def get_lazy_edge_grad():
+    return _LAZY_EDGE_GRAD
 
 
 _WGRAD_OVERLAP = os.environ.get('SEGAN_WGRAD_OVERLAP', '0') == '1'
@@ -617,15 +637,48 @@
             if bn == 'eval':
                 raise RuntimeError('Discriminator backward in eval() mode with BatchNorm is not '
                                    'supported; call .train() (the reference never does this)')
+            padL = ops.conv_pad(K, S)[0]
+            want_w = W.needs_grad(blk.conv)
+            dbias = _gb(blk.conv.bias)
+            if (l == 0 and bn is not None and _LAZY_EDGE_GRAD and (want_w or ctx.x_needs)
+                    and (want_w or dbias is None)):
+                totals, ws, count = _act_bwd_bn_reduce(cs[l], dh, blk.act.weight, bn,
+                                                       _gb(blk.act.weight), _gb(bn[2]), _gb(bn[3]))
+                g = ops.GradSrc(cs[l], dh, slope=blk.act.weight, bn=bn, totals=totals, count_total=count)
+                w_done = not want_w
+                if want_w:
+                    with _SideStream(srcs[l], *g.tensors()):
+                        gw = W.grad_target(blk.conv)
+                        if ops.wgrad_lazy(g, srcs[l], gw, K, S, padL, PAD_REFLECT, roll=ctx.rolls[l],
+                                          dbias=dbias):
+                            W.finish(blk.conv, gw)
+                            _ready(blk)
+                            w_done = True
+                            dbias = None
+                if ctx.x_needs:
+                    dx = ops.conv1d_dgrad_lazy(g, w, srcs[l].L, S, roll=ctx.rolls[l])
+                if w_done and (dx is not None or not ctx.x_needs):
+                    if not want_w:
+                        _ready(blk)
+                    continue
+                dc = ops.act_bwd_bn_apply(cs[l], dh, blk.act.weight, bn, totals, count, dbias, ws)
+                with _SideStream(dc, srcs[l]):
+                    if not w_done:
+                        ops.wgrad(Src(dc), srcs[l], gw, K, S, padL, PAD_REFLECT, roll=ctx.rolls[l])
+                        W.finish(blk.conv, gw)
+                    if not w_done or not want_w:
+                        _ready(blk)
+                if ctx.x_needs and dx is None:
+                    dx = ops.conv1d_dgrad(dc, w, srcs[l].L, S, roll=ctx.rolls[l], pack=blk._pack)
+                continue
             if bn is not None:
                 dc = _act_bwd_bn(cs[l], dh, blk.act.weight, bn, _gb(blk.act.weight), _gb(bn[2]),
-                                 _gb(bn[3]), _gb(blk.conv.bias))
+                                 _gb(bn[3]), dbias)
             else:
                 dc = ops.act_bwd(cs[l], dh, slope=blk.act.weight, dslope=_gb(blk.act.weight),
-                                 dbias=_gb(blk.conv.bias))
-            padL = ops.conv_pad(K, S)[0]
+                                 dbias=dbias)
             with _SideStream(dc, srcs[l]):
-                if W.needs_grad(blk.conv):
+                if want_w:
                     gw = W.grad_target(blk.conv)
                     ops.wgrad(Src(dc), srcs[l], gw, K, S, padL, PAD_REFLECT, roll=ctx.rolls[l])
                     W.finish(blk.conv, gw)
diff --git a/segan_pytorch_amd/ops.py b/segan_pytorch_amd/ops.py
--- a/segan_pytorch_amd/ops.py
+++ b/segan_pytorch_amd/ops.py
@@ -5,7 +5,7 @@
 
 from . import _lib
 from . import layout
-from ._lib import ACT_NONE, ACT_TANH, PAD_REFLECT, PAD_ZERO, SeganSrc, check
+from ._lib import ACT_NONE, ACT_TANH, PAD_REFLECT, PAD_ZERO, SeganGradSrc, SeganSrc, check
 
 
 import os as _os
@@ -403,6 +403,91 @@
                           pad_mode, roll, PREC_FP32, flags,
                           ctypes.c_void_p(scratch.data_ptr()) if scratch is not None else None, nbytes,
                           _stream()), 'wgrad')
+
+
+class GradSrc(object):
+
+    def __init__(self, a, dh, dskip=None, slope=None, alpha=None, bn=None, totals=None,
+                 count_total=None):
+        _chk(a, 'a', 3)
+        _chk(dh, 'dh', 3)
+        if dh.shape != a.shape or (dskip is not None and dskip.shape != a.shape):
+            raise ValueError('GradSrc: a, dh and dskip must have one shape')
+        self.a, self.dh, self.dskip, self.slope, self.alpha = a, dh, dskip, slope, alpha
+        self.bn, self.totals = bn, totals
+        self.B, self.C, self.L = a.shape
+        if bn is not None:
+            if totals is None:
+                raise ValueError('GradSrc: the BatchNorm kind needs totals')
+            count = float(self.B) * float(self.L) if count_total is None else float(count_total)
+            self.inv_count = 1.0 / count
+        else:
+            self.inv_count = 0.0
+
+    def tensors(self):
+        bn = self.bn or ()
+        return [t for t in (self.a, self.dh, self.dskip, self.slope, self.alpha, self.totals) + tuple(bn)
+                if t is not None]
+
+    def c_struct(self):
+        g = SeganGradSrc()
+        p = lambda t: t.data_ptr() if t is not None else None
+        g.a, g.dh, g.dskip, g.slope, g.alpha = p(self.a), p(self.dh), p(self.dskip), p(self.slope), p(self.alpha)
+        if self.bn is not None:
+            mean, rstd, gamma, beta = self.bn
+            g.bn_mean, g.bn_rstd, g.bn_gamma, g.bn_beta = p(mean), p(rstd), p(gamma), p(beta)
+            g.totals = p(self.totals)
+        g.inv_count = self.inv_count
+        return g
+
+
+def wgrad_lazy(g, hi, dw, K, S, padL, pad_mode, roll=0, dbias=None):
+    if not g.a.is_cuda:
+        return False
+    _chk(dw, 'dw', 3)
+    M, N = g.C, hi.C
+    if tuple(dw.shape) != (M, N, K):
+        raise ValueError('wgrad_lazy: dw {} != ({}, {}, {})'.format(tuple(dw.shape), M, N, K))
+    if g.B != hi.B or g.L * S != hi.L:
+        raise ValueError('wgrad_lazy: lo [{}x{}] / hi [{}x{}] inconsistent for stride {}'.format(
+            g.B, g.L, hi.B, hi.L, S))
+    lib = _lib.load()
+    flags = 1 if _deterministic else 0
+    scratch, nbytes = None, 0
+    if flags:
+        nbytes = lib.segan_wgrad_scratch_bytes(g.B, M, N, g.L, S, PREC_FP32, flags)
+        scratch = _stream_scratch(nbytes, dw.device)
+    cg, ch = g.c_struct(), hi.c_struct()
+    rc = lib.segan_wgrad_lazy(ctypes.byref(cg), ctypes.byref(ch), _ptr(dw), _ptr(dbias), g.B, M, N, g.L,
+                              K, S, padL, pad_mode, roll, _precision, flags,
+                              ctypes.c_void_p(scratch.data_ptr()) if scratch is not None else None,
+                              nbytes, _stream())
+    if rc == _EUNSUPPORTED:
+        return False
+    check(rc, 'wgrad_lazy')
+    return True
+
+
+def conv1d_dgrad_lazy(g, w, L, S, roll=0, padL=None):
+    _chk(w, 'weight', 3)
+    M, N, K = w.shape
+    if g.C != M or g.L * S != L:
+        raise ValueError('conv1d_dgrad_lazy: gradient [{}x{}] inconsistent with weight {} / L {}'.format(
+            g.C, g.L, tuple(w.shape), L))
+    if N > 2 or _precision != PREC_FP32 or not g.a.is_cuda:
+        return None
+    if padL is None:
+        padL = conv_pad(K, S)[0]
+    B = g.B
+    dx = torch.empty((B, N, L), device=w.device, dtype=torch.float32)
+    halo = torch.empty((B * N * max(K - 1, 1),), device=w.device, dtype=torch.float32)
+    cg = g.c_struct()
+    rc = _lib.load().segan_conv1d_dgrad_lazy(ctypes.byref(cg), _ptr(w.detach()), _ptr(dx), _ptr(halo), B,
+                                             N, M, L, K, S, padL, roll, PREC_FP32, _stream())
+    if rc == _EUNSUPPORTED:
+        return None
+    check(rc, 'conv1d_dgrad_lazy')
+    return dx
 
 
 def deconv1d_fwd(src, w, bias, S, act=ACT_NONE, pack=None):
```

Result: no change. 3568 (median of 6 runs) (+0.4%).
